# octree-nn/octfusion

Hardware: AMD Instinct MI355X
Metric: denoising-steps/sec (depth-8 octree, batch 8) (higher is better)
Workload: dtype f32 storage, fp16x3 products (fp16 hi + lo operand pairs = 22 significand bits, three fp16 MFMAs per product, fp32 accumulate)

## Files before the change

### include/ofx.h

```cpp
#ifndef OFX_H_
#define OFX_H_

#include <stddef.h>
#include <stdint.h>

#ifdef __cplusplus
extern "C" {
#endif

#define OFX_OK 0
#define OFX_EINVAL (-1)
#define OFX_ELAUNCH (-2)
#define OFX_ENODEV (-3)

#define OFX_ACT_NONE 0
#define OFX_ACT_SILU 1
#define OFX_ACT_GELU 2

#define OFX_MAX_DEPTH 16

int ofx_version(void);
const char* ofx_status_string(int status);
int ofx_device_check(void);
const char* ofx_build_hash(void);
// ... 189 lines not shown
                             const int32_t* col, const int32_t* nbr_ext, const int32_t* multi_seg, int64_t n_multi,
                             void* aux, size_t aux_bytes, const void* tfp, int64_t ldt_bytes, int nt, const void* W2,
                             int cout, const float* bias, const float* emb, int64_t lde, const int32_t* batch_id,
                             const float* res, int64_t ldr, float* out, int64_t ldc, double* stats ,
                             int64_t stats_ld, void* ws, size_t ws_bytes, void* sync , size_t sync_bytes,
                             int mode, int aux_ready, void* stream);
int ofx_set_gconv_persistent(int on);
int64_t ofx_gemm_planes_packed_bytes(int K, int N, int mode);
int ofx_pack_gemm_planes(const float* W, int64_t sk, int64_t sn, int K, int N, int mode, void* out, void* stream);
int ofx_gemm_planes(const void* ap, int64_t lda_bytes, int64_t n_a, int64_t M, int K, const int32_t* row_tab,
                    const void* W2, int N, const float* bias, float* out, int64_t ldc, int out_mode, void* ws,
                    size_t ws_bytes, void* sync, size_t sync_bytes, int mode, void* stream);
int ofx_set_gconv_cus(int cus);
int ofx_gconv3_plan(int64_t n_rows, int cout, int nkt, int wm, int ni, int cus, int32_t* out, int64_t out_len);
int ofx_set_gconv2_tile(int wm);

int ofx_grid_conv_table(int mode, int depth_out, int batch_size, int32_t pad, int32_t* nbr27,
                        void* stream);
int64_t ofx_conv3d_packed_k(int cin);
int ofx_pack_conv3d(const float* W, int cin, int cout, float* Wp, void* stream);
int ofx_gridconv_fwd(const float* x, int64_t ldx, int cin, int64_t n_in, int64_t n_out,
                     const int32_t* nbr27 ,
                     const int32_t* nbr27_ext ,
                     const float* zero_row ,
                     const float* Wp, int cout, const float* bias, const float* emb, int64_t lde,
                     const int32_t* batch_id, const float* res, int64_t ldr, float* out,
                     int64_t ldc, void* ws, size_t ws_bytes, void* stream);
int ofx_gather_gemm_f32(const float* x, int64_t ldx, int cin, int ntap, int64_t n_src, int64_t n_out, const int32_t* tab,
                        const float* zero_row, const float* Wp, int64_t Kp, int cout, const float* bias,
                        const float* res, int64_t ldr, float* out, int64_t ldc, const int32_t* out_rows, void* ws,
                        size_t ws_bytes, int out_mode, void* stream);
int ofx_set_attention_split(int on);
int ofx_attention(const float* qkv, int64_t ldq, int batch_size, int T, int heads, int ch,
                  float* out, int64_t ldo, void* stream);

int ofx_attention_bwd(const float* qkv, int64_t ldq, const float* dout, int64_t ldo, int batch_size, int T, int heads,
                      int ch, float* rowstat, float* dqkv, int64_t ldd, void* stream);

int ofx_gather_mean(const float* x, int64_t ldx, int cin, int64_t n_nodes,
                    const int32_t* seg_ptr, const int32_t* col, float* col_data,
                    void* stream);

int ofx_gn_stats(const float* x, int64_t ldx, int64_t n, int C, const int32_t* batch_id,
                 int batch_size, double* sums, void* stream);
int ofx_gn_stats_acc(const float* x, int64_t ldx, int64_t n, int C, const int32_t* batch_id, int batch_size,
                     double* sums, void* stream);
int ofx_gn_finalize(const double* sums, const float* count, int batch_size, int C, int groups,
                    float eps, float count_eps, float* mean, float* rstd, void* stream);
int ofx_gn_apply(const float* x, int64_t ldx, int64_t n, int C, const int32_t* batch_id,
                 const float* mean , const float* rstd , const double* sums ,
                 const float* count, int groups, float eps, float count_eps, const float* w, const float* bias,
                 int act, float* out, int64_t ldo, void* stream);

int ofx_gn_fused_rows(const float* x, int64_t ldx, int rows_per_batch, int batch_size, int C, int groups, float eps,
                      float count_eps, const float* w, const float* bias, int act, float* out, int64_t ldo,
                      void* stream);

int ofx_set_gn_rows16(int on);

int ofx_rows_copy(const float* src, int64_t lds, const int32_t* smap, float* dst, int64_t ldd,
                  const int32_t* dmap, int64_t n, int C, void* stream);
int ofx_rows_copy_planes(const float* src, int64_t lds, const int32_t* smap, float* dst, int64_t ldd,
                         const int32_t* dmap, int64_t n, int C, int mode, void* stream);
int ofx_act(const float* x, float* y, int64_t n, int act, void* stream);
int ofx_timestep_embedding(const float* t, int batch_size, int dim, float max_period,
                           float* out, void* stream);
int ofx_learned_sinusoid(const float* t, const float* w, int batch_size, int half, float* out, void* stream);
int ofx_linear_small(const float* a, int64_t lda, int M, int K, const float* W, int64_t ldw, int N, const float* bias,
                     const float* res, int64_t ldr, int act_in, int act_out, float* out, int64_t ldo, void* stream);
int ofx_ddim_eps_update(float* x, const float* eps, const float* coef, float* x0_out, int64_t n,
                        void* stream);
int ofx_ddim_x0_update(float* x, const float* x0, const float* noise, const float* coef,
                       int64_t n, void* stream);

size_t ofx_mc_ws_bytes(int batch, int size);
int ofx_mc_count(const float* sdf, int batch, int size, float level, void* ws, int64_t* counts, void* stream);
int ofx_mc_emit(const float* sdf, int batch, int size, float level, float step, float bbmin, float scale, void* ws,
                const int64_t* vert_off, const int64_t* tri_off, float* verts, int32_t* faces, void* stream);
int ofx_mc_table_host(int8_t* tri_table, uint8_t* ntri);

size_t ofx_mesh_cc_ws_bytes(int64_t total_verts, int64_t total_faces, int batch);
int ofx_mesh_cc_label(const int32_t* faces, const int64_t* vert_off, const int64_t* tri_off, int batch,
                      int64_t total_verts, int64_t total_faces, int32_t* label, void* ws, int32_t* status,
                      void* stream);
int ofx_mesh_cc_table(const int32_t* faces, const int32_t* label, const int64_t* vert_off, const int64_t* tri_off,
                      int batch, int64_t total_verts, int64_t total_faces, int32_t* comp_of_vert, int32_t* comp_off,
                      void* ws, const int32_t* status, void* stream);
int ofx_mesh_cc_stats(const float* verts, const int32_t* faces, const int32_t* label, const int64_t* vert_off,
                      const int64_t* tri_off, int batch, int64_t total_verts, int64_t total_faces, int64_t n_comp,
                      int32_t* table, void* ws, const int32_t* status, void* stream);
int ofx_mesh_cc_select(const float* verts, const int32_t* faces, const int32_t* label, const int64_t* vert_off,
                       const int64_t* tri_off, int batch, int64_t total_verts, int64_t total_faces,
                       int32_t* winner_label, int64_t* keep_counts, void* ws, const int32_t* status, void* stream);
int ofx_mesh_cc_extract(const float* verts, const int32_t* faces, const int64_t* vert_off, const int64_t* tri_off,
                        int batch, int64_t total_verts, int64_t total_faces, const int64_t* new_vert_off,
                        const int64_t* new_tri_off, float* out_verts, int32_t* out_faces, void* ws,
                        const int32_t* status, void* stream);

size_t ofx_voxmesh_ws_bytes(int batch, int depth, int weld);
int ofx_voxmesh_mask_keys(const int64_t* keys, int64_t n, int batch0, int batch, int depth, void* ws, void* stream);
int ofx_voxmesh_mask_dense(const float* occ, int batch, int depth, float threshold, void* ws, void* stream);
int ofx_voxmesh_count(int batch, int depth, int weld, void* ws, int64_t* counts, void* stream);
int ofx_voxmesh_emit(int batch, int depth, int weld, void* ws, const int64_t* vert_off, const int64_t* tri_off,
                     float* verts, int32_t* faces, void* stream);

#define OFX_EMD_MAX_POINTS 2048
// ... 28 lines not shown
```

### octfusion_amd/_lib.py

```python
import ctypes
import os

import torch

_HERE = os.path.dirname(os.path.abspath(__file__))
LIB_PATH = os.environ.get('OFX_LIB', os.path.join(_HERE, 'libofx.so'))

c_p = ctypes.c_void_p
c_i = ctypes.c_int
c_l = ctypes.c_int64
c_f = ctypes.c_float
c_sz = ctypes.c_size_t
c_u64 = ctypes.c_uint64


class OfxTree(ctypes.Structure):
    _fields_ = [('depth', c_i), ('full_depth', c_i), ('batch_size', c_i),
                ('child_all', c_p), ('key_all', c_p), ('leafrank_all', c_p),
                ('nnum_host', c_p), ('nnum_nempty_host', c_p)]


_SIGS = {
    'ofx_version': (c_i, [], False),
    'ofx_status_string': (ctypes.c_char_p, [c_i], False),
    'ofx_device_check': (c_i, [], False),
    'ofx_build_hash': (ctypes.c_char_p, [], False),
    'ofx_probe_mfma_sustained': (c_i, [c_i, c_i, c_p, c_p, c_p], True),
    'ofx_scan_ws_bytes': (c_sz, [c_l], False),
    'ofx_scan_i32': (c_i, [c_p, c_p, c_l, c_p, c_p], True),
    'ofx_octree_full_layer': (c_i, [c_i, c_i, c_p, c_p, c_p], True),
    'ofx_octree_split': (c_i, [c_p, c_l, c_p, c_p, c_p, c_p], True),
    'ofx_octree_grow': (c_i, [c_p, c_p, c_l, c_p, c_p, c_p], True),
    'ofx_split_small_label0': (c_i, [c_p, c_i, c_i, c_p, c_p], True),
    'ofx_split_small_label1': (c_i, [c_p, c_i, c_i, c_p, c_p, c_p], True),
    'ofx_split_large_label0': (c_i, [c_p, c_l, c_p, c_p], True),
    'ofx_split_large_label1': (c_i, [c_p, c_l, c_p, c_p, c_p], True),
    'ofx_octree2voxel_cf': (c_i, [c_p, c_l, c_i, c_i, c_i, c_p, c_p], True),
    'ofx_voxel2octree_cf': (c_i, [c_p, c_i, c_i, c_i, c_p, c_l, c_p], True),
    'ofx_points_sort_ws_bytes': (c_sz, [c_l], False),
    'ofx_points_keys': (c_i, [c_p, c_l, c_p, c_i, c_l, c_i, c_p, c_p, c_p], True),
    'ofx_points_sort': (c_i, [c_p, c_p, c_l, c_p, c_p, c_p, c_sz, c_p], True),
    'ofx_octree_label_from_points': (c_i, [c_p, c_l, c_p, c_l, c_i, c_i, c_p, c_p], True),
    'ofx_octree_point_features': (c_i, [c_p, c_p, c_l, c_p, c_l, c_p, c_l, c_p, c_l, c_i, c_p, c_p, c_p, c_p], True),
    'ofx_tree_leafrank_ws_bytes': (c_sz, [c_l], False),
    'ofx_tree_leafrank': (c_i, [c_p, c_p, c_i, c_p, c_p, c_p], True),
    'ofx_graph_nodes': (c_i, [ctypes.POINTER(OfxTree), c_i, c_p, c_p, c_p, c_p, c_p], True),
    'ofx_graph_count': (c_i, [ctypes.POINTER(OfxTree), c_i, c_p, c_p], True),
    'ofx_graph_reverse_count': (c_i, [c_p, c_p, c_l, c_p, c_p], True),
    'ofx_graph_reverse_fill': (c_i, [c_p, c_p, c_l, c_p, c_p, c_p, c_p, c_p], True),
    'ofx_graph_primary_w': (c_i, [c_p, c_p, c_p, c_l, c_p, c_p], True),
    'ofx_graph_multi_flag_w': (c_i, [c_p, c_p, c_l, c_p, c_p], True),
    'ofx_graph_primary_ext_w': (c_i, [c_p, c_p, c_p, c_l, c_p, c_p, c_p, c_p], True),
    'ofx_graphconv_bwd_data': (c_i, [c_p, c_l, c_i, c_l, c_p, c_p, c_p, c_p, c_p, c_p, c_l, c_p, c_p, c_l, c_i, c_p,
                                     c_l, c_p, c_sz, c_p], True),
    'ofx_graphconv_bwd_weight': (c_i, [c_p, c_l, c_i, c_l, c_p, c_p, c_p, c_p, c_p, c_l, c_p, c_p, c_l, c_i, c_p, c_l,
                                       c_i, c_p, c_l, c_p, c_sz, c_p], True),
    'ofx_gn_backward': (c_i, [c_p, c_l, c_p, c_l, c_l, c_i, c_p, c_i, c_p, c_i, c_f, c_p, c_p, c_p, c_p, c_i, c_p, c_p,
                              c_p, c_l, c_p, c_p, c_p], True),
    'ofx_gemm_tn_f32': (c_i, [c_p, c_l, c_p, c_l, c_l, c_l, c_l, c_p, c_p, c_sz, c_p], True),
    'ofx_table_reverse_count': (c_i, [c_p, c_l, c_i, c_l, c_p, c_p], True),
    'ofx_table_reverse_fill': (c_i, [c_p, c_l, c_i, c_l, c_p, c_p, c_p, c_p, c_p], True),
    'ofx_seg_primary_w': (c_i, [c_p, c_p, c_p, c_l, c_p, c_p], True),
    'ofx_seg_multi_flag_w': (c_i, [c_p, c_p, c_l, c_p, c_p], True),
    'ofx_seg_primary_ext_w': (c_i, [c_p, c_p, c_p, c_l, c_l, c_p, c_p, c_p, c_p], True),
    'ofx_gridconv_bwd_data': (c_i, [c_p, c_l, c_i, c_l, c_l, c_p, c_p, c_p, c_p, c_p, c_p, c_l, c_p, c_p, c_i, c_p, c_l,
                                    c_p, c_sz, c_p], True),
    'ofx_gridconv_bwd_weight': (c_i, [c_p, c_l, c_i, c_l, c_l, c_p, c_p, c_p, c_p, c_l, c_i, c_p, c_p, c_sz, c_p], True),
    'ofx_attention_bwd': (c_i, [c_p, c_l, c_p, c_l, c_i, c_i, c_i, c_i, c_p, c_p, c_l, c_p], True),
    'ofx_adamw_step': (c_i, [c_p, c_p, c_p, c_p, c_l, c_f, c_f, c_f, c_f, c_f, c_i, c_p], True),
    'ofx_ema_update': (c_i, [c_p, c_p, c_l, c_f, c_p], True),
    'ofx_gn_fused_rows': (c_i, [c_p, c_l, c_i, c_i, c_i, c_i, c_f, c_f, c_p, c_p, c_i, c_p, c_l, c_p], True),
    'ofx_set_gn_rows16': (c_i, [c_i], True),
    'ofx_mpu_eval': (c_i, [ctypes.POINTER(OfxTree), c_i, c_i, c_p, c_l, c_p, c_p, c_p, c_p], True),
    'ofx_mpu_eval_grid': (c_i, [ctypes.POINTER(OfxTree), c_i, c_i, c_p, c_i, c_f, c_f, c_i, c_l, c_l, c_p, c_p, c_p], True),
    'ofx_mpu_eval_grad': (c_i, [ctypes.POINTER(OfxTree), c_i, c_i, c_p, c_l, c_p, c_p, c_p, c_p, c_p], True),
    'ofx_mpu_backward': (c_i, [ctypes.POINTER(OfxTree), c_i, c_i, c_p, c_l, c_p, c_p, c_p, c_p, c_p], True),
    'ofx_octree_ce': (c_i, [c_p, c_l, c_p, c_l, c_f, c_p, c_p, c_l, c_p], True),
    'ofx_sdf_reg_loss': (c_i, [c_p, c_p, c_p, c_p, c_l, c_f, c_f, c_p, c_p, c_p, c_p], True),
    'ofx_kl_sample_fwd': (c_i, [c_p, c_l, c_p, c_l, c_i, c_p, c_p, c_p], True),
    'ofx_kl_sample_bwd': (c_i, [c_p, c_l, c_p, c_p, c_l, c_i, c_f, c_p, c_l, c_p], True),
    'ofx_graph_fill': (c_i, [ctypes.POINTER(OfxTree), c_i, c_p, c_p, c_p], True),
    'ofx_graph_expand': (c_i, [c_p, c_l, c_p, c_p, c_p, c_p, c_p], True),
    'ofx_graph_type_frac': (c_i, [c_p, c_p, c_p, c_l, c_i, c_p, c_l, c_p], True),
    'ofx_set_precision': (c_i, [c_i], True),
    'ofx_set_range_words': (c_i, [c_p], True),
    'ofx_get_precision': (c_i, [], False),
    'ofx_gn_apply_rows': (c_i, [], False),
    'ofx_set_attention_split': (c_i, [c_i], True),
    'ofx_gather_gemm_f32': (c_i, [c_p, c_l, c_i, c_i, c_l, c_l, c_p, c_p, c_p, c_l, c_i, c_p, c_p, c_l, c_p, c_l, c_p, c_p, c_sz, c_i, c_p], True),
    'ofx_graphconv_narrow_in_tab': (c_i, [c_p, c_l, c_i, c_l, c_p, c_p, c_p, c_p, c_l, c_p, c_p, c_i, c_p, c_i, c_p, c_p, c_p, c_l, c_p, c_l,
                                          c_p, c_sz, c_p], True),
    'ofx_graphconv_narrow_in': (c_i, [c_p, c_l, c_i, c_l, c_p, c_p, c_p, c_i, c_p, c_i, c_p, c_p, c_p, c_l, c_p, c_l, c_p, c_sz, c_p], True),
    'ofx_narrow_out_pack': (c_i, [c_p, c_i, c_i, c_i, c_i, c_p, c_p], True),
    'ofx_narrow_out_type_term': (c_i, [c_p, c_l, c_i, c_l, c_p, c_i, c_i, c_p, c_p, c_p], True),
    'ofx_graphconv_narrow_out': (c_i, [c_p, c_l, c_i, c_l, c_p, c_p, c_p, c_p, c_l, c_p], True),
    'ofx_packed_floats': (c_l, [c_l, c_l], False),
    'ofx_packed_k': (c_l, [c_l], False),
    'ofx_graphconv_packed_k': (c_l, [c_i, c_i], False),
    'ofx_pack_weights': (c_i, [c_p, c_l, c_l, c_l, c_l, c_i, c_i, c_p, c_l, c_p], True),
    'ofx_gemm_f32': (c_i, [c_p, c_l, c_p, c_l, c_l, c_p, c_l, c_l, c_p, c_p, c_l, c_p, c_l, c_p, c_p, c_sz, c_p], True),
    'ofx_gemm_f32_planes': (c_i, [c_p, c_l, c_p, c_l, c_l, c_p, c_l, c_l, c_p, c_p, c_l, c_p, c_l, c_p, c_p, c_sz, c_i, c_p], True),
    'ofx_graphconv_fwd': (c_i, [c_p, c_l, c_i, c_l, c_p, c_p, c_p, c_p, c_p, c_l, c_p, c_p, c_l, c_i, c_p, c_l,
                                c_i, c_p, c_p, c_l, c_p, c_p, c_l, c_p, c_l, c_p, c_l, c_p, c_sz, c_p], True),
    'ofx_planes_split': (c_i, [c_p, c_l, c_l, c_i, c_i, c_i, c_p, c_l, c_p], True),
    'ofx_planes_merge': (c_i, [c_p, c_l, c_l, c_i, c_i, c_p, c_l, c_p], True),
    'ofx_gn_apply_planes': (c_i, [c_p, c_l, c_l, c_i, c_p, c_p, c_p, c_p, c_p, c_i, c_f, c_f, c_p, c_p, c_i, c_i, c_p,
                                  c_l, c_p, c_p, c_p, c_l, c_p, c_p, c_l, c_p], True),
    'ofx_gn_apply_planes_oct': (c_i, [c_p, c_l, c_l, c_i, c_p, c_p, c_p, c_p, c_p, c_i, c_f, c_f, c_p, c_p, c_i, c_i, c_p,
                                      c_l, c_l, c_p, c_p, c_p, c_l, c_i, c_p, c_p, c_l, c_p], True),
    'ofx_planes_packed_ktiles': (c_l, [c_i, c_i, c_i], False),
    'ofx_planes_packed_bytes': (c_l, [c_i, c_i, c_i, c_i], False),
    'ofx_pack_weights_planes': (c_i, [c_p, c_l, c_l, c_i, c_i, c_i, c_i, c_p, c_p], True),
    'ofx_graphconv_fwd_planes': (c_i, [c_p, c_l, c_i, c_l, c_p, c_p, c_p, c_p, c_l, c_p, c_sz, c_p, c_l, c_i, c_p, c_i,
                                       c_p, c_p, c_l, c_p, c_p, c_l, c_p, c_l, c_p, c_l, c_p, c_sz, c_p, c_sz, c_i, c_i,
                                       c_p], True),
    'ofx_set_gconv_persistent': (c_i, [c_i], True),
    'ofx_set_gconv_cus': (c_i, [c_i], True),
    'ofx_gemm_planes_packed_bytes': (c_l, [c_i, c_i, c_i], False),
    'ofx_pack_gemm_planes': (c_i, [c_p, c_l, c_l, c_i, c_i, c_i, c_p, c_p], True),
    'ofx_gemm_planes': (c_i, [c_p, c_l, c_l, c_l, c_i, c_p, c_p, c_i, c_p, c_p, c_l, c_i, c_p, c_sz, c_p, c_sz, c_i, c_p], False),
    'ofx_gconv3_plan': (c_i, [c_l, c_i, c_i, c_i, c_i, c_i, c_p, c_l], False),
    'ofx_set_gconv2_tile': (c_i, [c_i], True),
    'ofx_graph_multi_flag': (c_i, [c_p, c_l, c_p, c_p], True),
    'ofx_graph_primary_ext': (c_i, [c_p, c_p, c_l, c_p, c_p, c_p, c_p], True),
    'ofx_graph_primary': (c_i, [c_p, c_p, c_l, c_p, c_p], True),
    'ofx_grid_conv_table': (c_i, [c_i, c_i, c_i, c_i, c_p, c_p], True),
    'ofx_conv3d_packed_k': (c_l, [c_i], False),
    'ofx_pack_conv3d': (c_i, [c_p, c_i, c_i, c_p, c_p], True),
    'ofx_gridconv_fwd': (c_i, [c_p, c_l, c_i, c_l, c_l, c_p, c_p, c_p, c_p, c_i, c_p, c_p, c_l, c_p, c_p, c_l, c_p,
                               c_l, c_p, c_sz, c_p], True),
    'ofx_attention': (c_i, [c_p, c_l, c_i, c_i, c_i, c_i, c_p, c_l, c_p], True),
    'ofx_gather_mean': (c_i, [c_p, c_l, c_i, c_l, c_p, c_p, c_p, c_p], True),
    'ofx_gn_stats': (c_i, [c_p, c_l, c_l, c_i, c_p, c_i, c_p, c_p], True),
    'ofx_gn_stats_acc': (c_i, [c_p, c_l, c_l, c_i, c_p, c_i, c_p, c_p], True),
    'ofx_gn_finalize': (c_i, [c_p, c_p, c_i, c_i, c_i, c_f, c_f, c_p, c_p, c_p], True),
    'ofx_gn_apply': (c_i, [c_p, c_l, c_l, c_i, c_p, c_p, c_p, c_p, c_p, c_i, c_f, c_f, c_p, c_p, c_i, c_p, c_l, c_p], True),
    'ofx_rows_copy': (c_i, [c_p, c_l, c_p, c_p, c_l, c_p, c_l, c_i, c_p], True),
    'ofx_rows_copy_planes': (c_i, [c_p, c_l, c_p, c_p, c_l, c_p, c_l, c_i, c_i, c_p], True),
    'ofx_act': (c_i, [c_p, c_p, c_l, c_i, c_p], True),
    'ofx_timestep_embedding': (c_i, [c_p, c_i, c_i, c_f, c_p, c_p], True),
    'ofx_learned_sinusoid': (c_i, [c_p, c_p, c_i, c_i, c_p, c_p], True),
    'ofx_linear_small': (c_i, [c_p, c_l, c_i, c_i, c_p, c_l, c_i, c_p, c_p, c_l, c_i, c_i, c_p, c_l, c_p], True),
    'ofx_ddim_eps_update': (c_i, [c_p, c_p, c_p, c_p, c_l, c_p], True),
    'ofx_ddim_x0_update': (c_i, [c_p, c_p, c_p, c_p, c_l, c_p], True),
    'ofx_mc_ws_bytes': (c_sz, [c_i, c_i], False),
    'ofx_mc_count': (c_i, [c_p, c_i, c_i, c_f, c_p, c_p, c_p], True),
    'ofx_mc_emit': (c_i, [c_p, c_i, c_i, c_f, c_f, c_f, c_f, c_p, c_p, c_p, c_p, c_p, c_p], True),
    'ofx_mc_table_host': (c_i, [c_p, c_p], True),
    'ofx_mesh_cc_ws_bytes': (c_sz, [c_l, c_l, c_i], False),
    'ofx_mesh_cc_label': (c_i, [c_p, c_p, c_p, c_i, c_l, c_l, c_p, c_p, c_p, c_p], True),
    'ofx_mesh_cc_table': (c_i, [c_p, c_p, c_p, c_p, c_i, c_l, c_l, c_p, c_p, c_p, c_p, c_p], True),
    'ofx_mesh_cc_stats': (c_i, [c_p, c_p, c_p, c_p, c_p, c_i, c_l, c_l, c_l, c_p, c_p, c_p, c_p], True),
    'ofx_mesh_cc_select': (c_i, [c_p, c_p, c_p, c_p, c_p, c_i, c_l, c_l, c_p, c_p, c_p, c_p, c_p], True),
    'ofx_mesh_cc_extract': (c_i, [c_p, c_p, c_p, c_p, c_i, c_l, c_l, c_p, c_p, c_p, c_p, c_p, c_p, c_p], True),
    'ofx_voxmesh_ws_bytes': (c_sz, [c_i, c_i, c_i], False),
    'ofx_voxmesh_mask_keys': (c_i, [c_p, c_l, c_i, c_i, c_i, c_p, c_p], True),
    'ofx_voxmesh_mask_dense': (c_i, [c_p, c_i, c_i, c_f, c_p, c_p], True),
    'ofx_voxmesh_count': (c_i, [c_i, c_i, c_i, c_p, c_p, c_p], True),
    'ofx_voxmesh_emit': (c_i, [c_i, c_i, c_i, c_p, c_p, c_p, c_p, c_p, c_p], True),
    'ofx_surface_sample_ws_bytes':(c_sz, [c_i, c_l], False),
    'ofx_surface_sample': (c_i, [c_p, c_p, c_p, c_p, c_i, c_l, c_i, c_u64, c_i, c_p, c_p, c_p], True),
    'ofx_surface_sample_oriented': (c_i, [c_p, c_p, c_p, c_p, c_i, c_l, c_i, c_u64, c_i, c_p, c_p, c_p, c_p], True),
    'ofx_nn_matrix': (c_i, [c_p, c_l, c_i, c_p, c_l, c_i, c_p, c_p], True),
    'ofx_emd_matrix': (c_i, [c_p, c_l, c_p, c_l, c_i, c_i, c_p, c_p], True),
    'ofx_metrics_hash': (c_u64, [c_u64, c_l, c_l, c_i], False),
    'ofx_sdf_sample_ws_bytes': (c_sz, [c_l, c_i], False),
    'ofx_sdf_sample_nodes': (c_i, [c_p, c_i, c_p, c_l, c_p, c_i, c_i, c_i, c_u64, c_l, c_p, c_f, c_p, c_p, c_p, c_p, c_p,
                                   c_p], True),
    'ofx_sdf_sample_occu': (c_i, [c_p, c_i, c_l, c_u64, c_l, c_p, c_f, c_p, c_p, c_p], True),
    'ofx_mesh_sdf_ws_bytes': (c_sz, [c_i, c_l, c_l, c_i], False),
    'ofx_mesh_sdf': (c_i, [c_p, c_p, c_p, c_p, c_i, c_i, c_i, c_p, c_p, c_p, c_p], True),
    'ofx_mesh_sdf_set_counters': (c_i, [c_p], True),
}

EXPORTS = sorted(_SIGS)


class OfxError(RuntimeError):
    pass


_lib = None


def lib():
    global _lib
    if _lib is None:
        if not os.path.exists(LIB_PATH):
            raise OfxError('libofx.so not built: run `python -m octfusion_amd.build` '
                           '(the product has no CPU / eager fallback)')
        L = ctypes.CDLL(LIB_PATH)
        for name, (res, args, _) in _SIGS.items():
            fn = getattr(L, name)
            fn.restype = res
            fn.argtypes = args
        _check_fresh(L)
        _lib = L
    return _lib


def _check_fresh(L):
    if 'OFX_LIB' in os.environ:
        return
    from . import build
    try:
        want = build.source_hash()
    except OSError:
        return
    have = L.ofx_build_hash().decode()
    if have != want:
        raise OfxError('libofx.so is stale: built from sources %s, the tree is %s -- run `python -m octfusion_amd.build`'
                       % (have, want))


PROFILE = None
META = None


def _timed(prof, name, args, always):
    global META
    meta, META = META, None
    e0 = torch.cuda.Event(enable_timing=True)
    e1 = torch.cuda.Event(enable_timing=True)
    e0.record()
    rc = getattr(lib(), name)(*args)
    e1.record()
    if always or rc == 0:
        prof.append((name, e0, e1, meta))
    return rc


def call(name, *args):
    prof = PROFILE
    if prof is not None and _SIGS[name][2]:
        rc = _timed(prof, name, args, True)
    else:
        rc = getattr(lib(), name)(*args)
    if _SIGS[name][2] and rc != 0:
        msg = lib().ofx_status_string(rc).decode()
        raise OfxError('%s failed: %s (%d)' % (name, msg, rc))
    return rc


def call_may_decline(name, *args):
    prof = PROFILE
    if prof is not None:
        rc = _timed(prof, name, args, False)
    else:
        rc = getattr(lib(), name)(*args)
    if rc < 0:
        raise OfxError('%s failed with status %d' % (name, rc))
    return rc == 0


def ptr(t):
    if t is None:
        return None
    return t.data_ptr()


def stream():
    return torch.cuda.current_stream().cuda_stream


def require_device():
    if not torch.cuda.is_available():
        raise OfxError('no HIP device: octfusion_amd has no CPU path')
    rc = lib().ofx_device_check()
    if rc != 0:
        raise OfxError('ofx_device_check: %s' % lib().ofx_status_string(rc).decode())
```

### octfusion_amd/csrc/ofx_common.h

```cpp
#pragma once
#include <hip/hip_runtime.h>
#include <stdint.h>

#include "../../include/ofx.h"

#define OFX_LAUNCH_CHECK()                         \
  do {                                             \
    if (hipGetLastError() != hipSuccess) return OFX_ELAUNCH; \
  } while (0)

static inline hipStream_t ofx_stream(void* s) { return reinterpret_cast<hipStream_t>(s); }

static inline int64_t ofx_cdiv(int64_t a, int64_t b) { return (a + b - 1) / b; }

constexpr int OFX_MAX_DEVICES = 64;
static inline bool ofx_raise_lds_limit(const void* kernel, int bytes, bool (&done)[OFX_MAX_DEVICES]) {
  int dev = 0;
  if (hipGetDevice(&dev) != hipSuccess || dev < 0 || dev >= OFX_MAX_DEVICES) return false;
  if (done[dev]) return true;
  if (hipFuncSetAttribute(kernel, hipFuncAttributeMaxDynamicSharedMemorySize, bytes) != hipSuccess) return false;
  done[dev] = true;
  return true;
}

uint32_t* ofx_range_words();

static inline int ofx_grid(int64_t work_items, int block) {
  int64_t g = ofx_cdiv(work_items, block);
  if (g < 1) g = 1;
  if (g > 2048 * 4) g = 2048 * 4;
  return (int)g;
}

constexpr uint64_t MT_GAMMA = 0x9E3779B97F4A7C15ull;
__host__ __device__ __forceinline__ uint64_t mt_mix(uint64_t z) {
  z = (z ^ (z >> 30)) * 0xBF58476D1CE4E5B9ull;
  z = (z ^ (z >> 27)) * 0x94D049BB133111EBull;
  return z ^ (z >> 31);
}
__host__ __device__ __forceinline__ uint64_t mt_step(uint64_t h, uint64_t x) { return mt_mix(h + MT_GAMMA * (x + 1)); }

__host__ __device__ static inline uint32_t ofx_compact3(uint64_t v) {
  v &= 0x1249249249249249ull;
  v = (v ^ (v >> 2)) & 0x10c30c30c30c30c3ull;
  v = (v ^ (v >> 4)) & 0x100f00f00f00f00full;
  v = (v ^ (v >> 8)) & 0x1f0000ff0000ffull;
  v = (v ^ (v >> 16)) & 0x1f00000000ffffull;
  v = (v ^ (v >> 32)) & 0x1fffffull;
  return (uint32_t)v;
}
__host__ __device__ static inline uint64_t ofx_spread3(uint64_t v) {
  v &= 0x1fffffull;
  v = (v | (v << 32)) & 0x1f00000000ffffull;
  v = (v | (v << 16)) & 0x1f0000ff0000ffull;
  v = (v | (v << 8)) & 0x100f00f00f00f00full;
  v = (v | (v << 4)) & 0x10c30c30c30c30c3ull;
  v = (v | (v << 2)) & 0x1249249249249249ull;
  return v;
}
__host__ __device__ static inline void ofx_key2xyz(int64_t key, int& x, int& y, int& z, int& b) {
  const uint64_t k = (uint64_t)key & ((1ull << 48) - 1);
  b = (int)((uint64_t)key >> 48);
  z = (int)ofx_compact3(k);
  y = (int)ofx_compact3(k >> 1);
  x = (int)ofx_compact3(k >> 2);
}
__host__ __device__ static inline uint64_t ofx_xyz2morton(int x, int y, int z) {
  return (ofx_spread3((uint64_t)x) << 2) | (ofx_spread3((uint64_t)y) << 1) | ofx_spread3((uint64_t)z);
}
```

### octfusion_amd/csrc/ofx_gemm.hip

```cpp
#include "ofx_gemm_common.h"

constexpr int BM = 128;
constexpr int BK = 32;
constexpr int A_LD = BK + 4;
constexpr int MODE_DENSE = 0;
constexpr int MODE_GATHER = 1;

struct TileCoords { int split, tm, tn; };
__device__ __forceinline__ TileCoords tile_coords(const GemmArgs& g) {
  const int ntile = g.ntm * g.ntn;
  int bid = ofx_xcd_swizzle(blockIdx.x, ntile * g.nsplit);
  const int split = bid / ntile;
  bid -= split * ntile;
  const int tm = bid / g.ntn;
  return {split, tm, bid - tm * g.ntn};
}

__device__ __forceinline__ void load_a_dense(const GemmArgs& g, int64_t m0, int64_t k0, float4 (&va)[4]) {
  const int c4 = threadIdx.x & 7, r0 = threadIdx.x >> 3;
  const int64_t k = k0 + c4 * 4;
  const bool vec = ((g.lda & 3) == 0) && (k + 3 < g.K) && ((((uintptr_t)g.A) & 15) == 0);
#pragma unroll
  for (int i = 0; i < 4; ++i) {
    const int64_t m = m0 + r0 + 32 * i;
// ... 748 lines not shown
                                                            int64_t N, const int32_t* __restrict__ bid,
                                                            double* __restrict__ stats, int64_t stats_ld) {
  __shared__ double red[3][64][2];
  const int c = threadIdx.x & 63, rg = threadIdx.x >> 6;
  const int64_t n = (int64_t)blockIdx.y * 64 + c;
  const int64_t w0 = (int64_t)blockIdx.x * 64;
  const int64_t nc = n < N ? n : N - 1;
  int b[16];
  float2 v[16];
#pragma unroll
  for (int i = 0; i < 16; ++i) {
    const int64_t w = w0 + rg * 16 + i;
    const int64_t wc = w < nwr ? w : nwr - 1;
    b[i] = bid[wc * wr_rows];
    v[i] = *reinterpret_cast<const float2*>(part + (wc * N + nc) * 2);
    if (w >= nwr) { b[i] = -1; v[i] = make_float2(0.f, 0.f); }
  }
  const int bfirst = bid[w0 * wr_rows];
  bool ok = true;
#pragma unroll
  for (int i = 0; i < 16; ++i) ok = ok && (b[i] == bfirst || b[i] < 0);
  const bool uni = __syncthreads_and(ok);
  auto flush = [&](int bb, double s, double q) {
    double* o = stats + ((int64_t)bb * stats_ld + n) * 2;
    unsafeAtomicAdd(o, s); unsafeAtomicAdd(o + 1, q);
  };
  if (uni) {
    double s = 0.0, q = 0.0;
#pragma unroll
    for (int i = 0; i < 16; ++i) { s += (double)v[i].x; q += (double)v[i].y; }
    if (rg > 0) { red[rg - 1][c][0] = s; red[rg - 1][c][1] = q; }
    __syncthreads();
    if (rg == 0 && n < N) {
#pragma unroll
      for (int r = 0; r < 3; ++r) { s += red[r][c][0]; q += red[r][c][1]; }
      flush(bfirst, s, q);
    }
  } else if (n < N) {
    double s = 0.0, q = 0.0;
    int sb = -1;
#pragma unroll
    for (int i = 0; i < 16; ++i) {
      if (b[i] < 0) continue;
      if (b[i] != sb) {
        if (sb >= 0) flush(sb, s, q);
        sb = b[i]; s = 0.0; q = 0.0;
      }
      s += (double)v[i].x; q += (double)v[i].y;
    }
    if (sb >= 0) flush(sb, s, q);
  }
}

int ofx_launch_stats_reduce(const GemmArgs& g, int wr_rows, hipStream_t st) {
  const int64_t nwr = ofx_cdiv(g.M, wr_rows);
  stats_reduce_kernel<<<dim3((unsigned)ofx_cdiv(nwr, 64), (unsigned)ofx_cdiv(g.N, 64)), 256, 0, st>>>(
      g.stats_part, nwr, wr_rows, g.N, g.bid, g.stats, g.stats_ld);
  OFX_LAUNCH_CHECK();
  return OFX_OK;
}

template <int MODE>
static int launch_gemm(GemmArgs& g, float* ws, size_t ws_bytes, hipStream_t st) {
  if (g.M <= 0 || g.N <= 0) return OFX_OK;
  if (MODE == MODE_GATHER && !(g.fast && g.nbr_ext && g.aux && (!g.out_rows || g.gather_out_rows))) return OFX_EINVAL;
  {
    auto al16 = [](const void* p) { return (reinterpret_cast<uintptr_t>(p) & 15) == 0; };
    g.vec4 = g.N % 4 == 0 && al16(g.out) && g.ldc % 4 == 0 && (!g.res || (al16(g.res) && g.ldr % 4 == 0)) &&
             (!g.emb || (al16(g.emb) && g.lde % 4 == 0)) && (!g.bias || al16(g.bias));
  }
  const int bn = g.N <= 32 ? 32 : (g.N <= 64 ? 64 : 128);
  g.ntm = (int)ofx_cdiv(g.M, BM);
  g.ntn = (int)ofx_cdiv(g.N, bn);
  const int nkt = (int)(g.Kp / BK);
  int nsplit = 1;
  const int tiles = g.ntm * g.ntn;
  if (ws && tiles < 256 && nkt >= 8) {
    nsplit = (int)ofx_cdiv(512, tiles);
    if (nsplit > nkt / 4) nsplit = nkt / 4;
    if (nsplit > 64) nsplit = 64;
    const size_t per = (size_t)g.M * g.N * sizeof(float);
    if ((size_t)nsplit * per > ws_bytes) nsplit = (int)(ws_bytes / per);
    if (nsplit < 2) nsplit = 1;
  }
  g.kt_per_split = (int)ofx_cdiv(nkt, nsplit);
  nsplit = (int)ofx_cdiv(nkt, g.kt_per_split);
  g.nsplit = nsplit;
  g.ws = ws;
  bool fast = true;
  if (MODE == MODE_DENSE) {
    fast = ((g.lda & 3) == 0) && ((g.K & 3) == 0) && g.K >= 4 && ((((uintptr_t)g.A) & 15) == 0);
    if (fast) { g.ndir = 1; g.n_src = 0; g.aux = g.A; g.tf = g.A; g.ldt = g.lda; g.nbr_ext = (const int32_t*)g.A; }
  }
  g.W16 = (g_precision != 1) ? reinterpret_cast<const uint16_t*>(g.Wp + g.Kp * g.N) : nullptr;
  const int wr_rows = bn == 32 ? 32 : 64;
  const int64_t nwr = ofx_cdiv(g.M, wr_rows);
  if (!(g.stats && g.vec4 && nsplit == 1 && g.stats_part &&
        (size_t)nwr * g.N * 2 * sizeof(float) <= g.stats_part_bytes && (((uintptr_t)g.stats_part) & 15) == 0))
    g.stats_part = nullptr;
  g.oscale_p = (fast && g.W16) ? g.Wp + 2 * g.Kp * g.N : nullptr;
  const int flavour = !fast ? 0 : (!g.W16 ? 1 : (g_precision == 3 ? 3 : 2));
  int rc;
  if (bn == 32) rc = launch_cfg<MODE, 4, 1, 1, 1>(g, flavour, st);
  else if (bn == 64) rc = launch_cfg<MODE, 2, 2, 2, 1>(g, flavour, st);
  else rc = launch_cfg<MODE, 2, 2, 2, 2>(g, flavour, st);
  if (rc) return rc;
  if (nsplit > 1) {
    const bool ws16 = (((uintptr_t)g.ws) & 15) == 0;
    if (g.vec4 && ws16) splitk_reduce_v4_kernel<<<ofx_grid(g.M * (g.N >> 2), 256), 256, 0, st>>>(g);
    else splitk_reduce_kernel<<<ofx_grid(g.M * g.N, 256), 256, 0, st>>>(g);
  }
  if (g.stats_part) {
    rc = ofx_launch_stats_reduce(g, wr_rows, st);
    if (rc) return rc;
  }
  OFX_LAUNCH_CHECK();
  return OFX_OK;
}

static inline int64_t pad32(int64_t v) { return (v + 31) / 32 * 32; }

extern "C" int64_t ofx_packed_k(int64_t K) { return pad32(K); }
extern "C" int64_t ofx_graphconv_packed_k(int cin, int nt) {
  return pad32(7 * (int64_t)cin) + (nt > 1 ? pad32(7 * (int64_t)nt) : 0);
}

__global__ void pack_weights_kernel(const float* __restrict__ W, int64_t sk, int64_t sn, int64_t K, int64_t N, int cin,
                                    int nt, float* __restrict__ Wp, int64_t Kp) {
  const int64_t total = (Kp / 4) * N;
  const int ntc = nt > 1 ? nt : 0;
  const int64_t Kf = (7 * (int64_t)cin + 31) / 32 * 32;
  for (int64_t t = (int64_t)blockIdx.x * blockDim.x + threadIdx.x; t < total; t += (int64_t)gridDim.x * blockDim.x) {
    const int64_t kq = t / N, n = t - kq * N;
    float v[4];
#pragma unroll
    for (int kk = 0; kk < 4; ++kk) {
      const int64_t k = kq * 4 + kk;
      int64_t src = -1;
      if (cin > 0) {
        if (k < 7 * (int64_t)cin) {
          const int64_t dir = k / cin, c = k - dir * cin;
          src = dir * (cin + ntc) + c;
        } else if (k >= Kf && ntc > 0 && k - Kf < 7 * (int64_t)ntc) {
          const int64_t kt = k - Kf, dir = kt / ntc, ty = kt - dir * ntc;
          src = dir * (cin + ntc) + cin + ty;
        }
      } else if (k < K) {
        src = k;
      }
      v[kk] = src >= 0 ? W[src * sk + n * sn] : 0.f;
    }
    *reinterpret_cast<float4*>(Wp + t * 4) = make_float4(v[0], v[1], v[2], v[3]);
  }
}

extern "C" int ofx_pack_weights(const float* W, int64_t sk, int64_t sn, int64_t K, int64_t N, int cin, int nt,
                                float* Wp, int64_t Kp, void* stream) {
  if (!W || !Wp || K < 1 || N < 1 || (Kp & 31) || cin < 0 || nt < 0) return OFX_EINVAL;
  if (cin > 0) {
    if (Kp != ofx_graphconv_packed_k(cin, nt) || K != 7 * (int64_t)(cin + (nt > 1 ? nt : 0))) return OFX_EINVAL;
  } else if (Kp != pad32(K)) {
    return OFX_EINVAL;
  }
  if (((uintptr_t)Wp & 15) != 0) return OFX_EINVAL;
  pack_weights_kernel<<<ofx_grid((Kp / 4) * N, 256), 256, 0, ofx_stream(stream)>>>(W, sk, sn, K, N, cin, nt, Wp, Kp);
  if (int rc = pack_bf16x3(Wp, Kp, N, ofx_stream(stream))) return rc;
// ... 52 lines not shown
extern "C" int ofx_gemm_f32(const float* A, int64_t lda, const int32_t* a_rows, int64_t M, int64_t K, const float* Wp,
                            int64_t Kp, int64_t N, const float* bias, const float* res, int64_t ldr, float* out,
                            int64_t ldc, const int32_t* out_rows, void* ws, size_t ws_bytes, void* stream) {
  return ofx_gemm_f32_planes(A, lda, a_rows, M, K, Wp, Kp, N, bias, res, ldr, out, ldc, out_rows, ws, ws_bytes, 0, stream);
}

static int gather_common(GemmArgs& g, const float* x, int64_t ldx, int cin, int ndir, int64_t n_rows,
                         const int32_t* nbr, const int32_t* seg_ptr, const int32_t* col, const float* Wp, int64_t Kp,
                         int cout, const float* bias, const float* emb, int64_t lde, const int32_t* batch_id,
                         const float* res, int64_t ldr, float* out, int64_t ldc) {
  if (n_rows < 0 || cin < 1 || cout < 1 || !x || !nbr || !Wp || !out || ldx < cin || ldc < cout ||
      (res && ldr < cout) || (emb && (!batch_id || lde < cout)) || ((uintptr_t)Wp & 15))
    return OFX_EINVAL;
  g.x = x; g.ldx = ldx; g.cin = cin; g.ndir = ndir;
  g.fast = (cin % 32 == 0) && ((ldx & 3) == 0) && (((uintptr_t)x & 15) == 0);
  g.nbr = nbr; g.seg_ptr = seg_ptr; g.col = col;
  g.Kf = pad32((int64_t)ndir * cin);
  g.M = n_rows; g.K = Kp; g.Wp = Wp; g.Kp = Kp; g.N = cout; g.bias = bias;
  g.emb = emb; g.lde = lde; g.bid = batch_id; g.res = res; g.ldr = ldr; g.out = out; g.ldc = ldc;
  return OFX_OK;
}

__device__ __forceinline__ float gather_elem(const GemmArgs& g, int64_t row, int64_t k) {
  if (k >= (int64_t)g.ndir * g.cin) return 0.f;
  const int dir = (int)(k / g.cin), c = (int)(k - (int64_t)dir * g.cin);
  const int32_t nb = g.nbr[row * g.ndir + dir];
  if (nb >= 0) return g.x[(int64_t)nb * g.ldx + c];
  if (nb == -1) return 0.f;
  const int64_t s = row * g.ndir + dir;
  const int32_t a = g.seg_ptr[s], e = g.seg_ptr[s + 1];
  float acc = 0.f;
  if (g.edge_w) {
    for (int32_t p = a; p < e; ++p) acc += g.edge_w[p] * g.x[(int64_t)g.col[p] * g.ldx + c];
    return acc;
  }
  for (int32_t p = a; p < e; ++p) acc += g.x[(int64_t)g.col[p] * g.ldx + c];
  if (e - a > 1) acc /= (float)(e - a);
  return acc;
}
__global__ void __launch_bounds__(256) col_rows_kernel(const GemmArgs g, int64_t row0, int64_t rows,
                                                       float* __restrict__ colbuf) {
  const int64_t k4n = g.Kp >> 2, total = rows * k4n;
  for (int64_t t = (int64_t)blockIdx.x * blockDim.x + threadIdx.x; t < total; t += (int64_t)gridDim.x * blockDim.x) {
    const int64_t r = t / k4n, k = (t - r * k4n) * 4;
    const int64_t row = row0 + r;
    float v[4];
#pragma unroll
    for (int kk = 0; kk < 4; ++kk)
      v[kk] = (k + kk < g.Kf) ? gather_elem(g, row, k + kk) : g.tf[row * g.ldt + (k + kk - g.Kf)];
    *reinterpret_cast<float4*>(colbuf + t * 4) = make_float4(v[0], v[1], v[2], v[3]);
  }
}

static int launch_gather_via_col(const GemmArgs& g, float* ws, size_t ws_bytes, hipStream_t st) {
  if (!ws || (((uintptr_t)ws) & 15)) return OFX_EINVAL;
  size_t tail = ws_bytes / 8;
  if (tail > (size_t(16) << 20)) tail = size_t(16) << 20;
  tail &= ~size_t(15);
  const size_t row_bytes = (size_t)g.Kp * sizeof(float);
  int64_t chunk = (int64_t)((ws_bytes - tail) / row_bytes) / 128 * 128;
  if (chunk < 128) return OFX_EINVAL;
  float* tail_ws = reinterpret_cast<float*>(reinterpret_cast<char*>(ws) + (ws_bytes - tail));
  for (int64_t r0 = 0; r0 < g.M; r0 += chunk) {
    const int64_t rows = g.M - r0 < chunk ? g.M - r0 : chunk;
    col_rows_kernel<<<ofx_grid(rows * (g.Kp >> 2), 256), 256, 0, st>>>(g, r0, rows, ws);
    GemmArgs d = {};
    d.A = ws; d.lda = g.Kp; d.M = rows; d.K = g.Kp; d.Wp = g.Wp; d.Kp = g.Kp; d.N = g.N; d.bias = g.bias;
    d.emb = g.emb; d.lde = g.lde; d.bid = g.bid ? g.bid + r0 : nullptr;
    d.res = g.res ? g.res + r0 * g.ldr : nullptr; d.ldr = g.ldr;
    d.out = g.out + r0 * g.ldc; d.ldc = g.ldc;
    d.stats = g.stats; d.stats_ld = g.stats_ld;
    if (g.stats) { d.stats_part = tail_ws; d.stats_part_bytes = tail; }
    const int rc = launch_gemm<MODE_DENSE>(d, g.stats ? nullptr : tail_ws, tail, st);
    if (rc) return rc;
  }
  return OFX_OK;
}

extern "C" int ofx_graphconv_fwd(const float* x, int64_t ldx, int cin, int64_t n_nodes, const int32_t* nbr,
                                 const int32_t* seg_ptr, const int32_t* col, const int32_t* nbr_ext,
                                 const int32_t* multi_seg, int64_t n_multi, float* aux, const float* type_frac,
                                 int64_t ldt, int nt_pad, const float* Wp, int64_t Kp, int cout, const float* bias,
                                 const float* emb, int64_t lde, const int32_t* batch_id, const float* res, int64_t ldr,
                                 float* out, int64_t ldc, double* stats, int64_t stats_ld, void* ws, size_t ws_bytes,
                                 void* stream) {
  if (n_nodes == 0 && cin >= 1 && cout >= 1) return OFX_OK;
  GemmArgs g = {};
  int rc = gather_common(g, x, ldx, cin, 7, n_nodes, nbr, seg_ptr, col, Wp, Kp, cout, bias, emb, lde, batch_id, res,
                         ldr, out, ldc);
  if (rc) return rc;
  if (!seg_ptr || !col) return OFX_EINVAL;
  if (nt_pad < 0 || (nt_pad & 31) || Kp != g.Kf + nt_pad) return OFX_EINVAL;
  if (nt_pad > 0 && (!type_frac || ldt < nt_pad || (ldt & 3) || ((uintptr_t)type_frac & 15))) return OFX_EINVAL;
  g.tf = type_frac; g.ldt = ldt;
  if (stats) {
    if (!batch_id || stats_ld < cout) return OFX_EINVAL;
    g.stats = stats; g.stats_ld = stats_ld; g.bid = batch_id;
    g.stats_part = (float*)ws; g.stats_part_bytes = ws_bytes;
    ws = nullptr;
  }
  hipStream_t st = ofx_stream(stream);
  if (g.fast && nbr_ext && aux && (((uintptr_t)aux & 15) == 0)) {
    if (n_multi < 0 || (n_multi > 0 && !multi_seg)) return OFX_EINVAL;
    multi_mean_kernel<<<ofx_grid((n_multi + 1) * (cin / 4), 256), 256, 0, st>>>(x, ldx, cin, seg_ptr, col, multi_seg,
                                                                               n_multi, aux, ldx, nullptr);
    g.nbr_ext = nbr_ext; g.aux = aux; g.ldaux = ldx; g.n_src = n_nodes;
    if (!g.tf) { g.tf = x; g.ldt = ldx; }
    return launch_gemm<MODE_GATHER>(g, (float*)ws, ws_bytes, st);
  }
  return launch_gather_via_col(g, stats ? g.stats_part : (float*)ws, stats ? g.stats_part_bytes : ws_bytes, st);
}

extern "C" int ofx_graphconv_bwd_data(const float* dy, int64_t ldy, int cout, int64_t n_nodes, const int32_t* nbr_rev,
                                      const int32_t* rev_ptr, const int32_t* rev_row, const float* rev_w,
                                      const int32_t* nbr_ext_rev, const int32_t* multi_seg, int64_t n_multi, float* aux,
                                      const float* WpT, int64_t KpT, int cin, float* dx, int64_t ldx, void* ws,
                                      size_t ws_bytes, void* stream) {
  if (n_nodes == 0 && cin >= 1 && cout >= 1) return OFX_OK;
  GemmArgs g = {};
  int rc = gather_common(g, dy, ldy, cout, 7, n_nodes, nbr_rev, rev_ptr, rev_row, WpT, KpT, cin, nullptr, nullptr, 0,
                         nullptr, nullptr, 0, dx, ldx);
  if (rc) return rc;
  if (!rev_ptr || !rev_row || !rev_w || KpT != g.Kf) return OFX_EINVAL;
  g.edge_w = rev_w;
  g.tf = dy; g.ldt = ldy;
  hipStream_t st = ofx_stream(stream);
  if (g.fast && nbr_ext_rev && aux && (((uintptr_t)aux & 15) == 0)) {
    if (n_multi < 0 || (n_multi > 0 && !multi_seg)) return OFX_EINVAL;
    multi_mean_kernel<<<ofx_grid((n_multi + 1) * (cout / 4), 256), 256, 0, st>>>(dy, ldy, cout, rev_ptr, rev_row,
                                                                                multi_seg, n_multi, aux, ldy, rev_w);
    g.nbr_ext = nbr_ext_rev; g.aux = aux; g.ldaux = ldy; g.n_src = n_nodes;
    return launch_gemm<MODE_GATHER>(g, (float*)ws, ws_bytes, st);
  }
  return launch_gather_via_col(g, (float*)ws, ws_bytes, st);
}

struct TnArgs {
  const float* P; int64_t ldp;
  const float* x; int64_t ldx; int cin; int ndir;
  const int32_t* nbr_ext; const float* aux; int64_t n_src;
  const float* tf; int64_t ldt; int64_t Kf;
  const float* Q; int64_t ldq;
  int64_t rows, row0, Kp, N;
  int64_t rows_per_slice;
  float* part;
};

template <bool DENSE_P, bool BF16X3>
__global__ void __launch_bounds__(256, 2) tn_gemm_kernel(const TnArgs a) {
  constexpr int LD = 132;
  constexpr int TP = 128 * 80;
  __shared__ __attribute__((aligned(16))) char tn_smem[BF16X3 ? 4 * TP : 2 * 32 * LD * 4];
  float* const Ps = reinterpret_cast<float*>(tn_smem);
  float* const Qs = Ps + 32 * LD;
  char* const Pt = tn_smem;
  char* const Qt = tn_smem + 2 * TP;
  const int lane = threadIdx.x & 63, wid = threadIdx.x >> 6;
  const int wm = wid >> 1, wn = wid & 1, l31 = lane & 31, h = lane >> 5;
  const int64_t m0 = (int64_t)blockIdx.x * 128, n0 = (int64_t)blockIdx.y * 128;
  const int64_t r_begin = (int64_t)blockIdx.z * a.rows_per_slice;
  const int64_t r_end = r_begin + a.rows_per_slice < a.rows ? r_begin + a.rows_per_slice : a.rows;
  f32x16 acc[2][2];
#pragma unroll
// ... 408 lines not shown
```

### octfusion_amd/csrc/ofx_gemm2.hip

```cpp
#include "ofx_planes.h"

template <int PREC, int WM, int NI>
__global__ void __launch_bounds__(512, 2) gconv2_kernel(const Gemm2Args a) {
  typedef G2Half<PREC, NI> Half;
  typedef G2Cfg<WM, NI> CF;
  constexpr int G2_NI = NI, G2_BN = CF::BN, G2_EPI_LOADS = CF::EPI_LOADS, RH = CF::READS;
  constexpr int G2_WM = WM, G2_BM = CF::BM, G2_A_BYTES = CF::A_BYTES, G2_BUF = CF::BUF, G2_TAB = CF::TAB;
  constexpr int G2_GLDS_PER_STEP = CF::GLDS;
  extern __shared__ __attribute__((aligned(128))) char smem2[];
  const GemmArgs& g = a.e;

  float osc = *g.oscale_p;
  asm volatile("" : "+s"(osc));
  const int ntile = g.ntm * g.ntn;
  const int bid = ofx_xcd_swizzle(blockIdx.x, ntile);
  const int tm = bid / g.ntn, tn = bid - tm * g.ntn;
  const int64_t m0 = a.row0 + (int64_t)tm * G2_BM, n0 = (int64_t)tn * G2_BN;

  const int lane = threadIdx.x & 63;
  const int wid = __builtin_amdgcn_readfirstlane(threadIdx.x >> 6);
  const int wm = wid >> 1, wn = wid & 1;
  const int l31 = lane & 31, h = lane >> 5;
  if (WM == 2 && a.stagger > 0 && blockIdx.x >= 256 && (int)blockIdx.x < a.prefetch) {
    const int grp = (int)blockIdx.x >> 8, ngrp = a.prefetch >> 8;
// ... 467 lines not shown
        const int64_t kk = k - Kf, dir = kk / ntc, ty = kk - dir * ntc;
        src = dir * (cin + ntc) + cin + ty;
      }
      w[e] = src >= 0 ? W[src * sk + n * sn] * wscale : 0.f;
    }
    u32x4 o;
    if (g2_pairs(mode)) {
#pragma unroll
      for (int e = 0; e < 4; ++e) {
        unsigned hi, lo;
        g2_split2(mode, w[2 * e], w[2 * e + 1], hi, lo);
        o[e] = p < 4 ? hi : lo;
      }
    } else {
#pragma unroll
      for (int e = 0; e < 4; ++e) o[e] = g2_pk_f16(w[2 * e], w[2 * e + 1]);
    }
    *reinterpret_cast<u32x4*>(out + t * 16) = o;
  }
}

extern "C" int ofx_pack_weights_planes(const float* W, int64_t sk, int64_t sn, int cin, int nt, int cout, int mode,
                                       void* out, void* stream) {
  if (!W || !out || mode < 1 || mode > 3 || cin < 1 || (cin % g2_chunk(mode)) || nt < 0 || cout < 1 ||
      ((uintptr_t)out & 15))
    return OFX_EINVAL;
  const int64_t nkt = ofx_planes_packed_ktiles(cin, nt, mode);
  const int ntc = nt > 1 ? nt : 0;
  if (ofx_launch_weight_scale(W, sk, sn, 7 * (int64_t)(cin + ntc), cout, mode != 2 ? 1 : 0,
                              reinterpret_cast<float*>((char*)out + nkt * cout * G2_LINE), ofx_stream(stream)))
    return OFX_ELAUNCH;
  planes_pack_kernel<<<ofx_grid(nkt * cout * 8, 256), 256, 0, ofx_stream(stream)>>>(W, sk, sn, cin, ntc,
                                                                                    cout, nkt, mode, (char*)out);
  OFX_LAUNCH_CHECK();
  return OFX_OK;
}

extern "C" int64_t ofx_gemm_planes_packed_bytes(int K, int N, int mode) {
  if (!g2_pairs(mode) || K < 32 || (K % 32) || N < 1) return 0;
  return (int64_t)(K / 32) * N * G2_LINE + G2_TRAILER;
}
extern "C" int ofx_pack_gemm_planes(const float* W, int64_t sk, int64_t sn, int K, int N, int mode, void* out,
                                    void* stream) {
  if (!W || !out || !g2_pairs(mode) || K < 32 || (K % 32) || N < 1 || ((uintptr_t)out & 15)) return OFX_EINVAL;
  const int64_t nkt = K / 32;
  if (ofx_launch_weight_scale(W, sk, sn, K, N, mode != 2 ? 1 : 0, reinterpret_cast<float*>((char*)out + nkt * N * G2_LINE),
                              ofx_stream(stream)))
    return OFX_ELAUNCH;
  planes_pack_kernel<<<ofx_grid(nkt * N * 8, 256), 256, 0, ofx_stream(stream)>>>(W, sk, sn, K, 0, N, nkt, mode, (char*)out, 1);
  OFX_LAUNCH_CHECK();
  return OFX_OK;
}

int ofx_launch_stats_reduce(const GemmArgs& g, int wr_rows, hipStream_t st);

template <int PREC, int WM, int NI>
static int g2_launch(const Gemm2Args& a, hipStream_t st) {
  static bool attr_set[OFX_MAX_DEVICES] = {};
  if (!ofx_raise_lds_limit(reinterpret_cast<const void*>(&gconv2_kernel<PREC, WM, NI>), G2Cfg<WM, NI>::LDS, attr_set))
    return OFX_ELAUNCH;
  gconv2_kernel<PREC, WM, NI><<<a.e.ntm * a.e.ntn, G2Cfg<WM, NI>::THREADS, G2Cfg<WM, NI>::LDS, st>>>(a);
  return OFX_OK;
}

static int g2_wm = 0;
constexpr int G2_STAGGER_PER_KTILE = 1100;
extern "C" int ofx_set_gconv2_tile(int wm) {
  if (wm != 0 && wm != 2 && wm != 4) return OFX_EINVAL;
  g2_wm = wm;
  return OFX_OK;
}

static int g3_wm_pref = 0;
static int g3_auto_wm(int64_t M, int cout, int nkt, int ni) {
  (void)cout; (void)ni;
  if (g3_wm_pref == 2 || g3_wm_pref == 4) return g3_wm_pref;
  const int64_t U4 = ofx_cdiv(M, 256) * ofx_cdiv(cout, 64 * ni) * nkt;
  return U4 >= 3500 ? 4 : 2;
}
int ofx_launch_gconv3(Gemm2Args& a, int mode, int wm, int ni, void* ws_tail, size_t ws_tail_bytes, void* sync,
                      size_t sync_bytes, hipStream_t st, int nd = 7);
static int g2_persistent = 1;
void ofx_gconv3_set_hybrid(int on);
extern "C" int ofx_set_gconv_persistent(int on) {
  if (on < 0 || on > 2) return OFX_EINVAL;
  g2_persistent = on ? 1 : 0;
  ofx_gconv3_set_hybrid(on == 2 ? 0 : 1);
  return OFX_OK;
}

extern "C" int ofx_graphconv_fwd_planes(const void* xp, int64_t ldx_bytes, int cin, int64_t n_nodes,
                                        const int32_t* seg_ptr, const int32_t* col, const int32_t* nbr_ext,
                                        const int32_t* multi_seg, int64_t n_multi, void* aux, size_t aux_bytes,
                                        const void* tfp, int64_t ldt_bytes, int nt, const void* W2, int cout,
                                        const float* bias, const float* emb, int64_t lde, const int32_t* batch_id,
                                        const float* res, int64_t ldr, float* out, int64_t ldc, double* stats,
                                        int64_t stats_ld, void* ws, size_t ws_bytes, void* sync, size_t sync_bytes,
                                        int mode, int aux_ready, void* stream) {
  if (mode < 1 || mode > 3) return OFX_EINVAL;
  const int64_t ch = g2_chunk(mode);
  if (n_nodes == 0 && cin >= 1 && cout >= 1) return OFX_OK;
  if (n_nodes < 0 || cin < 1 || (cin % ch) || cout < 1 || !xp || !seg_ptr || !col || !nbr_ext || !aux || !W2 || !out ||
      ldx_bytes < (int64_t)cin * (g2_pairs(mode) ? 4 : 2) || (ldx_bytes & 127) || ((uintptr_t)xp & 127) ||
      ((uintptr_t)aux & 127) || ((uintptr_t)W2 & 127) || ldc < cout || (res && ldr < cout) ||
      (emb && (!batch_id || lde < cout)) || n_multi < 0 || (n_multi > 0 && !multi_seg) || nt < 0)
    return OFX_EINVAL;
  if (aux_bytes < (size_t)(n_multi + 1) * (size_t)ldx_bytes) return OFX_EINVAL;
  const int ntc = nt > 1 ? nt : 0;
  if (ntc > 0 && (!tfp || (ldt_bytes & 127) || ((uintptr_t)tfp & 127))) return OFX_EINVAL;
  if (stats && (!batch_id || stats_ld < cout)) return OFX_EINVAL;
  hipStream_t st = ofx_stream(stream);
  if (!aux_ready)
    planes_multi_mean_kernel<<<ofx_grid((n_multi + 1) * (cin / 8), 256), 256, 0, st>>>(
        (const char*)xp, ldx_bytes, cin, seg_ptr, col, multi_seg, n_multi, mode, (char*)aux);
  Gemm2Args a = {};
  a.xp = (const char*)xp; a.ldx = ldx_bytes; a.aux = (const char*)aux; a.n_src = n_nodes; a.nbr_ext = nbr_ext;
  a.tfp = ntc ? (const char*)tfp : (const char*)xp; a.ldt = ntc ? ldt_bytes : ldx_bytes;
  a.W2 = (const char*)W2;
  a.tpd = (int)(cin / ch); a.nkt_g = 7 * a.tpd; a.nkt = (int)ofx_planes_packed_ktiles(cin, nt, mode);
  GemmArgs& g = a.e;
  g.M = n_nodes; g.N = cout; g.K = g.Kp = (int64_t)a.nkt * ch; g.bias = bias; g.emb = emb; g.lde = lde; g.bid = batch_id;
  g.res = res; g.ldr = ldr; g.out = out; g.ldc = ldc; g.nsplit = 1;
  g.oscale_p = reinterpret_cast<const float*>((const char*)W2 + (int64_t)a.nkt * cout * G2_LINE);
  {
    auto al16 = [](const void* p) { return (reinterpret_cast<uintptr_t>(p) & 15) == 0; };
    g.vec4 = g.N % 4 == 0 && al16(g.out) && g.ldc % 4 == 0 && (!g.res || (al16(g.res) && g.ldr % 4 == 0)) &&
             (!g.emb || (al16(g.emb) && g.lde % 4 == 0)) && (!g.bias || al16(g.bias));
  }
  const int ni = cout <= 64 ? 1 : 2;
  g.ntn = (int)ofx_cdiv(g.N, 64 * ni);
  if (stats) {
    g.stats = stats; g.stats_ld = stats_ld;
    const int64_t nwr = ofx_cdiv(g.M, 64);
    if (g.vec4 && ws && (size_t)nwr * g.N * 2 * sizeof(float) <= ws_bytes && (((uintptr_t)ws) & 15) == 0) {
      g.stats_part = (float*)ws; g.stats_part_bytes = ws_bytes;
    }
  }
  int rc = OFX_OK;
#define G2_GO(P_, WM_)                                                                        \
  (ni == 1 ? (WM_ == 4 ? g2_launch<P_, 4, 1>(a, st) : g2_launch<P_, 2, 1>(a, st))             \
           : (WM_ == 4 ? g2_launch<P_, 4, 2>(a, st) : g2_launch<P_, 2, 2>(a, st)))
  auto launch = [&](int wm, int64_t row0, int64_t rows) -> int {
    a.row0 = row0;
    g.ntm = (int)ofx_cdiv(rows, wm * 64);
    a.stagger = wm == 2 ? G2_STAGGER_PER_KTILE * a.nkt : 0;
    a.prefetch = wm == 4 ? 256 : (ni == 1 ? 768 : 512);
    return mode == 2 ? G2_GO(2, wm) : (mode == 3 ? G2_GO(3, wm) : G2_GO(1, wm));
  };
  const int64_t tiles4 = ofx_cdiv(g.M, 256) * g.ntn;
  const int64_t tail4 = tiles4 % 256;
  const bool small_tail = tail4 > 0 && tail4 <= 64 && tiles4 < 1536;
  int wm_auto = (cout <= 128 && tiles4 < 2048) ? 2 : 4;
  if (cout > 128 && small_tail) wm_auto = 2;
  rc = 1;
  if (g2_persistent && sync) {
    size_t used = 0;
    if (g.stats_part) used = ((size_t)ofx_cdiv(g.M, 64) * (size_t)g.N * 2 * sizeof(float) + 255) & ~(size_t)255;
    const int wm3 = (g2_wm == 2 || g2_wm == 4) ? g2_wm : g3_auto_wm(g.M, cout, a.nkt, ni);
    if (ws && used <= ws_bytes)
      rc = ofx_launch_gconv3(a, mode, wm3, ni, (char*)ws + used, ws_bytes - used, sync, sync_bytes, st);
    if (rc < 0) return rc;
  }
  if (rc == 1) rc = launch((g2_wm == 2 || g2_wm == 4) ? g2_wm : wm_auto, 0, g.M);
#undef G2_GO
  if (rc) return rc;
  if (g.stats_part) {
    rc = ofx_launch_stats_reduce(g, 64, st);
    if (rc) return rc;
  }
  OFX_LAUNCH_CHECK();
  return OFX_OK;
}

extern "C" int ofx_gemm_planes(const void* ap, int64_t lda_bytes, int64_t n_a, int64_t M, int K, const int32_t* row_tab,
                               const void* W2, int N, const float* bias, float* out, int64_t ldc, int out_mode, void* ws,
                               size_t ws_bytes, void* sync, size_t sync_bytes, int mode, void* stream) {
  if (!g2_pairs(mode) || !ap || !row_tab || !W2 || !out || M < 0 || n_a < 1 || K < 32 || (K % 32) || N < 4 || (N & 3) ||
      lda_bytes < (int64_t)K * 4 || (lda_bytes & 127) || ((uintptr_t)ap & 127) || ((uintptr_t)W2 & 127) || ldc < N ||
      (ldc & 3) || ((uintptr_t)out & 15) || (bias && ((uintptr_t)bias & 15)) ||
      (out_mode && (!g2_pairs(out_mode) || (ldc & 31) || (N & 31) || ((uintptr_t)out & 127))))
    return OFX_EINVAL;
  if (M == 0) return OFX_OK;
  if (!sync || !ws || N < 128) return 1;
  Gemm2Args a = {};
  a.xp = (const char*)ap; a.ldx = lda_bytes; a.aux = (const char*)ap; a.n_src = n_a; a.nbr_ext = row_tab;
  a.tfp = (const char*)ap; a.ldt = lda_bytes;
  a.W2 = (const char*)W2;
  a.tpd = K / 32; a.nkt_g = a.tpd; a.nkt = a.tpd;
  GemmArgs& g = a.e;
  g.M = M; g.N = N; g.K = g.Kp = K; g.bias = bias; g.out = out; g.ldc = ldc; g.nsplit = 1; g.out_planes = out_mode;
  g.oscale_p = reinterpret_cast<const float*>((const char*)W2 + (int64_t)a.nkt * N * G2_LINE);
  g.vec4 = 1;
  g.ntn = (int)ofx_cdiv(g.N, 128);
  const int wm = g3_auto_wm(M, N, a.nkt, 2);
  const int rc = ofx_launch_gconv3(a, mode, wm, 2, ws, ws_bytes, sync, sync_bytes, ofx_stream(stream), 1);
  if (rc) return rc;
  OFX_LAUNCH_CHECK();
  return OFX_OK;
}
```

### octfusion_amd/csrc/ofx_gemm_common.h

```cpp
#pragma once
#include "ofx_common.h"

typedef float f32x16 __attribute__((ext_vector_type(16)));

struct GemmArgs {
  const float* A; int64_t lda; const int32_t* a_rows;
  const float* x; int64_t ldx; int cin; int ndir; int fast;
  const int32_t* nbr;
  const int32_t* seg_ptr; const int32_t* col;
  const float* edge_w;
  const float* tf; int64_t ldt; int64_t Kf;
  const int32_t* nbr_ext;
  const float* aux; int64_t ldaux; int64_t n_src;
  int64_t M, K;
  const float* Wp; int64_t Kp, N;
  const uint16_t* W16;
  const float* oscale_p;
  const float* bias;
  const float* emb; int64_t lde; const int32_t* bid;
  const float* res; int64_t ldr;
  float* out; int64_t ldc; const int32_t* out_rows;
  int gather_out_rows;
  int out_planes;
  double* stats; int64_t stats_ld;
  int ntm, ntn, nsplit, kt_per_split;
  float* ws;
  int vec4;
  float* stats_part; size_t stats_part_bytes;
};

static __global__ void __launch_bounds__(256) weight_absmax_kernel(const float* __restrict__ W, int64_t sk, int64_t sn, int64_t K,
                                                            int64_t N, unsigned* __restrict__ acc) {
  __shared__ float red[256];
  float m = 0.f;
  for (int64_t t = (int64_t)blockIdx.x * 256 + threadIdx.x; t < K * N; t += (int64_t)gridDim.x * 256) {
    const float a = fabsf(W[(t / N) * sk + (t % N) * sn]);
    if (a <= 3.0e38f) m = fmaxf(m, a);
  }
  red[threadIdx.x] = m;
  __syncthreads();
  for (int o = 128; o > 0; o >>= 1) {
    if ((int)threadIdx.x < o) red[threadIdx.x] = fmaxf(red[threadIdx.x], red[threadIdx.x + o]);
    __syncthreads();
  }
  if (threadIdx.x == 0) atomicMax(acc, __float_as_uint(red[0]));
}
static __global__ void weight_scale_finish_kernel(int fp16_operands, float* __restrict__ scale) {
  const float mx = __uint_as_float(reinterpret_cast<const unsigned*>(scale)[0]);
  float s = 1.f;
  if (fp16_operands && mx > 0.f) {
    int e;
    frexpf(mx, &e);
    int sh = 15 - e;
    sh = sh < -60 ? -60 : (sh > 60 ? 60 : sh);
    s = ldexpf(1.f, sh);
  }
  scale[0] = 1.f / s;
  scale[1] = s;
}
static inline int ofx_launch_weight_scale(const float* W, int64_t sk, int64_t sn, int64_t K, int64_t N, int fp16_operands,
                                          float* scale, hipStream_t st) {
  if (hipMemsetAsync(scale, 0, sizeof(float), st) != hipSuccess) return OFX_ELAUNCH;
  int64_t nb = (K * N + 256 * 16 - 1) / (256 * 16);
  nb = nb < 1 ? 1 : (nb > 1024 ? 1024 : nb);
  weight_absmax_kernel<<<(unsigned)nb, 256, 0, st>>>(W, sk, sn, K, N, reinterpret_cast<unsigned*>(scale));
  if (hipGetLastError() != hipSuccess) return OFX_ELAUNCH;
  weight_scale_finish_kernel<<<1, 1, 0, st>>>(fp16_operands, scale);
  if (hipGetLastError() != hipSuccess) return OFX_ELAUNCH;
  return OFX_OK;
}


__device__ __forceinline__ unsigned g2_pk_bf16(float a, float b) {
  unsigned r;
  asm("v_cvt_pk_bf16_f32 %0, %1, %2" : "=v"(r) : "v"(a), "v"(b));
  return r;
}
__device__ __forceinline__ unsigned g2_pk_f16(float a, float b) {
  const _Float16 x = (_Float16)a, y = (_Float16)b;
  return (unsigned)__builtin_bit_cast(unsigned short, x) | ((unsigned)__builtin_bit_cast(unsigned short, y) << 16);
}
__device__ __forceinline__ float g2_bf16_lo(unsigned p) { return __uint_as_float(p << 16); }
__device__ __forceinline__ float g2_bf16_hi(unsigned p) { return __uint_as_float(p & 0xffff0000u); }
// ... 213 lines not shown
```

### octfusion_amd/csrc/ofx_narrow.hip

```cpp
#include "ofx_gemm_common.h"

int ofx_launch_stats_reduce(const GemmArgs& g, int wr_rows, hipStream_t st);

namespace {

struct NarrowInArgs {
  const float* x; int64_t ldx; int cin; int64_t N;
  const int32_t* seg_ptr; const int32_t* col;
  const uint8_t* ntype; int nt;
  const float* W; int cout; const float* bias;
  float* out; int64_t ldc;
  const int32_t* bid; float* stats_part; double* stats; int64_t stats_ld;
};

template <int KP, int CI>
__global__ void __launch_bounds__(512, KP == 64 ? 6 : 4) narrow_in_kernel(const NarrowInArgs a) {
  constexpr int LD = KP + 1;
  __shared__ float cd[64 * LD];
  __shared__ float red[8][32][2];
  const int tid = threadIdx.x, lane = tid & 63, wv = tid >> 6;
  const int64_t row0 = (int64_t)blockIdx.x * 64;
  const int cin = a.cin, nt = a.nt, cpd = cin + nt, K = 7 * cpd;
  const bool wide = a.cout == 128;
  const int slice = wide ? (wv & 3) : (wv & 1);
  const int mt0 = wide ? (wv >> 2) : ((wv >> 1) & 1), nmt = (wide || wv < 4) ? 1 : 0;
  const int ln = lane & 31, lk = lane >> 5;

  {
    const int r = tid >> 3;
    for (int k = K + (tid & 7); k < KP; k += 8) cd[r * LD + k] = 0.f;
  }
  for (int s = tid; s < 64 * 7; s += 512) {
    const int r = s / 7, dir = s - r * 7;
    const int64_t row = row0 + r;
    float acc[CI], tc[8];
#pragma unroll
    for (int c = 0; c < CI; ++c) acc[c] = 0.f;
#pragma unroll
    for (int t = 0; t < 8; ++t) tc[t] = 0.f;
    int32_t b = 0, e = 0;
    if (row < a.N) { b = a.seg_ptr[row * 7 + dir]; e = a.seg_ptr[row * 7 + dir + 1]; }
    for (int32_t p = b; p < e; ++p) {
      const int64_t j = a.col[p];
      const float* xr = a.x + j * a.ldx;
      float v[CI];
#pragma unroll
      for (int c = 0; c < CI; ++c) v[c] = xr[c < cin ? c : cin - 1];
      const int ty = nt ? (int)a.ntype[j] : 0;
#pragma unroll
      for (int c = 0; c < CI; ++c) acc[c] += v[c];
#pragma unroll
      for (int t = 0; t < 8; ++t) tc[t] += ty == t ? 1.f : 0.f;
    }
    const float inv = __frcp_rn((float)(e - b > 1 ? e - b : 1));
    float* o = &cd[r * LD + dir * cpd];
// ... 305 lines not shown
__global__ void __launch_bounds__(256) narrow_out_kernel(const NarrowOutArgs a) {
  const int tid = threadIdx.x;
  const int d = tid & 7;
  const int64_t row = (int64_t)blockIdx.x * 32 + (tid >> 3);
  float acc[CO];
#pragma unroll
  for (int o = 0; o < CO; ++o) acc[o] = 0.f;
  if (row < a.N) {
    if (d < 7) {
      const int32_t b = a.seg_ptr[row * 7 + d], e = a.seg_ptr[row * 7 + d + 1];
      for (int32_t p = b; p < e; ++p) {
        const float* pr = a.P + (int64_t)a.col[p] * a.ldp + d * a.cout;
        float v[CO];
#pragma unroll
        for (int o = 0; o < CO; ++o) v[o] = pr[o < a.cout ? o : 0];
#pragma unroll
        for (int o = 0; o < CO; ++o) acc[o] += v[o];
      }
      const float cnt = (float)(e - b > 1 ? e - b : 1);
#pragma unroll
      for (int o = 0; o < CO; ++o) acc[o] = o < a.cout ? acc[o] / cnt : 0.f;
    } else if (a.tt) {
#pragma unroll
      for (int o = 0; o < CO; ++o) {
        const float v = a.tt[row * a.cout + (o < a.cout ? o : 0)];
        acc[o] = o < a.cout ? v : 0.f;
      }
    }
  }
#pragma unroll
  for (int o = 0; o < CO; ++o) {
    acc[o] += __shfl_xor(acc[o], 1);
    acc[o] += __shfl_xor(acc[o], 2);
    acc[o] += __shfl_xor(acc[o], 4);
  }
  if (d == 0 && row < a.N) {
#pragma unroll
    for (int o = 0; o < CO; ++o)
      if (o < a.cout) a.out[row * a.ldc + o] = acc[o];
  }
}

__global__ void narrow_out_pack_kernel(const float* __restrict__ W, int C, int nt, int cout, int pw, float* __restrict__ Wd) {
  const int64_t total = (int64_t)C * pw;
  for (int64_t t = (int64_t)blockIdx.x * blockDim.x + threadIdx.x; t < total; t += (int64_t)gridDim.x * blockDim.x) {
    const int c = (int)(t / pw), q = (int)(t - (int64_t)c * pw);
    const int dir = q / cout, o = q - dir * cout;
    Wd[t] = q < 7 * cout ? W[((int64_t)dir * (C + nt) + c) * cout + o] : 0.f;
  }
}

}

extern "C" int ofx_graphconv_narrow_in(const float* x, int64_t ldx, int cin, int64_t n_nodes, const int32_t* seg_ptr,
                                       const int32_t* col, const uint8_t* node_type, int nt, const float* W, int cout,
                                       const float* bias, const int32_t* batch_id, float* out, int64_t ldc, double* stats,
                                       int64_t stats_ld, void* ws, size_t ws_bytes, void* stream) {
  if (!x || !seg_ptr || !col || !W || !out || cin < 1 || cin > 8 || ldx < cin || nt < 0 || nt > 8 || (nt > 0 && !node_type) ||
      (cout != 64 && cout != 128) || ldc < cout || n_nodes < 0 ||
      7 * (cin + nt) > 96)
    return OFX_EINVAL;
  if (n_nodes == 0) return OFX_OK;
  const int64_t nblk = ofx_cdiv(n_nodes, 64);
  if (stats && (!batch_id || stats_ld < cout || !ws || ws_bytes < (size_t)nblk * cout * 2 * sizeof(float))) return OFX_EINVAL;
  hipStream_t st = ofx_stream(stream);
  NarrowInArgs a = {x, ldx, cin, n_nodes, seg_ptr, col, node_type, nt, W, cout, bias, out, ldc,
                    batch_id, (float*)ws, stats, stats_ld};
  const int K = 7 * (cin + nt);
  const unsigned nb = (unsigned)nblk;
  if (K <= 64) { if (cin <= 4) narrow_in_kernel<64, 4><<<nb, 512, 0, st>>>(a); else narrow_in_kernel<64, 8><<<nb, 512, 0, st>>>(a); }
  else { if (cin <= 4) narrow_in_kernel<96, 4><<<nb, 512, 0, st>>>(a); else narrow_in_kernel<96, 8><<<nb, 512, 0, st>>>(a); }
  OFX_LAUNCH_CHECK();
  if (stats) {
    GemmArgs g = {};
    g.M = n_nodes; g.N = cout; g.bid = batch_id; g.stats = stats; g.stats_ld = stats_ld; g.stats_part = (float*)ws;
    return ofx_launch_stats_reduce(g, 64, st);
  }
  return OFX_OK;
}

extern "C" int ofx_graphconv_narrow_in_tab(const float* x, int64_t ldx, int cin, int64_t n_nodes, const int32_t* seg_ptr,
                                           const int32_t* col, const int32_t* nbr_ext, const int32_t* multi_seg,
                                           int64_t n_multi, void* aux, const uint8_t* node_type, int nt, const float* W,
                                           int cout, const float* bias, const int32_t* batch_id, float* out, int64_t ldc,
                                           double* stats, int64_t stats_ld, void* ws, size_t ws_bytes, void* stream) {
  if (!x || !seg_ptr || !col || !nbr_ext || !aux || ((uintptr_t)aux & 15) || n_multi < 0 || (n_multi > 0 && !multi_seg) || !W ||
      !out || cin < 1 || cin > 8 || ldx < cin || nt < 0 || nt > 8 || (nt > 0 && !node_type) || (cout != 64 && cout != 128) ||
      ldc < cout || n_nodes < 0 || 7 * (cin + nt) > 96 || n_nodes + 1 + n_multi >= (1ll << 31))
    return OFX_EINVAL;
  if (n_nodes == 0) return OFX_OK;
  const int64_t ngroups = ofx_cdiv(n_nodes, 64);
  if (stats && (!batch_id || stats_ld < cout || !ws || ws_bytes < (size_t)ngroups * cout * 2 * sizeof(float))) return OFX_EINVAL;
  hipStream_t st = ofx_stream(stream);
  {
    const int64_t nbn = ofx_cdiv(n_nodes + 1, 256);
    const unsigned gn_ = (unsigned)(nbn < 16384 ? nbn : 16384);
    if (cin <= 4) narrow_rec_nodes_kernel<4><<<gn_, 256, 0, st>>>(x, ldx, cin, n_nodes, node_type, nt, (float*)aux);
    else narrow_rec_nodes_kernel<8><<<gn_, 256, 0, st>>>(x, ldx, cin, n_nodes, node_type, nt, (float*)aux);
    if (n_multi > 0) {
      const unsigned ga_ = (unsigned)ofx_cdiv(n_multi, 256);
      if (cin <= 4) narrow_rec_aux_kernel<4><<<ga_, 256, 0, st>>>(x, ldx, cin, n_nodes, seg_ptr, col, multi_seg, n_multi, node_type, nt, (float*)aux);
      else narrow_rec_aux_kernel<8><<<ga_, 256, 0, st>>>(x, ldx, cin, n_nodes, seg_ptr, col, multi_seg, n_multi, node_type, nt, (float*)aux);
    }
  }
  OFX_LAUNCH_CHECK();
  NarrowIn2Args a = {x, ldx, cin, n_nodes, nbr_ext, (const float*)aux, nt, W, cout, bias, out, ldc,
                     batch_id, (float*)ws, stats, stats_ld, ngroups};
  int dev = 0, cus = 256;
  if (hipGetDevice(&dev) == hipSuccess) {
    int n = 0;
    if (hipDeviceGetAttribute(&n, hipDeviceAttributeMultiprocessorCount, dev) == hipSuccess && n > 0) cus = n;
  }
  const int64_t want = (int64_t)cus * 2;
  const unsigned nb = (unsigned)(ngroups < want ? ngroups : want);
  const int K = 7 * (cin + nt);
  if (K <= 64) { if (cin <= 4) narrow_in2_kernel<64, 4><<<nb, 512, 0, st>>>(a); else narrow_in2_kernel<64, 8><<<nb, 512, 0, st>>>(a); }
  else if (K <= 72) { if (cin <= 4) narrow_in2_kernel<72, 4><<<nb, 512, 0, st>>>(a); else narrow_in2_kernel<72, 8><<<nb, 512, 0, st>>>(a); }
  else { if (cin <= 4) narrow_in2_kernel<96, 4><<<nb, 512, 0, st>>>(a); else narrow_in2_kernel<96, 8><<<nb, 512, 0, st>>>(a); }
  OFX_LAUNCH_CHECK();
  if (stats) {
    GemmArgs g = {};
    g.M = n_nodes; g.N = cout; g.bid = batch_id; g.stats = stats; g.stats_ld = stats_ld; g.stats_part = (float*)ws;
    return ofx_launch_stats_reduce(g, 64, st);
  }
  return OFX_OK;
}

extern "C" int ofx_narrow_out_pack(const float* W, int C, int nt, int cout, int pw, float* Wd, void* stream) {
  if (!W || !Wd || C < 1 || nt < 0 || cout < 1 || cout > 8 || pw < 7 * cout) return OFX_EINVAL;
  narrow_out_pack_kernel<<<ofx_grid((int64_t)C * pw, 256), 256, 0, ofx_stream(stream)>>>(W, C, nt, cout, pw, Wd);
  OFX_LAUNCH_CHECK();
  return OFX_OK;
}

extern "C" int ofx_narrow_out_type_term(const float* type_frac, int64_t ldt, int nt, int64_t n_nodes, const float* W, int C,
                                        int cout, const float* bias, float* tt, void* stream) {
  if (!W || !tt || C < 1 || cout < 1 || cout > 8 || nt < 0 || (nt > 0 && (!type_frac || ldt < 7 * nt)) || n_nodes < 0)
    return OFX_EINVAL;
  if (n_nodes == 0) return OFX_OK;
  const unsigned nblk = (unsigned)ofx_cdiv(n_nodes, 32);
  hipStream_t st = ofx_stream(stream);
  if (cout <= 4) narrow_type_term_kernel<4><<<nblk, 256, 0, st>>>(type_frac, ldt, nt, n_nodes, W, C, cout, bias, tt);
  else narrow_type_term_kernel<8><<<nblk, 256, 0, st>>>(type_frac, ldt, nt, n_nodes, W, C, cout, bias, tt);
  OFX_LAUNCH_CHECK();
  return OFX_OK;
}

extern "C" int ofx_graphconv_narrow_out(const float* P, int64_t ldp, int cout, int64_t n_nodes, const int32_t* seg_ptr,
                                        const int32_t* col, const float* type_term, float* out, int64_t ldc, void* stream) {
  if (!P || !seg_ptr || !col || !out || cout < 1 || cout > 8 || ldp < 7 * cout || ldc < cout || n_nodes < 0) return OFX_EINVAL;
  if (n_nodes == 0) return OFX_OK;
  NarrowOutArgs a = {P, ldp, cout, n_nodes, seg_ptr, col, type_term, out, ldc};
  hipStream_t st = ofx_stream(stream);
  const unsigned nblk = (unsigned)ofx_cdiv(n_nodes, 32);
  if (cout <= 4) narrow_out_kernel<4><<<nblk, 256, 0, st>>>(a);
  else narrow_out_kernel<8><<<nblk, 256, 0, st>>>(a);
  OFX_LAUNCH_CHECK();
  return OFX_OK;
}
```

### octfusion_amd/csrc/ofx_norm.hip

```cpp
#include "ofx_planes.h"

constexpr int GN_ROWS_PER_BLOCK = 64;

static inline int64_t gn_stats_rows(int64_t n, int batch_size, int C = 128) {
  const int64_t chunks = (n + GN_ROWS_PER_BLOCK - 1) / GN_ROWS_PER_BLOCK;
  const int64_t bytes_per_batch = n * (int64_t)C * 4 / (batch_size > 0 ? batch_size : 1);
  int64_t per_batch = bytes_per_batch / (512 << 10);
  per_batch = per_batch < 8 ? 8 : (per_batch > 128 ? 128 : per_batch);
  int64_t cap = per_batch * (int64_t)batch_size;
  if (cap < 64) cap = 64;
  return chunks <= cap ? GN_ROWS_PER_BLOCK : GN_ROWS_PER_BLOCK * ((chunks + cap - 1) / cap);
}

__global__ void __launch_bounds__(256) gn_stats_kernel(const float* __restrict__ x, int64_t ldx, int64_t n, int C,
                                                       const int32_t* __restrict__ bid, double* __restrict__ sums,
                                                       int64_t rpb) {
  __shared__ int sb[256];
  __shared__ float sv[256][8];
  const int CT = C >> 2;
  const int RP = 256 / CT;
  const int cl = threadIdx.x % CT, rl = threadIdx.x / CT;
  int cb = -1;
  float s[4] = {0, 0, 0, 0}, q[4] = {0, 0, 0, 0};
  auto flush_direct = [&](int b, const float* ps, const float* pq) {
// ... 38 lines not shown
    for (int j = 0; j < RP; ++j) {
      const int t = j * CT + cl;
      const int b = sb[t];
      if (b < 0) continue;
      if (b == cb) {
#pragma unroll
        for (int k = 0; k < 4; ++k) { ds[k] += (double)sv[t][k]; dq[k] += (double)sv[t][4 + k]; }
      } else {
        flush_direct(b, &sv[t][0], &sv[t][4]);
      }
    }
    if (cb >= 0) {
      double* o = sums + ((int64_t)cb * C + cl * 4) * 2;
#pragma unroll
      for (int k = 0; k < 4; ++k) { unsafeAtomicAdd(o + 2 * k, ds[k]); unsafeAtomicAdd(o + 2 * k + 1, dq[k]); }
    }
  }
}

extern "C" int ofx_gn_stats(const float* x, int64_t ldx, int64_t n, int C, const int32_t* batch_id, int batch_size,
                            double* sums, void* stream) {
  if (!x || !batch_id || !sums || n < 0 || C < 4 || (C & 3) || C > 1024 || ldx < C || (ldx & 3) ||
      ((uintptr_t)x & 15) || batch_size < 1)
    return OFX_EINVAL;
  hipStream_t st = ofx_stream(stream);
  if (hipMemsetAsync(sums, 0, sizeof(double) * 2 * (size_t)batch_size * C, st) != hipSuccess) return OFX_ELAUNCH;
  if (n > 0) gn_stats_kernel<<<(int)ofx_cdiv(n, gn_stats_rows(n, batch_size, C)), 256, 0, st>>>(x, ldx, n, C, batch_id, sums,
                                                                                             gn_stats_rows(n, batch_size, C));
  OFX_LAUNCH_CHECK();
  return OFX_OK;
}

extern "C" int ofx_gn_stats_acc(const float* x, int64_t ldx, int64_t n, int C, const int32_t* batch_id, int batch_size,
                                double* sums, void* stream) {
  if (!x || !batch_id || !sums || n < 0 || C < 4 || (C & 3) || C > 1024 || ldx < C || (ldx & 3) ||
      ((uintptr_t)x & 15) || batch_size < 1)
    return OFX_EINVAL;
  if (n > 0) gn_stats_kernel<<<(int)ofx_cdiv(n, gn_stats_rows(n, batch_size, C)), 256, 0, ofx_stream(stream)>>>(
      x, ldx, n, C, batch_id, sums, gn_stats_rows(n, batch_size, C));
  OFX_LAUNCH_CHECK();
  return OFX_OK;
}

__global__ void gn_finalize_kernel(const double* __restrict__ sums, const float* __restrict__ count, int B, int C, int G,
                                   float eps, float count_eps, float* __restrict__ mean, float* __restrict__ rstd) {
  const int cpg = C / G;
  for (int t = blockIdx.x * blockDim.x + threadIdx.x; t < B * G; t += gridDim.x * blockDim.x) {
    const int b = t / G, g = t - b * G;
    double S = 0, SS = 0;
    for (int c = g * cpg; c < (g + 1) * cpg; ++c) {
      S += sums[((int64_t)b * C + c) * 2];
      SS += sums[((int64_t)b * C + c) * 2 + 1];
    }
    const float cnt = count[b] * (float)cpg;
    const float inv = 1.0f / (cnt + count_eps);
    const double m = S * (double)inv;
    const double ssd = SS - 2.0 * m * S + (double)cnt * m * m;
    const double var = (ssd > 0 ? ssd : 0) * (double)inv;
    const float rs = (float)(1.0 / sqrt(var + (double)eps));
    for (int c = g * cpg; c < (g + 1) * cpg; ++c) {
      mean[(int64_t)b * C + c] = (float)m;
      rstd[(int64_t)b * C + c] = rs;
    }
  }
}

extern "C" int ofx_gn_finalize(const double* sums, const float* count, int batch_size, int C, int groups, float eps,
                               float count_eps, float* mean, float* rstd, void* stream) {
  if (!sums || !count || !mean || !rstd || batch_size < 1 || C < 1 || groups < 1 || C % groups) return OFX_EINVAL;
  gn_finalize_kernel<<<ofx_grid((int64_t)batch_size * groups, 64), 64, 0, ofx_stream(stream)>>>(
      sums, count, batch_size, C, groups, eps, count_eps, mean, rstd);
  OFX_LAUNCH_CHECK();
  return OFX_OK;
}

__device__ __forceinline__ float ofx_apply_act(float v, int act) {
  if (act == OFX_ACT_SILU) return v / (1.f + __expf(-v));
  if (act == OFX_ACT_GELU) return 0.5f * v * (1.f + erff(v * 0.70710678118654752440f));
  return v;
}

constexpr int GN_APPLY_ROWS = 64;
struct GnFin { const double* sums; const float* count; int G; float eps, count_eps; };
__device__ __forceinline__ void gn_group_stats(const GnFin& f, int b, int g, int C, float& mean, float& rstd) {
  const int cpg = C / f.G;
  double S = 0, SS = 0;
  for (int c = g * cpg; c < (g + 1) * cpg; ++c) {
    S += f.sums[((int64_t)b * C + c) * 2];
    SS += f.sums[((int64_t)b * C + c) * 2 + 1];
  }
  const float cnt = f.count[b] * (float)cpg;
  const float inv = 1.0f / (cnt + f.count_eps);
  const double m = S * (double)inv;
  const double ssd = SS - 2.0 * m * S + (double)cnt * m * m;
  const double var = (ssd > 0 ? ssd : 0) * (double)inv;
  mean = (float)m;
  rstd = (float)(1.0 / sqrt(var + (double)f.eps));
}
template <int MODE, bool FIN>
__global__ void __launch_bounds__(256) gn_apply_kernel(const float* __restrict__ x, int64_t ldx, int64_t n, int C,
                                                       const int32_t* __restrict__ bid, const float* __restrict__ mean,
                                                       const float* __restrict__ rstd, const GnFin fin,
                                                       const float* __restrict__ w,
                                                       const float* __restrict__ bias, int act, char* __restrict__ out,
                                                       int64_t ldo, int64_t aux_blocks,
                                                       const int32_t* __restrict__ seg_ptr,
                                                       const int32_t* __restrict__ col,
                                                       const int32_t* __restrict__ multi_seg, int64_t n_multi,
                                                       char* __restrict__ aux, const int32_t* __restrict__ aux_plan) {
  const int CT = C >> 2, RP = 256 / CT;
  const int cl = threadIdx.x % CT, rl = threadIdx.x / CT;
  __shared__ float fin_ms[FIN ? 2 * 2 * 1024 : 1];
  constexpr int AUX_LDS = 64;
  __shared__ int aux_v[AUX_LDS], aux_n[AUX_LDS], aux_src[AUX_LDS][4];
  int fb0 = -1, fb1 = -1;
  const int64_t gT = gridDim.x;
  const int64_t a_before = aux_blocks > 0 ? ((int64_t)blockIdx.x * aux_blocks) / gT : 0;
  const bool is_aux = aux_blocks > 0 && (((int64_t)blockIdx.x + 1) * aux_blocks) / gT > a_before;
  const int64_t aux_id = a_before, main_id = (int64_t)blockIdx.x - a_before;
  const int64_t r_begin0 = main_id * GN_APPLY_ROWS;
  const int64_t r_end0 = r_begin0 + GN_APPLY_ROWS < n ? r_begin0 + GN_APPLY_ROWS : n;
  const bool pre = FIN && !is_aux && rl < RP && r_begin0 + rl + 3 * (int64_t)RP < r_end0;
  float4 pv0, pv1, pv2, pv3;
  int pb0 = 0, pb1 = 0, pb2 = 0, pb3 = 0;
  if (pre) {
    const int64_t r = r_begin0 + rl;
    const int c_ = cl * 4;
    pb0 = bid[r]; pb1 = bid[r + RP]; pb2 = bid[r + 2 * RP]; pb3 = bid[r + 3 * RP];
    pv0 = *reinterpret_cast<const float4*>(x + r * ldx + c_);
    pv1 = *reinterpret_cast<const float4*>(x + (r + RP) * ldx + c_);
    pv2 = *reinterpret_cast<const float4*>(x + (r + 2 * RP) * ldx + c_);
    pv3 = *reinterpret_cast<const float4*>(x + (r + 3 * RP) * ldx + c_);
  }
  if (FIN) {
    if (!is_aux) {
      fb0 = bid[r_begin0];
      fb1 = bid[r_end0 - 1];
    } else {
      const int64_t v0 = aux_id * RP, v1e = v0 + RP - 1 < n_multi ? v0 + RP - 1 : n_multi;
      if (n_multi > 0) {
        fb0 = bid[multi_seg[(v0 > 0 ? v0 : 1) - 1] / 7];
        fb1 = bid[multi_seg[(v1e > 0 ? v1e : 1) - 1] / 7];
      }
    }
    const int cpg = C / fin.G;
    for (int t = threadIdx.x; t < 2 * fin.G && fb0 >= 0; t += 256) {
      const int slot = t / fin.G, g = t - slot * fin.G;
      if (slot == 1 && fb1 == fb0) continue;
      float mm, rr;
      gn_group_stats(fin, slot ? fb1 : fb0, g, C, mm, rr);
// ... 826 lines not shown
```

### octfusion_amd/graph_unet_hr.py

```python
import inspect

import torch
import torch.nn as nn

from . import ops
from .modules import (GraphConv, GraphDownsample, GraphResBlockEmbed, GraphUpsample, _Linear,
                      graphnormalization)


def level_plan(input_depth, channel_mult, num_res_blocks):
    enc, dec = [], []
    d = input_depth
    last = len(channel_mult) - 1
    for level in range(len(channel_mult)):
        enc += [('res', d, level)] * num_res_blocks[level]
        if level != last:
            enc.append(('down', d, level))
            d -= 1
    for level in range(last, -1, -1):
        for i in range(num_res_blocks[level] + 1):
            dec.append(('res', d, level))
            if level and i == num_res_blocks[level]:
                dec.append(('up', d, level))
                d += 1
# ... 89 lines not shown
            self._emb_cat_w = torch.cat([l.weight.detach() for l in lins], dim=0).contiguous()
            self._emb_cat_b = torch.cat([l.bias.detach() for l in lins], dim=0).contiguous()
            self._emb_cat_pw = ops.PackedWeight()
            self._emb_cat_key = key
        if ops.LINEAR_SMALL and emb_act.shape[0] <= 16:
            allout = ops.linear_small(emb_act, self._emb_cat_w, self._emb_cat_b)
        else:
            allout = ops.gemm(emb_act, self._emb_cat_pw.get(self._emb_cat_w, 'nk'), self._emb_cat_b)
        outs, off = {}, 0
        for b, l in zip(blocks, lins):
            outs[id(b)] = allout[:, off:off + l.out_features]
            off += l.out_features
        return outs

    def forward_as_middle(self, h, doctree, timesteps, label, context, out=None):
        return self.forward(x=h, doctree=doctree, timesteps=timesteps, label=label, context=context,
                            as_middle=True, out=out)

    @torch.no_grad()
    def forward(self, x=None, doctree=None, unet_lr=None, timesteps=None, label=None, context=None,
                as_middle=False, out=None, **kwargs):
        with ops.stats_scope(x.device):
            return self._forward(x, doctree, unet_lr, timesteps, label, context, as_middle, out)

    def _forward(self, x, doctree, unet_lr, timesteps, label, context, as_middle, out_mid=None):
        assert (label is not None) == (self.num_classes is not None), \
            'must specify y if and only if the model is class-conditional'
        timesteps = timesteps.float()
        emb = None

        def embed():
            t_emb = ops.timestep_embedding(timesteps, self.model_channels)
            lab = None
            if self.num_classes is not None:
                assert label.shape == (doctree.batch_size,)
                lab = self.label_emb(label)
            e_act = self.time_embed[2](self.time_embed[0](t_emb, act_out='silu'), res=lab, act_out='silu')
            return e_act, self._all_emb_outs(e_act)
        emb_main, emb_fork = ops.fork_stream(x.device)
        if emb_fork is not None:
            with torch.cuda.stream(emb_fork):
                emb_act, emb_outs = embed()
            if unet_lr is not None and hasattr(unet_lr, 'precompute_embeddings'):
                unet_lr.precompute_embeddings(timesteps, label, doctree.batch_size)
        else:
            emb_act, emb_outs = embed()

        dev = x.device
        n_at = {dd: doctree.csr(dd)[2] for dd in range(self._d_mid, self.input_depth + 1)}
        cat_bufs = []
        for (c_h, c_skip, dd) in self._cat_plan:
            cat_bufs.append(torch.empty(n_at[dd], c_h + c_skip, dtype=torch.float32, device=dev))

        def skip_slot(i):
            c_h, c_skip, _ = self._cat_plan[i]
            return cat_bufs[i][:, c_h:]

        d = self.input_depth
        if as_middle:
            h = x
            ops.rows_copy(x, skip_slot(0), x.shape[0])
            hs = [skip_slot(0)]
        else:
            h = self.input_blocks[0](x, doctree, d, out=skip_slot(0))
            hs = [h]
        if emb_fork is not None:
            emb_main.wait_stream(emb_fork)
        for k, ((kind, dd, _), module) in enumerate(zip(self._enc, self.input_blocks[1:])):
            slot = skip_slot(k + 1)
            if kind == 'res':
                h = module(h, emb, doctree, dd, emb_act=emb_act, out=slot, emb_out=emb_outs[id(module)])
            else:
                h = module(h, doctree, dd, out=slot)
            hs.append(h)
        d = self._d_mid

        if unet_lr is not None:
            c_mid = self.middle_block1.out_channels
            mid = torch.empty(n_at[d], 2 * c_mid, dtype=torch.float32, device=dev)
            h = self.middle_block1(h, emb, doctree, d, emb_act=emb_act, out=mid[:, :c_mid], emb_out=emb_outs[id(self.middle_block1)])
            if 'out' in inspect.signature(unet_lr.forward_as_middle).parameters:
                h_lr = unet_lr.forward_as_middle(h, doctree, timesteps, label, context, out=mid[:, c_mid:])
            else:
                h_lr = unet_lr.forward_as_middle(h, doctree, timesteps, label, context)
            if h_lr.data_ptr() == mid[:, c_mid:].data_ptr() and h_lr.shape[1] == c_mid:
                h = ops.cat_channels(h, h_lr, buf=mid)
            else:
                h = ops.cat_channels(h, h_lr)
            h = self.middle_block2(h, emb, doctree, d, emb_act=emb_act, emb_out=emb_outs[id(self.middle_block2)])

        n_skip = len(hs)
        j = 0
        pending = h
        for idx, ((kind, dd, _), module) in enumerate(zip(self._dec, self.output_blocks)):
            nxt_is_res = idx + 1 < len(self._dec) and self._dec[idx + 1][0] == 'res'
            out_slot = None
            if nxt_is_res:
                c_h_n = self._cat_plan[n_skip - 1 - (j + (1 if kind == 'res' else 0))][0]
                out_slot = cat_bufs[n_skip - 1 - (j + (1 if kind == 'res' else 0))][:, :c_h_n]
            if kind == 'res':
                si = n_skip - 1 - j
                c_h = self._cat_plan[si][0]
                left = cat_bufs[si][:, :c_h]
                if pending.data_ptr() != left.data_ptr():
                    ops.rows_copy(pending, left, pending.shape[0])
                    st = ops.get_stats(pending)
                    if st is not None:
                        setattr(left, ops.STATS_ATTR, st)
                    pending = left
                hcat = ops.cat_channels(pending, hs[si], buf=cat_bufs[si])
                pending = module(hcat, emb, doctree, dd, emb_act=emb_act, out=out_slot, emb_out=emb_outs[id(module)])
                j += 1
            else:
                pending = module(pending, doctree, dd, out=out_slot)
        h = pending
        h = self.end_norm(h, doctree, self.input_depth, act='silu', out=out_mid if as_middle else None)
        if as_middle:
            return h
        out = self.out(h, doctree, self.input_depth)
        assert out.shape[0] == x.shape[0]
        return out
```

### octfusion_amd/modules.py

```python
import math

import torch
import torch.nn as nn

from . import ops


def _gn_groups(channels, group=32):
    if channels <= 32:
        group = channels // 4
    elif channels % group != 0:
        group = 30
    assert channels % group == 0
    return group


class GraphConv(nn.Module):

    def __init__(self, in_channels, out_channels, n_edge_type=7, avg_degree=7, n_node_type=0,
                 use_bias=False):
        super().__init__()
        assert n_edge_type == 7, 'the dual octree graph has 7 edge types'
        self.in_channels = in_channels
        self.out_channels = out_channels
        self.use_bias = use_bias
        self.n_edge_type = n_edge_type
        self.avg_degree = avg_degree
        self.n_node_type = n_node_type
        node_channel = n_node_type if n_node_type > 1 else 0
        self.weights = nn.Parameter(torch.empty(n_edge_type * (in_channels + node_channel), out_channels))
        if use_bias:
            self.bias = nn.Parameter(torch.empty(out_channels))
        self.reset_parameters()
        self._pw = ops.PackedWeight()
        self._pw2 = ops.PackedPlanes()
        self._pno = ops.PackedNarrowOut()
        self.emit_stats = True

    def planes_mode(self, doctree, d, cin=None):
        mode = ops.planes_mode()
        if not mode:
            return 0
        cin = self.in_channels if cin is None else (cin if ops.planes_pairs(mode) else 64)
        N = doctree.csr(d)[2]
        tiles = ((N + 255) // 256) * ((self.out_channels + 127) // 128)
        if (cin % (32 if ops.planes_pairs(mode) else 64) or self.out_channels % 4 or self.out_channels < 64 or
                tiles < ops.PLANES_MIN_TILES):
            return 0
        return mode

    def reset_parameters(self):
        fan_in = self.avg_degree * self.in_channels
        fan_out = self.avg_degree * self.out_channels
        a = math.sqrt(3.0) * math.sqrt(2.0 / float(fan_in + fan_out))
        nn.init.uniform_(self.weights, -a, a)
        if self.use_bias:
            nn.init.zeros_(self.bias)

    @torch.no_grad()
    def forward(self, x, doctree, d, emb=None, res=None, out=None, split_input=False):
        nt = self.n_node_type if self.n_node_type > 1 else 0
        seg_ptr, col, N, E = doctree.csr(d)
        assert x.shape[0] == N, 'x has %d rows, graph depth %d has %d nodes' % (x.shape[0], d, N)
        stats = None
        if self.emit_stats and N * self.out_channels >= (1 << 14) and self.out_channels % 4 == 0:
            stats = ops.stats_zeros(doctree.batch_size * self.out_channels * 2, x.device)
        mode = ops.planes_of(x)
        cin_k = self.in_channels
        if not mode and emb is None and res is None:
            if ops.narrow_in_ok(self.in_channels, self.out_channels, nt):
                y = ops.graphconv_narrow_in(x, seg_ptr, col, self.weights, self.in_channels, nt,
                                            doctree.node_type8(d) if nt else None, self.bias if self.use_bias else None,
                                            doctree.batch_id32(d) if stats is not None else None, out, stats,
                                            ext=doctree.ext(d))
                if stats is not None:
                    setattr(y, ops.STATS_ATTR, stats)
                return y
            if ops.NARROW_OUT and self.out_channels <= 8 and self.in_channels % 32 == 0 and N >= 4096:
                pno = self._pno.get(self.weights, self.in_channels, nt)
                bias = self.bias if self.use_bias else None
                tkey = ('narrow_tt', d, nt, self.weights.data_ptr(), self.weights._version,
                        None if bias is None else (bias.data_ptr(), bias._version))
                tt = doctree._tf.get(tkey)
                if tt is None and (nt or bias is not None):
                    tt = doctree._tf[tkey] = pno.type_term(doctree.type_frac(d, nt) if nt else None, nt, N, self.in_channels, bias)
                return ops.graphconv_narrow_out(x, seg_ptr, col, pno, self.in_channels, tt, out)
        if not mode and split_input:
            mode = self.planes_mode(doctree, d)
            if mode:
                x = ops.planes_split(x, mode)
        if not mode and self.in_channels < 32:
            mode = self.planes_mode(doctree, d, cin=32)
            if mode:
                cin_k = 32 if ops.planes_pairs(mode) else 64
                x = ops.planes_split(x, mode, Cpad=cin_k)
        if mode:
            pw2 = self._pw2.get(self.weights, self.in_channels, nt, mode, cin_pad=cin_k)
            y = ops.graphconv_planes(x, mode, seg_ptr, col, doctree.ext(d), pw2, cin_k, nt,
                                     doctree.type_frac_planes(d, nt, mode) if nt else None,
                                     self.bias if self.use_bias else None, emb,
                                     doctree.batch_id32(d) if (emb is not None or stats is not None) else None,
                                     res, out, stats=stats)
            if stats is not None:
                setattr(y, ops.STATS_ATTR, stats)
            return y
        pw = self._pw.get(self.weights, 'graphconv', self.in_channels, nt)
        tf = doctree.type_frac(d, nt) if nt else None
        y = ops.graphconv(x, doctree.nbr(d), seg_ptr, col, pw, self.in_channels, tf,
                          self.bias if self.use_bias else None, emb,
                          doctree.batch_id32(d) if (emb is not None or stats is not None) else None, res, out,
                          ext=doctree.ext(d), stats=stats)
        if stats is not None:
            setattr(y, ops.STATS_ATTR, stats)
        return y

    def extra_repr(self):
        return 'channel_in={}, channel_out={}, n_edge_type={}, avg_degree={}, n_node_type={}'.format(
            self.in_channels, self.out_channels, self.n_edge_type, self.avg_degree, self.n_node_type)


class DualOctreeGroupNorm(nn.Module):

    def __init__(self, in_channels, group=32, nempty=False):
        super().__init__()
        self.eps = 1e-5
        self.nempty = nempty
        self.in_channels = in_channels
        self.group = _gn_groups(in_channels, group)
        self.channels_per_group = in_channels // self.group
        self.weights = nn.Parameter(torch.ones(1, in_channels))
        self.bias = nn.Parameter(torch.zeros(1, in_channels))

    @torch.no_grad()
    def forward(self, data, doctree, depth, act=None, out=None, planes=0):
        assert doctree.batch_id32(depth).shape[0] == data.shape[0]
        stats = ops.get_stats(data)
        if ops.planes_pairs(planes) and out is not None and not ops.planes_ok(out, planes):
            out = None
        aux_graph = None
        if planes:
            seg_ptr, col, _, _ = doctree.csr(depth)
            _, multi_seg, n_multi = doctree.ext(depth)
            oct_plan = doctree.oct_plan(depth) if ops.AUX_PLAN == 'oct' else None
            block_plan = doctree.aux_plan(depth) if ops.AUX_PLAN and oct_plan is None else None
            aux_graph = ops.AuxGraph(seg_ptr, col, multi_seg, n_multi, oct_plan, block_plan)
        y = ops.group_norm(data, doctree.batch_id32(depth), doctree.count(depth), doctree.batch_size,
                           self.weights, self.bias, self.group, self.eps, act, out, stats=stats, planes=planes,
                           aux_graph=aux_graph)
        if out is data and stats is not None:
            delattr(data, ops.STATS_ATTR)
        return y

    def extra_repr(self):
        return 'in_channels={}, group={}, nempty={}'.format(self.in_channels, self.group, self.nempty)


class _Linear(nn.Module):

    def __init__(self, cin, cout, bias=True):
        super().__init__()
        self.in_features, self.out_features = cin, cout
        self.weight = nn.Parameter(torch.empty(cout, cin))
        self.bias = nn.Parameter(torch.empty(cout)) if bias else None
        nn.init.kaiming_uniform_(self.weight, a=math.sqrt(5))
        if bias:
            bound = 1 / math.sqrt(cin)
            nn.init.uniform_(self.bias, -bound, bound)
        self._pw = ops.PackedWeight()

    @torch.no_grad()
    def forward(self, x, res=None, out=None, act_in=None, act_out=None):
        if ops.LINEAR_SMALL and x.dim() == 2 and x.shape[0] <= 16:
            return ops.linear_small(x, self.weight, self.bias, res, act_in, act_out, out)
        if act_in is not None:
            x = ops.act(x, act_in)
        y = ops.gemm(x, self._pw.get(self.weight, 'nk'), self.bias, res, out)
        return ops.act(y, act_out, out=y) if act_out is not None else y


class Conv1x1(nn.Module):

    def __init__(self, channel_in, channel_out, use_bias=False):
        super().__init__()
        self.linear = _Linear(channel_in, channel_out, use_bias)

    def forward(self, x, res=None):
        return self.linear(x, res)


class Conv1x1Gn(nn.Module):

    def __init__(self, channel_in, channel_out):
        super().__init__()
        self.conv = Conv1x1(channel_in, channel_out, use_bias=False)
        self.gn = DualOctreeGroupNorm(channel_out)

    def forward(self, x, doctree, depth):
        return self.gn(self.conv(x), doctree, depth)


class Conv1x1GnGelu(nn.Module):

    def __init__(self, channel_in, channel_out):
# ... 76 lines not shown
            ops.rows_copy(x, xa, M, smap=a_rows, planes=mode)
            setattr(xa, ops.PLANES_ATTR, mode)
            if ops.gemm_planes(xa, self._pgp.get(self.weights.view(C, C * 8), mode), out, out_planes):
                return out
        y = ops.gemm(x, self.packed(), out=out, a_rows=a_rows, out_planes=out_planes)
        return y.view(-1, self.channels) if out is None else out

    def extra_repr(self):
        return 'channels={}'.format(self.channels)


def _planes_dst(n, C, planes, device):
    out = torch.empty(n, C, dtype=torch.float32, device=device)
    ok = ops.planes_pairs(planes) and C % 32 == 0 and out.data_ptr() % 128 == 0
    return out, (planes if ok else 0)


def pool_nodes(x, doctree, d, downsample, planes=0):
    copy_src, gemm_rows, n_out = doctree.pool_maps(d)
    C = x.shape[1]
    numd = int(doctree.nnum[d])
    out, planes = _planes_dst(n_out, C, planes, x.device)
    ops.rows_copy(x, out, n_out, smap=copy_src, planes=planes)
    downsample(x[x.shape[0] - numd:], out=out, out_rows=gemm_rows, out_planes=planes)
    if planes:
        setattr(out, ops.PLANES_ATTR, planes)
    return out


def unpool_nodes(x, doctree, d, upsample, planes=0):
    copy_src, a_rows, n_copy = doctree.unpool_maps(d)
    C = x.shape[1]
    n_ne = a_rows.numel()
    out, planes = _planes_dst(n_copy + 8 * n_ne, C, planes, x.device)
    if planes and n_ne and out[n_copy:].data_ptr() % 128:
        planes = 0
    ops.rows_copy(x, out, n_copy, smap=copy_src, planes=planes)
    if n_ne:
        upsample(x, a_rows=a_rows, out=out[n_copy:].view(n_ne, 8 * C), out_planes=planes)
    if planes:
        setattr(out, ops.PLANES_ATTR, planes)
    return out


class GraphDownsample(nn.Module):

    def __init__(self, channels_in, channels_out, n_edge_type, avg_degree, n_node_type):
        super().__init__()
        self.channels_in = channels_in
        self.channels_out = channels_out
        self.downsample = Downsample(channels_in)
        self.conv = GraphConv(channels_in, channels_out, n_edge_type, avg_degree, n_node_type)

    def forward(self, x, doctree, d, out=None):
        return self.conv(pool_nodes(x, doctree, d, self.downsample, planes=self.conv.planes_mode(doctree, d - 1)),
                         doctree, d - 1, out=out, split_input=True)


class GraphUpsample(nn.Module):

    def __init__(self, channels_in, channels_out, n_edge_type, avg_degree, n_node_type):
        super().__init__()
        self.channels_in = channels_in
        self.channels_out = channels_out
        self.upsample = Upsample(channels_in)
        self.conv = GraphConv(channels_in, channels_out, n_edge_type, avg_degree, n_node_type)

    def forward(self, x, doctree, d, out=None):
        return self.conv(unpool_nodes(x, doctree, d, self.upsample, planes=self.conv.planes_mode(doctree, d + 1)),
                         doctree, d + 1, out=out, split_input=True)


def graphnormalization(channels):
    return DualOctreeGroupNorm(channels, min(32, channels))


class TimestepBlock(nn.Module):
    pass


class GraphResBlockEmbed(TimestepBlock):

    def __init__(self, channels, emb_channels, dropout, out_channels, n_edge_type, avg_degree,
                 n_node_type, use_conv=False, use_scale_shift_norm=False, dims=2,
                 use_checkpoint=False, up=False, down=False):
        super().__init__()
        if use_scale_shift_norm or use_conv:
            raise NotImplementedError('use_scale_shift_norm / use_conv are dead in the reference')
        self.channels = channels
        self.emb_channels = emb_channels
        self.out_channels = channels if out_channels is None else out_channels
        self.use_checkpoint = use_checkpoint
        self.block1_norm = graphnormalization(self.channels)
        self.silu = nn.SiLU()
        self.conv1 = GraphConv(self.channels, self.out_channels, n_edge_type, avg_degree, n_node_type)
        self.emb_layers = nn.Sequential(nn.SiLU(), _Linear(emb_channels, self.out_channels))
        self.block2_norm = graphnormalization(self.out_channels)
        self.dropout = nn.Dropout(p=dropout)
        self.conv2 = GraphConv(self.out_channels, self.out_channels, n_edge_type, avg_degree, n_node_type)
        for p in self.conv2.parameters():
            p.detach().zero_()
        if self.out_channels == channels:
            self.skip_connection = nn.Identity()
        else:
            self.skip_connection = Conv1x1(self.channels, self.out_channels)

    @torch.no_grad()
    def forward(self, x, emb, doctree, depth, emb_act=None, out=None, emb_out=None):
        skip, side = x, None
        if not isinstance(self.skip_connection, nn.Identity):
            if ops.SIDE_STREAM:
                main, side = torch.cuda.current_stream(x.device), ops.side_stream(x.device)
                side.wait_stream(main)
                with torch.cuda.stream(side):
                    skip = self.skip_connection(x)
            else:
                skip = self.skip_connection(x)
        h = self.block1_norm(x, doctree, depth, act='silu', planes=self.conv1.planes_mode(doctree, depth))
        if emb_out is None:
            if emb_act is None:
                emb_act = ops.act(emb, 'silu')
            emb_out = self.emb_layers[1](emb_act)
        assert doctree.batch_size == emb_out.shape[0]
        h = self.conv1(h, doctree, depth, emb=emb_out)
        h = self.block2_norm(h, doctree, depth, act='silu', out=h, planes=self.conv2.planes_mode(doctree, depth))
        if side is not None:
            main.wait_stream(side)
        return self.conv2(h, doctree, depth, res=skip, out=out)


class GraphResBlock(nn.Module):

    def __init__(self, channel_in, channel_out, dropout, n_edge_type=7, avg_degree=7, n_node_type=0,
                 use_checkpoint=False):
        super().__init__()
        self.channel_in = channel_in
        self.channel_out = channel_out
        self.use_checkpoint = use_checkpoint
        self.norm1 = DualOctreeGroupNorm(channel_in)
        self.conv1 = GraphConv(channel_in, channel_out, n_edge_type, avg_degree, n_node_type)
        self.norm2 = DualOctreeGroupNorm(channel_out)
        self.dropout = nn.Dropout(dropout)
        self.conv2 = GraphConv(channel_out, channel_out, n_edge_type, avg_degree, n_node_type)
        if channel_in != channel_out:
            self.conv1x1c = Conv1x1Gn(channel_in, channel_out)

    @torch.no_grad()
    def forward(self, x, doctree, depth):
        h = self.norm1(x, doctree, depth, act='silu', planes=self.conv1.planes_mode(doctree, depth))
        h = self.conv1(h, doctree, depth)
        h = self.norm2(h, doctree, depth, act='silu', out=h, planes=self.conv2.planes_mode(doctree, depth))
        if self.channel_in != self.channel_out:
            x = self.conv1x1c(x, doctree, depth)
        return self.conv2(h, doctree, depth, res=x)


class GraphResBlocks(nn.Module):

    def __init__(self, channel_in, channel_out, dropout, resblk_num, n_edge_type=7, avg_degree=7,
                 n_node_type=0, use_checkpoint=False):
        super().__init__()
        self.resblk_num = resblk_num
        channels = [channel_in] + [channel_out] * resblk_num
        self.resblks = nn.ModuleList([
            GraphResBlock(channels[i], channels[i + 1], dropout, n_edge_type, avg_degree, n_node_type,
                          use_checkpoint) for i in range(resblk_num)])

    def forward(self, data, doctree, depth):
        for blk in self.resblks:
            data = blk(data, doctree, depth)
        return data
```

### octfusion_amd/ops.py

```python
import contextlib
import os
from typing import NamedTuple

import torch

from . import _lib
from ._lib import call, call_may_decline, ptr, stream

ACT = {None: 0, 'none': 0, 'silu': 1, 'gelu': 2}

GRAPHCONV_PROFILE = None
_NO_BRACKET = contextlib.nullcontext()


@contextlib.contextmanager
def _timed_layer(prof, *rec):
    e0 = torch.cuda.Event(enable_timing=True)
    e1 = torch.cuda.Event(enable_timing=True)
    e0.record()
    yield
    e1.record()
    prof.append((e0, e1) + rec)


def _layer_bracket(flops, nbytes, width, tag):
    prof = GRAPHCONV_PROFILE
    return _NO_BRACKET if prof is None else _timed_layer(prof, flops, nbytes, width, tag)


def _meta(kind, flops=0.0, nbytes=0.0, tag=None):
    if _lib.PROFILE is not None:
        _lib.META = (kind, float(flops), float(nbytes), tag)


def _chk(t, dtype=torch.float32):
    if t is None:
        return
    if not t.is_cuda:
        raise _lib.OfxError('octfusion_amd ops need HIP tensors (no CPU path)')
    if t.dtype != dtype:
        raise TypeError('expected %s, got %s' % (dtype, t.dtype))


def _row_major(t):
    if t is None:
        return None, 0
    _chk(t)
    if t.dim() != 2:
        raise ValueError('expected a 2-D tensor')
    if t.stride(1) != 1 and t.shape[1] != 1:
        t = t.contiguous()
    ld = t.stride(0) if t.shape[0] > 1 else max(t.shape[1], t.stride(0))
    if ld < t.shape[1]:
# ... 127 lines not shown
    Cpad = Cpad if Cpad is not None else (C + ch - 1) // ch * ch
    out, ldo = _planes_out(n, Cpad, mode, x.device, out)
    range_words(x.device)
    _meta('planes_split', 0, 4.0 * n * C + (4.0 if planes_pairs(mode) else 2.0) * n * Cpad, (n, C, Cpad))
    call('ofx_planes_split', ptr(x), ldx, n, C, Cpad, mode, ptr(out), ldo, stream())
    setattr(out, PLANES_ATTR, mode)
    return out


def planes_merge(p, mode=None):
    mode = mode or planes_of(p)
    n, C = p.shape
    ld = p.stride(0) * (4 if planes_pairs(mode) else 2)
    out = torch.empty(n, C, dtype=torch.float32, device=p.device)
    call('ofx_planes_merge', ptr(p), ld, n, C, mode, ptr(out), C, stream())
    return out


class PackedPlanes:

    def __init__(self):
        self.t = None
        self.key = None

    def get(self, w, cin, nt, mode, cin_pad=None):
        cin_pad = cin if cin_pad is None else cin_pad
        key = (w.data_ptr(), w._version, tuple(w.shape), cin, nt, mode, cin_pad)
        if key == self.key:
            return self
        _chk(w)
        w = w.detach()
        if not w.is_contiguous():
            w = w.contiguous()
        K, N = w.shape
        ntc = nt if nt > 1 else 0
        assert K == 7 * (cin + ntc)
        k_logical, cin_logical = K, cin
        if cin_pad != cin:
            wp = torch.zeros(7, cin_pad + ntc, N, dtype=torch.float32, device=w.device)
            w3 = w.view(7, cin + ntc, N)
            wp[:, :cin] = w3[:, :cin]
            wp[:, cin_pad:] = w3[:, cin:]
            w = wp.view(7 * (cin_pad + ntc), N)
            cin, K = cin_pad, 7 * (cin_pad + ntc)
        L = _lib.lib()
        out = torch.empty(L.ofx_planes_packed_bytes(cin, nt, N, mode), dtype=torch.uint8, device=w.device)
        call('ofx_pack_weights_planes', ptr(w), N, 1, cin, nt, N, mode, ptr(out), stream())
        self.t, self.key, self.N, self.K, self.cin, self.nt = out, key, N, k_logical, cin_logical, nt
        self.nkt = L.ofx_planes_packed_ktiles(cin, nt, mode)
        return self


def graphconv_planes(xp, mode, seg_ptr, col, ext, pw, cin, nt, tf_planes=None, bias=None, emb=None, batch_id=None,
                     res=None, out=None, stats=None):
    assert planes_of(xp) == mode and xp.shape[1] == cin
    N = xp.shape[0]
    bpc = 4 if planes_pairs(mode) else 2
    ldx = xp.stride(0) * bpc if N > 1 else cin * bpc
    out, ldc = _out2d(out, N, pw.N, xp.device)
    nbr_ext, multi_seg, n_multi = ext
    aux = getattr(xp, AUX_ATTR, None)
    aux_ready = 1 if aux is not None else 0
    if aux is None:
        aux = torch.empty((n_multi + 1) * ldx, dtype=torch.uint8, device=xp.device)
    assert aux.numel() >= (n_multi + 1) * ldx
    emb, lde = _row_major(emb)
    if emb is not None or stats is not None:
        _chk(batch_id, torch.int32)
    res, ldr = _row_major(res)
    ldt = tf_planes.stride(0) * bpc if tf_planes is not None else 0
    _chk(bias)
    _chk(stats, torch.float64)
    E = col.numel()
    flops = 2.0 * N * pw.K * pw.N
    nbytes = bpc * (E * pw.cin + pw.K * pw.N) + 4.0 * N * pw.N + 8.0 * E
    with _layer_bracket(flops, nbytes, pw.N, ('graph2' if planes_pairs(mode) else 'graph2h', N, pw.cin, pw.N)):
        ws = workspace(xp.device)
        sync = sync_words(xp.device)
        _meta('graphconv', flops, 0, (N, pw.cin, pw.N, 'planes', 'emb' if emb is not None else '',
                                      'res' if res is not None else '', 'stats' if stats is not None else ''))
        call('ofx_graphconv_fwd_planes', ptr(xp), ldx, cin, N, ptr(seg_ptr), ptr(col), ptr(nbr_ext), ptr(multi_seg),
             n_multi, ptr(aux), aux.numel() * aux.element_size(), ptr(tf_planes), ldt, nt, ptr(pw.t), pw.N, ptr(bias),
             ptr(emb), lde, ptr(batch_id) if (emb is not None or stats is not None) else None, ptr(res), ldr, ptr(out),
             ldc, ptr(stats), pw.N, ptr(ws), ws.numel(), ptr(sync), sync.numel() * 4, mode, aux_ready, stream())
    return out


SIDE_STREAM = os.environ.get('OFX_SIDE_STREAM', '0') == '1'


def set_lane_cus(cus):
    call('ofx_set_gconv_cus', int(cus))


def side_stream(device):
    return _scratch('side', device, False, lambda: torch.cuda.Stream(device))


FORK = int(os.environ.get('OFX_FORK', '0'))


def fork_stream(device, level=1):
    if FORK < level or device.type != 'cuda':
        return None, None
    s = _scratch('fork', device, False, lambda: torch.cuda.Stream(device))
    main = torch.cuda.current_stream(device)
    if main.cuda_stream == s.cuda_stream:
        return None, None
    s.wait_stream(main)
    return main, s


SYNC_WORDS = 4096


def sync_words(device):
    def make():
        _no_capture('the flag words')
        return torch.zeros(SYNC_WORDS, dtype=torch.int32, device=device)
    return _scratch('sync', device, True, make)


def sync_error(device):
    return any(int(t.abs().sum().item()) != 0 for t in _scratch_all('sync', device))


def raise_on_sync_error(device):
    if not sync_error(device):
        return
    for t in _scratch_all('sync', device):
        t.zero_()
    call('ofx_set_gconv_persistent', 0)
    raise _lib.OfxError('a flag wait of the persistent GraphConv launch gave up on %s: the results of this call are '
                        'invalid; the process now uses the one-tile-per-block launch (ofx_set_gconv_persistent(0))' % device)


AUTO_RANGE_FALLBACK = True
# ... 165 lines not shown
    M, K = a_planes.shape
    assert planes_pairs(mode) and K == pgp.K and a_planes.stride(1) == 1
    dev = a_planes.device
    out, ldc = _out2d(out, M, pgp.N, dev)
    tabs = _scratch('row_tab', dev, False, dict)
    tab = tabs.get(M)
    if tab is None:
        if len(tabs) > 64:
            tabs.clear()
        _no_capture('the row table of a dense planes GEMM')
        tab = torch.zeros(M * 7 + 4, dtype=torch.int32, device=dev)
        tab[:M * 7].view(M, 7)[:, 0] = torch.arange(M, dtype=torch.int32, device=dev)
        tabs[M] = tab
    ws = workspace(dev)
    sync = sync_words(dev)
    _meta('dense_gemm', 2.0 * M * K * pgp.N, 4.0 * (M * K + K * pgp.N + M * pgp.N), (M, K, pgp.N, 'planes'))
    return call_may_decline('ofx_gemm_planes', ptr(a_planes), a_planes.stride(0) * 4, M, M, K, ptr(tab), ptr(pgp.t), pgp.N,
                            ptr(bias), ptr(out), ldc, out_planes, ptr(ws), ws.numel(), ptr(sync), sync.numel() * 4, mode,
                            stream())


LINEAR_SMALL = True


def linear_small(a, weight, bias=None, res=None, act_in=None, act_out=None, out=None):
    a, lda = _row_major(a)
    w, ldw = _row_major(weight.detach())
    M, K = a.shape
    N = w.shape[0]
    assert w.shape[1] == K and M <= 16
    out, ldo = _out2d(out, M, N, a.device)
    res, ldr = _row_major(res)
    _chk(bias)
    _meta('small_linear', 2.0 * M * K * N, 4.0 * (N * K + M * K + M * N), (M, K, N))
    call('ofx_linear_small', ptr(a), lda, M, K, ptr(w), ldw, N, ptr(bias.detach() if bias is not None else None), ptr(res),
         ldr, ACT[act_in], ACT[act_out], ptr(out), ldo, stream())
    return out


def learned_sinusoid(t, w):
    _chk(t), _chk(w)
    t, w = t.contiguous(), w.detach().contiguous()
    out = torch.empty(t.shape[0], 2 * w.shape[0] + 1, dtype=torch.float32, device=t.device)
    _meta('elementwise', 0, 4.0 * out.numel(), (out.numel(),))
    call('ofx_learned_sinusoid', ptr(t), ptr(w), t.shape[0], w.shape[0], ptr(out), stream())
    return out


def zero_row(device, n=4096):
    return _scratch('zeros', device, False, lambda: torch.zeros(n, dtype=torch.float32, device=device))


def graphconv(x, nbr, seg_ptr, col, pw, cin, type_frac=None, bias=None, emb=None, batch_id=None,
              res=None, out=None, ext=None, stats=None):
    x, ldx = _row_major(x)
    N = x.shape[0]
    if x.shape[1] != cin:
        raise ValueError('cin mismatch')
    out, ldc = _out2d(out, N, pw.N, x.device)
    ldt = nt_pad = 0
    if type_frac is not None:
        _chk(type_frac)
        ldt = type_frac.stride(0)
        nt_pad = type_frac.shape[1]
    emb, lde = _row_major(emb)
    if emb is not None or stats is not None:
        _chk(batch_id, torch.int32)
    res, ldr = _row_major(res)
    _chk(bias)
    _chk(stats, torch.float64)
    E = col.numel()
    flops = 2.0 * N * pw.K * pw.N
    nbytes = 4.0 * (E * cin + N * pw.N + pw.K * pw.N) + 8.0 * E
    with _layer_bracket(flops, nbytes, pw.N, ('graph', N, cin, pw.N)):
        ws = workspace(x.device)
        nbr_ext = multi_seg = aux = None
        n_multi = 0
        if ext is not None and cin % 32 == 0:
            nbr_ext, multi_seg, n_multi = ext
            aux = torch.empty((n_multi + 1) * ldx, dtype=torch.float32, device=x.device)
        args = ('ofx_graphconv_fwd', ptr(x), ldx, cin, N, ptr(nbr), ptr(seg_ptr), ptr(col), ptr(nbr_ext), ptr(multi_seg),
                n_multi, ptr(aux), ptr(type_frac), ldt, nt_pad,
                ptr(pw.t), pw.Kp, pw.N, ptr(bias), ptr(emb), lde,
                ptr(batch_id) if (emb is not None or stats is not None) else None,
                ptr(res), ldr, ptr(out), ldc, ptr(stats), pw.N, ptr(ws), ws.numel(), stream())
        _meta('graphconv', flops, 0, (N, cin, pw.N, 'reg'))
        if pw.N <= 64 or cin <= 64:
            with policy_scope('small_gemm'):
                call(*args)
        else:
            call(*args)
    return out


NARROW_IN = os.environ.get('OFX_NARROW_IN', '1') == '1'
NARROW_OUT = os.environ.get('OFX_NARROW_OUT', '1') == '1'


def narrow_in_ok(cin, cout, nt):
    return NARROW_IN and cin <= 8 and cout in (64, 128) and 7 * (cin + nt) <= 96


NARROW_IN_TAB = os.environ.get('OFX_NARROW_IN_TAB', '1') == '1'
NARROW_IN_TAB_MIN_ROWS = int(os.environ.get('OFX_NARROW_IN_TAB_MIN_ROWS', str(1 << 19)))


def graphconv_narrow_in(x, seg_ptr, col, weights, cin, nt, node_type=None, bias=None, batch_id=None, out=None, stats=None,
                        ext=None):
    x, ldx = _row_major(x)
    w = weights.detach()
    if not w.is_contiguous():
        w = w.contiguous()
    _chk(w)
    N, cout = x.shape[0], w.shape[1]
    assert x.shape[1] == cin and w.shape[0] == 7 * (cin + nt)
    out, ldc = _out2d(out, N, cout, x.device)
    if nt:
        _chk(node_type, torch.uint8)
    _chk(bias)
    _chk(stats, torch.float64)
    if stats is not None:
        _chk(batch_id, torch.int32)
    E = col.numel()
    flops = 2.0 * N * w.shape[0] * cout
    nbytes = 4.0 * (E * cin + N * cout + w.numel()) + 8.0 * E
    with _layer_bracket(flops, nbytes, cout, ('graph', N, cin, cout)):
        ws = workspace(x.device)
        _meta('graphconv_narrow', flops, nbytes, (N, cin, cout, 'narrow_in'))
        if ext is not None and NARROW_IN_TAB and N >= NARROW_IN_TAB_MIN_ROWS:
            nbr_ext, multi_seg, n_multi = ext
            aux = torch.empty((N + n_multi + 1) * (8 if cin <= 4 else 16), dtype=torch.float32, device=x.device)
            call('ofx_graphconv_narrow_in_tab', ptr(x), ldx, cin, N, ptr(seg_ptr), ptr(col), ptr(nbr_ext), ptr(multi_seg),
                 n_multi, ptr(aux), ptr(node_type) if nt else None, nt, ptr(w), cout, ptr(bias),
                 ptr(batch_id) if stats is not None else None, ptr(out), ldc, ptr(stats), cout, ptr(ws), ws.numel(),
                 stream())
        else:
            call('ofx_graphconv_narrow_in', ptr(x), ldx, cin, N, ptr(seg_ptr), ptr(col), ptr(node_type) if nt else None, nt,
                 ptr(w), cout, ptr(bias), ptr(batch_id) if stats is not None else None, ptr(out), ldc, ptr(stats), cout,
                 ptr(ws), ws.numel(), stream())
    return out


class PackedNarrowOut:

    def __init__(self):
        self.key = None
        self.pw = PackedWeight()

    def get(self, w, C, nt):
        key = (w.data_ptr(), w._version, tuple(w.shape), C, nt)
        if key != self.key:
            wd = w.detach()
            if not wd.is_contiguous():
                wd = wd.contiguous()
            _chk(wd)
            cout = wd.shape[1]
            self.width = 32 if 7 * cout <= 32 else 64
            self.wd = torch.empty(C, self.width, dtype=torch.float32, device=w.device)
            call('ofx_narrow_out_pack', ptr(wd), C, nt, cout, self.width, ptr(self.wd), stream())
            self.w = wd
            self.key = key
        return self

    def type_term(self, type_frac, nt, N, C, bias):
        cout = self.w.shape[1]
        tt = torch.empty(N, cout, dtype=torch.float32, device=self.w.device)
        _chk(bias)
        call('ofx_narrow_out_type_term', ptr(type_frac) if nt else None, type_frac.stride(0) if nt else 0, nt, N, ptr(self.w),
             C, cout, ptr(bias), ptr(tt), stream())
        return tt


def graphconv_narrow_out(x, seg_ptr, col, pno, C, type_term=None, out=None):
    N = x.shape[0]
    cout = pno.w.shape[1]
    E = col.numel()
    flops = 2.0 * N * pno.w.shape[0] * cout
    pwid = pno.width
    agg_bytes = 4.0 * (N * pwid + E + 7 * N + 2 * N * cout)
    nbytes = agg_bytes + 4.0 * (N * C + N * pwid + pno.w.numel())
    with _layer_bracket(flops, nbytes, cout, ('graph', N, C, cout)):
        P = gemm(x, pno.pw.get(pno.wd, 'kn'))
        out, ldc = _out2d(out, N, cout, x.device)
        _chk(type_term)
        assert type_term is None or (type_term.is_contiguous() and tuple(type_term.shape) == (N, cout))
        _meta('graphconv_narrow', flops, agg_bytes, (N, C, cout, 'narrow_out'))
        call('ofx_graphconv_narrow_out', ptr(P), P.stride(0), cout, N, ptr(seg_ptr), ptr(col), ptr(type_term), ptr(out),
             ldc, stream())
    return out


def gemm_tn(p, q):
# ... 147 lines not shown
    call('ofx_grid_conv_table', mode, depth_out, batch_size, pad, ptr(t), stream())
    return t


def attention(qkv, batch_size, T, heads, out=None):
    qkv, ldq = _row_major(qkv)
    C = qkv.shape[1] // 3
    ch = C // heads
    out, ldo = _out2d(out, qkv.shape[0], C, qkv.device)
    _meta('attention', 4.0 * batch_size * heads * T * T * ch, 4.0 * qkv.shape[0] * 4 * C, (batch_size, T, heads, ch))
    call('ofx_attention', ptr(qkv), ldq, batch_size, T, heads, ch, ptr(out), ldo, stream())
    return out


def attention_backward(qkv, dout, batch_size, T, heads):
    qkv, ldq = _row_major(qkv)
    dout, ldo = _row_major(dout)
    _chk(qkv), _chk(dout)
    C = qkv.shape[1] // 3
    ch = C // heads
    dqkv = torch.empty(qkv.shape[0], 3 * C, dtype=torch.float32, device=qkv.device)
    rowstat = torch.empty(batch_size * heads * T * 3, dtype=torch.float32, device=qkv.device)
    call('ofx_attention_bwd', ptr(qkv), ldq, ptr(dout), ldo, batch_size, T, heads, ch, ptr(rowstat), ptr(dqkv), 3 * C,
         stream())
    return dqkv


def gather_mean(x, seg_ptr, col):
    x, ldx = _row_major(x)
    N, C = x.shape
    out = torch.empty(N, 7, C, dtype=torch.float32, device=x.device)
    call('ofx_gather_mean', ptr(x), ldx, C, N, ptr(seg_ptr), ptr(col), ptr(out), stream())
    return out


AUX_ATTR = '_ofx_aux'
GN_FINALIZE_LAUNCH = False
GN_ROWS_TWO_KERNELS = int(os.environ.get('OFX_GN_ROWS_TWO_KERNELS', '2048'))
GN_FUSE_AUX_FINALIZE = os.environ.get('OFX_GN_FUSE_AUX_FINALIZE', '0') == '1'
GN_OCT_FINALIZE = os.environ.get('OFX_GN_OCT_FINALIZE', '1') == '1'
GN_OCT_FINALIZE_MAX_ELEMS = int(os.environ.get('OFX_GN_OCT_FINALIZE_MAX_ELEMS', str(9 << 20)))
AUX_PLAN = {'1': 'oct', '0': ''}.get(os.environ.get('OFX_AUX_PLAN', 'oct'), os.environ.get('OFX_AUX_PLAN', 'oct'))


class AuxGraph(NamedTuple):
    seg_ptr: torch.Tensor
    col: torch.Tensor
    multi_seg: torch.Tensor
    n_multi: int
    oct_plan: tuple = None
    block_plan: tuple = None


def _gn_launch(planes, aux_graph, elems, cpg=2):
    g = aux_graph if planes else None
    oct_plan, block_plan = (g.oct_plan, g.block_plan) if g is not None and AUX_PLAN else (None, None)
    oct_fin = (GN_OCT_FINALIZE and AUX_PLAN == 'oct' and oct_plan is not None and elems <= GN_OCT_FINALIZE_MAX_ELEMS
               and cpg >= 2)
    finalize = GN_FINALIZE_LAUNCH or (g is not None and not GN_FUSE_AUX_FINALIZE and not oct_fin)
    if not planes:
        return 'fp32', finalize
    if oct_plan is not None:
        return ('oct' if finalize or oct_fin else 'plain'), finalize
    return ('block' if block_plan is not None else 'plain'), finalize


def group_norm(x, batch_id, count, batch_size, weight, bias, groups, eps=1e-5, act=None, out=None,
               count_eps=None, stats=None, rows_per_batch=None, planes=0, aux_graph=None):
    if count_eps is None:
        count_eps = eps
    x, ldx = _row_major(x)
    n, C = x.shape
    dev = x.device
    range_words(dev)
    if (rows_per_batch is not None and stats is None and not planes and rows_per_batch * (C // groups) <= (1 << 16)
            and rows_per_batch < GN_ROWS_TWO_KERNELS):
        assert n == rows_per_batch * batch_size
        out, ldo = _out2d(out, n, C, dev)
        _meta('gn_fused_rows', 0, 8.0 * n * C, (n, C))
        call('ofx_gn_fused_rows', ptr(x), ldx, rows_per_batch, batch_size, C, groups, eps, count_eps,
             ptr(weight.detach().reshape(-1)), ptr(bias.detach().reshape(-1)), ACT[act], ptr(out), ldo, stream())
        return out
    if stats is not None:
        _chk(stats, torch.float64)
        assert stats.numel() == batch_size * C * 2
        sums = stats
    else:
        _meta('gn_stats', 0, 4.0 * n * C, (n, C))
        if stats_pool_has_room(batch_size * C * 2, dev):
            sums = stats_zeros(batch_size * C * 2, dev)
            call('ofx_gn_stats_acc', ptr(x), ldx, n, C, ptr(batch_id), batch_size, ptr(sums), stream())
        else:
            sums = torch.empty(batch_size * C * 2, dtype=torch.float64, device=dev)
            call('ofx_gn_stats', ptr(x), ldx, n, C, ptr(batch_id), batch_size, ptr(sums), stream())
    w = weight.detach().reshape(-1)
    b = bias.detach().reshape(-1)
    mean = rstd = None
    launch, finalize = _gn_launch(planes, aux_graph, n * C, C // groups)
    if finalize:
        mean = torch.empty(batch_size * C, dtype=torch.float32, device=dev)
        rstd = torch.empty(batch_size * C, dtype=torch.float32, device=dev)
        _meta('gn_finalize', 0, 24.0 * batch_size * C, (batch_size, C))
        call('ofx_gn_finalize', ptr(sums), ptr(count), batch_size, C, groups, eps, count_eps, ptr(mean), ptr(rstd),
             stream())
    if planes:
        if aux_graph is not None and out is not None and out.data_ptr() == x.data_ptr():
            out = None
        out, ldo = _planes_out(n, C, planes, dev, out if planes_pairs(planes) else None)
        aux = seg_ptr = col = multi_seg = None
        n_multi = 0
        if aux_graph is not None:
            seg_ptr, col, multi_seg, n_multi = aux_graph[:4]
            aux = torch.empty((n_multi + 1) * ldo, dtype=torch.uint8, device=dev)
            setattr(out, AUX_ATTR, aux)
        setattr(out, PLANES_ATTR, planes)
        _meta('gn_apply', 0, 8.0 * n * C + (n_multi + 1) * float(ldo), (n, C, 'planes+aux' if aux is not None else 'planes'))
        if launch == 'oct':
            op, shift, n_own, n_left, (o_ptr, o_ent, o_head, o_src) = aux_graph.oct_plan
            base = op.data_ptr()
            call('ofx_gn_apply_planes_oct', ptr(x), ldx, n, C, ptr(batch_id), ptr(mean), ptr(rstd), ptr(sums), ptr(count),
                 groups, eps, count_eps, ptr(w), ptr(b), ACT[act], planes, ptr(out), ldo, n_multi, ptr(aux), base + 4 * o_ptr,
                 base + 4 * o_ent, n_own, shift, base + 4 * o_head, base + 4 * o_src, n_left, stream())
        else:
            plan, n_left = aux_graph.block_plan if launch == 'block' else (None, 0)
            call('ofx_gn_apply_planes', ptr(x), ldx, n, C, ptr(batch_id), ptr(mean), ptr(rstd), ptr(sums), ptr(count), groups,
                 eps, count_eps, ptr(w), ptr(b), ACT[act], planes, ptr(out), ldo, ptr(seg_ptr), ptr(col), ptr(multi_seg),
                 n_multi, ptr(aux), ptr(plan), n_left, stream())
        return out
    out, ldo = _out2d(out, n, C, dev)
    _meta('gn_apply', 0, 8.0 * n * C, (n, C, 'fp32'))
    call('ofx_gn_apply', ptr(x), ldx, n, C, ptr(batch_id), ptr(mean), ptr(rstd), ptr(sums), ptr(count), groups, eps, count_eps,
         ptr(w), ptr(b), ACT[act], ptr(out), ldo, stream())
    return out


def group_norm_backward(x, dy, batch_id, count, batch_size, weight, bias, groups, eps=1e-5, act=None, count_eps=None):
    if count_eps is None:
        count_eps = eps
    x, ldx = _row_major(x)
    dy, ldy = _row_major(dy)
    _chk(x), _chk(dy)
    n, C = x.shape
    dev = x.device
    mean = torch.empty(batch_size * C, dtype=torch.float32, device=dev)
    rstd = torch.empty(batch_size * C, dtype=torch.float32, device=dev)
    sums = torch.empty(batch_size * C * 2, dtype=torch.float64, device=dev)
    call('ofx_gn_stats', ptr(x), ldx, n, C, ptr(batch_id), batch_size, ptr(sums), stream())
    call('ofx_gn_finalize', ptr(sums), ptr(count), batch_size, C, groups, eps, count_eps, ptr(mean), ptr(rstd),
         stream())
    w = weight.detach().reshape(-1).contiguous()
    b = bias.detach().reshape(-1).contiguous()
    coef = torch.empty(batch_size * C * 3, dtype=torch.float32, device=dev)
    dx = torch.empty(n, C, dtype=torch.float32, device=dev)
    dgamma = torch.empty(C, dtype=torch.float32, device=dev)
    dbeta = torch.empty(C, dtype=torch.float32, device=dev)
    call('ofx_gn_backward', ptr(x), ldx, ptr(dy), ldy, n, C, ptr(batch_id), batch_size, ptr(count), groups, count_eps,
         ptr(mean), ptr(rstd), ptr(w), ptr(b), ACT[act], ptr(sums), ptr(coef), ptr(dx), C, ptr(dgamma), ptr(dbeta),
         stream())
    return dx, dgamma, dbeta


STATS_ATTR = '_ofx_gn_stats'


class _StatsPool:
    SIZE = 1 << 19

    def __init__(self):
        self.buf = None
        self.cur = 0
        self.depth = 0
        self.gen = 0


def _stats_pool_of(device):
    return _scratch('stats', device, True, _StatsPool)


@contextlib.contextmanager
def stats_scope(device):
    p = _stats_pool_of(device)
    if p.depth == 0:
        if p.buf is None:
            _no_capture('the GroupNorm statistics pool')
            p.buf = torch.empty(p.SIZE, dtype=torch.float64, device=device)
        p.buf.zero_()
        p.cur = 0
        p.gen += 1
    p.depth += 1
    try:
        yield
    finally:
        p.depth -= 1


def stats_pool_has_room(n, device):
    p = _stats_pool_of(device)
    return p.depth > 0 and p.cur + n <= p.SIZE


def stats_zeros(n, device):
    p = _stats_pool_of(device)
    if p.depth > 0 and p.cur + n <= p.SIZE:
        st = p.buf[p.cur:p.cur + n]
        p.cur += (n + 1) & ~1
        st._ofx_gen = p.gen
        st._ofx_pool = p
        return st
    return torch.zeros(n, dtype=torch.float64, device=device)


def get_stats(t):
    st = getattr(t, STATS_ATTR, None)
    pool = getattr(st, '_ofx_pool', None)
    if pool is not None and st._ofx_gen != pool.gen:
        return None
    return st


def cat_channels(a, b, buf=None):
    out = buf if buf is not None else torch.cat([a, b], dim=1)
    sa, sb = get_stats(a), get_stats(b)
    if sa is not None and sb is not None:
        B = sa.numel() // (a.shape[1] * 2)
        st = torch.cat([sa.view(B, a.shape[1], 2), sb.view(B, b.shape[1], 2)], dim=1).contiguous().view(-1)
        setattr(out, STATS_ATTR, st)
    return out


def rows_copy(src, dst, n, smap=None, dmap=None, C=None, planes=0):
    src, lds = _row_major(src)
    C = C if C is not None else src.shape[1]
    dst, ldd = _out2d(dst, n, C, src.device)
    _meta('rows_copy', 0, 8.0 * n * C, (n, C))
    if planes:
        call('ofx_rows_copy_planes', ptr(src), lds, ptr(smap), ptr(dst), ldd, ptr(dmap), n, C, planes, stream())
    else:
        call('ofx_rows_copy', ptr(src), lds, ptr(smap), ptr(dst), ldd, ptr(dmap), n, C, stream())
    return dst


def act(x, kind, out=None):
    _chk(x)
    x = x.contiguous()
    if out is None:
        out = torch.empty_like(x)
    _meta('elementwise', 0, 8.0 * x.numel(), (x.numel(),))
    call('ofx_act', ptr(x), ptr(out), x.numel(), ACT[kind], stream())
    return out


def timestep_embedding(t, dim, max_period=10000.0):
    _chk(t)
    t = t.contiguous()
    out = torch.empty(t.shape[0], dim, dtype=torch.float32, device=t.device)
    call('ofx_timestep_embedding', ptr(t), t.shape[0], dim, float(max_period), ptr(out), stream())
    return out


def octree2voxel_cf(data, batch_size, depth):
    data, ld = _row_major(data)
    C = data.shape[1]
    S = 1 << depth
    vox = torch.empty(batch_size, C, S, S, S, dtype=torch.float32, device=data.device)
    call('ofx_octree2voxel_cf', ptr(data), ld, C, batch_size, depth, ptr(vox), stream())
    return vox


def voxel2octree_cf(vox, depth, out=None):
    _chk(vox)
    vox = vox.contiguous()
    B, C = vox.shape[:2]
    out, ld = _out2d(out, B * (8 ** depth), C, vox.device)
    call('ofx_voxel2octree_cf', ptr(vox), C, B, depth, ptr(out), ld, stream())
    return out


def ddim_eps_update(x, eps, coef, x0_out=None):
# ... 14 lines not shown
```

Before: 120.9.

## Fuse GroupNorm mean/rstd finalize into graphconv stats-reduce epilogue

Result: no change. 120.7 (-0.1%).

```diff
diff --git a/include/ofx.h b/include/ofx.h
--- a/include/ofx.h
+++ b/include/ofx.h
@@ -265,6 +265,36 @@
                  const float* count, int groups, float eps, float count_eps, const float* w, const float* bias,
                  int act, float* out, int64_t ldo, void* stream);
 
+typedef struct OfxStatsFin {
+  const float* count;
+  float* mean;
+  float* rstd;
+  int batch_size, groups, col_off, c_total;
+  float eps, count_eps;
+} OfxStatsFin;
+int ofx_graphconv_fwd_fin(const float* x, int64_t ldx, int cin, int64_t n_nodes, const int32_t* nbr,
+                          const int32_t* seg_ptr, const int32_t* col, const int32_t* nbr_ext, const int32_t* multi_seg,
+                          int64_t n_multi, float* aux, const float* type_frac, int64_t ldt, int nt_pad, const float* Wp,
+                          int64_t Kp, int cout, const float* bias, const float* emb, int64_t lde, const int32_t* batch_id,
+                          const float* res, int64_t ldr, float* out, int64_t ldc, double* stats, int64_t stats_ld,
+                          void* ws, size_t ws_bytes, const OfxStatsFin* fin, void* stream);
+int ofx_graphconv_fwd_planes_fin(const void* xp, int64_t ldx_bytes, int cin, int64_t n_nodes, const int32_t* seg_ptr,
+                                 const int32_t* col, const int32_t* nbr_ext, const int32_t* multi_seg, int64_t n_multi,
+                                 void* aux, size_t aux_bytes, const void* tfp, int64_t ldt_bytes, int nt, const void* W2,
+                                 int cout, const float* bias, const float* emb, int64_t lde, const int32_t* batch_id,
+                                 const float* res, int64_t ldr, float* out, int64_t ldc, double* stats, int64_t stats_ld,
+                                 void* ws, size_t ws_bytes, void* sync , size_t sync_bytes, int mode,
+                                 int aux_ready, const OfxStatsFin* fin, void* stream);
+int ofx_graphconv_narrow_in_fin(const float* x, int64_t ldx, int cin, int64_t n_nodes, const int32_t* seg_ptr,
+                                const int32_t* col, const uint8_t* node_type, int nt, const float* W, int cout,
+                                const float* bias, const int32_t* batch_id, float* out, int64_t ldc, double* stats,
+                                int64_t stats_ld, void* ws, size_t ws_bytes, const OfxStatsFin* fin, void* stream);
+int ofx_graphconv_narrow_in_tab_fin(const float* x, int64_t ldx, int cin, int64_t n_nodes, const int32_t* seg_ptr,
+                                    const int32_t* col, const int32_t* nbr_ext, const int32_t* multi_seg, int64_t n_multi,
+                                    void* aux, const uint8_t* node_type, int nt, const float* W, int cout,
+                                    const float* bias, const int32_t* batch_id, float* out, int64_t ldc, double* stats,
+                                    int64_t stats_ld, void* ws, size_t ws_bytes, const OfxStatsFin* fin, void* stream);
+
 int ofx_gn_fused_rows(const float* x, int64_t ldx, int rows_per_batch, int batch_size, int C, int groups, float eps,
                       float count_eps, const float* w, const float* bias, int act, float* out, int64_t ldo,
                       void* stream);
diff --git a/octfusion_amd/_lib.py b/octfusion_amd/_lib.py
--- a/octfusion_amd/_lib.py
+++ b/octfusion_amd/_lib.py
@@ -19,6 +19,13 @@
                 ('child_all', c_p), ('key_all', c_p), ('leafrank_all', c_p),
                 ('nnum_host', c_p), ('nnum_nempty_host', c_p)]
 
+
+class OfxStatsFin(ctypes.Structure):
+    _fields_ = [('count', c_p), ('mean', c_p), ('rstd', c_p), ('batch_size', c_i), ('groups', c_i), ('col_off', c_i),
+                ('c_total', c_i), ('eps', c_f), ('count_eps', c_f)]
+
+
+c_fin = ctypes.POINTER(OfxStatsFin)
 
 _SIGS = {
     'ofx_version': (c_i, [], False),
@@ -91,6 +98,10 @@
     'ofx_graphconv_narrow_in_tab': (c_i, [c_p, c_l, c_i, c_l, c_p, c_p, c_p, c_p, c_l, c_p, c_p, c_i, c_p, c_i, c_p, c_p, c_p, c_l, c_p, c_l,
                                           c_p, c_sz, c_p], True),
     'ofx_graphconv_narrow_in': (c_i, [c_p, c_l, c_i, c_l, c_p, c_p, c_p, c_i, c_p, c_i, c_p, c_p, c_p, c_l, c_p, c_l, c_p, c_sz, c_p], True),
+    'ofx_graphconv_narrow_in_tab_fin': (c_i, [c_p, c_l, c_i, c_l, c_p, c_p, c_p, c_p, c_l, c_p, c_p, c_i, c_p, c_i, c_p, c_p, c_p,
+                                              c_l, c_p, c_l, c_p, c_sz, c_fin, c_p], True),
+    'ofx_graphconv_narrow_in_fin': (c_i, [c_p, c_l, c_i, c_l, c_p, c_p, c_p, c_i, c_p, c_i, c_p, c_p, c_p, c_l, c_p, c_l, c_p,
+                                          c_sz, c_fin, c_p], True),
     'ofx_narrow_out_pack': (c_i, [c_p, c_i, c_i, c_i, c_i, c_p, c_p], True),
     'ofx_narrow_out_type_term': (c_i, [c_p, c_l, c_i, c_l, c_p, c_i, c_i, c_p, c_p, c_p], True),
     'ofx_graphconv_narrow_out': (c_i, [c_p, c_l, c_i, c_l, c_p, c_p, c_p, c_p, c_l, c_p], True),
@@ -102,6 +113,8 @@
     'ofx_gemm_f32_planes': (c_i, [c_p, c_l, c_p, c_l, c_l, c_p, c_l, c_l, c_p, c_p, c_l, c_p, c_l, c_p, c_p, c_sz, c_i, c_p], True),
     'ofx_graphconv_fwd': (c_i, [c_p, c_l, c_i, c_l, c_p, c_p, c_p, c_p, c_p, c_l, c_p, c_p, c_l, c_i, c_p, c_l,
                                 c_i, c_p, c_p, c_l, c_p, c_p, c_l, c_p, c_l, c_p, c_l, c_p, c_sz, c_p], True),
+    'ofx_graphconv_fwd_fin': (c_i, [c_p, c_l, c_i, c_l, c_p, c_p, c_p, c_p, c_p, c_l, c_p, c_p, c_l, c_i, c_p, c_l,
+                                    c_i, c_p, c_p, c_l, c_p, c_p, c_l, c_p, c_l, c_p, c_l, c_p, c_sz, c_fin, c_p], True),
     'ofx_planes_split': (c_i, [c_p, c_l, c_l, c_i, c_i, c_i, c_p, c_l, c_p], True),
     'ofx_planes_merge': (c_i, [c_p, c_l, c_l, c_i, c_i, c_p, c_l, c_p], True),
     'ofx_gn_apply_planes': (c_i, [c_p, c_l, c_l, c_i, c_p, c_p, c_p, c_p, c_p, c_i, c_f, c_f, c_p, c_p, c_i, c_i, c_p,
@@ -114,6 +127,9 @@
     'ofx_graphconv_fwd_planes': (c_i, [c_p, c_l, c_i, c_l, c_p, c_p, c_p, c_p, c_l, c_p, c_sz, c_p, c_l, c_i, c_p, c_i,
                                        c_p, c_p, c_l, c_p, c_p, c_l, c_p, c_l, c_p, c_l, c_p, c_sz, c_p, c_sz, c_i, c_i,
                                        c_p], True),
+    'ofx_graphconv_fwd_planes_fin': (c_i, [c_p, c_l, c_i, c_l, c_p, c_p, c_p, c_p, c_l, c_p, c_sz, c_p, c_l, c_i, c_p, c_i,
+                                           c_p, c_p, c_l, c_p, c_p, c_l, c_p, c_l, c_p, c_l, c_p, c_sz, c_p, c_sz, c_i, c_i,
+                                           c_fin, c_p], True),
     'ofx_set_gconv_persistent': (c_i, [c_i], True),
     'ofx_set_gconv_cus': (c_i, [c_i], True),
     'ofx_gemm_planes_packed_bytes': (c_l, [c_i, c_i, c_i], False),
@@ -215,6 +231,9 @@
 
 PROFILE = None
 META = None
+_PROFILE_NAME = {'ofx_graphconv_fwd_fin': 'ofx_graphconv_fwd', 'ofx_graphconv_fwd_planes_fin': 'ofx_graphconv_fwd_planes',
+                 'ofx_graphconv_narrow_in_fin': 'ofx_graphconv_narrow_in',
+                 'ofx_graphconv_narrow_in_tab_fin': 'ofx_graphconv_narrow_in_tab'}
 
 
 def _timed(prof, name, args, always):
@@ -226,7 +245,7 @@
     rc = getattr(lib(), name)(*args)
     e1.record()
     if always or rc == 0:
-        prof.append((name, e0, e1, meta))
+        prof.append((_PROFILE_NAME.get(name, name), e0, e1, meta))
     return rc
 
 
diff --git a/octfusion_amd/csrc/ofx_common.h b/octfusion_amd/csrc/ofx_common.h
--- a/octfusion_amd/csrc/ofx_common.h
+++ b/octfusion_amd/csrc/ofx_common.h
@@ -30,6 +30,17 @@
   if (g < 1) g = 1;
   if (g > 2048 * 4) g = 2048 * 4;
   return (int)g;
+}
+
+__device__ __forceinline__ void ofx_gn_mean_rstd(double S, double SS, float count_b, int cpg, float eps, float count_eps,
+                                                 float& mean, float& rstd) {
+  const float cnt = count_b * (float)cpg;
+  const float inv = 1.0f / (cnt + count_eps);
+  const double m = S * (double)inv;
+  const double ssd = SS - 2.0 * m * S + (double)cnt * m * m;
+  const double var = (ssd > 0 ? ssd : 0) * (double)inv;
+  mean = (float)m;
+  rstd = (float)(1.0 / sqrt(var + (double)eps));
 }
 
 constexpr uint64_t MT_GAMMA = 0x9E3779B97F4A7C15ull;
diff --git a/octfusion_amd/csrc/ofx_gemm.hip b/octfusion_amd/csrc/ofx_gemm.hip
--- a/octfusion_amd/csrc/ofx_gemm.hip
+++ b/octfusion_amd/csrc/ofx_gemm.hip
@@ -824,16 +824,129 @@
   }
 }
 
-int ofx_launch_stats_reduce(const GemmArgs& g, int wr_rows, hipStream_t st) {
+constexpr int STATS_FIN_MAX_WR = 16384;
+__global__ void __launch_bounds__(256) stats_reduce_fin_kernel(const float* __restrict__ part, int nwr, int wr_rows,
+                                                                int N, const int32_t* __restrict__ bid,
+                                                                double* __restrict__ stats, int64_t stats_ld,
+                                                                const OfxStatsFin f) {
+  __shared__ unsigned short list[STATS_FIN_MAX_WR];
+  __shared__ double red[256][2];
+  __shared__ double tot[OFX_STATS_FIN_MAX_CPG][2];
+  __shared__ int wave_cnt[4];
+  __shared__ float ms[2];
+  const int tid = threadIdx.x;
+  const int b = blockIdx.x / f.groups, g = blockIdx.x - b * f.groups;
+  const int cpg = f.c_total / f.groups;
+  const int c0 = g * cpg;
+  const int lo = c0 > f.col_off ? c0 : f.col_off;
+  const int hi = c0 + cpg < f.col_off + N ? c0 + cpg : f.col_off + N;
+  const int ncols = hi > lo ? hi - lo : 0;
+  double* srow = stats + ((int64_t)b * stats_ld - f.col_off) * 2;
+  const bool reduce = part != nullptr && ncols > 0;
+  if (reduce) {
+    const int CH = (nwr + 255) >> 8;
+    const int w_begin = tid * CH;
+    unsigned long long mine = 0;
+    for (int i0 = 0; i0 < CH; i0 += 16) {
+      int bb[16];
+#pragma unroll
+      for (int i = 0; i < 16; ++i) {
+        const int w = w_begin + i0 + i;
+        bb[i] = (i0 + i < CH && w < nwr) ? bid[(int64_t)w * wr_rows] : -1;
+      }
+#pragma unroll
+      for (int i = 0; i < 16; ++i) mine |= (unsigned long long)(bb[i] == b) << (i0 + i);
+    }
+    const int cnt = __popcll(mine);
+    int incl = cnt;
+    const int lane = tid & 63;
+#pragma unroll
+    for (int d = 1; d < 64; d <<= 1) {
+      const int up = __shfl_up(incl, d, 64);
+      if (lane >= d) incl += up;
+    }
+    if (lane == 63) wave_cnt[tid >> 6] = incl;
+    __syncthreads();
+    int base = incl - cnt, n = 0;
+#pragma unroll
+    for (int k = 0; k < 4; ++k) {
+      if (k < (tid >> 6)) base += wave_cnt[k];
+      n += wave_cnt[k];
+    }
+    while (mine) {
+      const int i = __ffsll((long long)mine) - 1;
+      mine &= mine - 1;
+      list[base++] = (unsigned short)(w_begin + i);
+    }
+    __syncthreads();
+    const int RP = 256 / ncols;
+    const int cl = tid % ncols, rl = tid / ncols;
+    double s = 0.0, q = 0.0;
+    if (rl < RP) {
+      const float* pc = part + (int64_t)(lo - f.col_off + cl) * 2;
+      for (int jb = rl; jb < n; jb += 8 * RP) {
+        float2 v[8];
+#pragma unroll
+        for (int i = 0; i < 8; ++i) {
+          const int j = jb + i * RP;
+          v[i] = j < n ? *reinterpret_cast<const float2*>(pc + (int64_t)list[j] * N * 2) : make_float2(0.f, 0.f);
+        }
+#pragma unroll
+        for (int i = 0; i < 8; ++i) { s += (double)v[i].x; q += (double)v[i].y; }
+      }
+    }
+    red[tid][0] = s; red[tid][1] = q;
+    __syncthreads();
+    int P = 1;
+    while (P < RP) P <<= 1;
+    for (int h = P >> 1; h > 0; h >>= 1) {
+      if (rl < h && rl + h < RP) {
+        red[tid][0] += red[tid + h * ncols][0];
+        red[tid][1] += red[tid + h * ncols][1];
+      }
+      __syncthreads();
+    }
+  }
+  if (tid < cpg) {
+    const int c = c0 + tid;
+    const bool own = c >= lo && c < hi;
+    double S = srow[2 * (int64_t)c], Q = srow[2 * (int64_t)c + 1];
+    if (reduce && own) {
+      S += red[c - lo][0]; Q += red[c - lo][1];
+      srow[2 * (int64_t)c] = S; srow[2 * (int64_t)c + 1] = Q;
+    }
+    tot[tid][0] = S; tot[tid][1] = Q;
+  }
+  __syncthreads();
+  if (tid == 0) {
+    double S = 0, SS = 0;
+    for (int k = 0; k < cpg; ++k) { S += tot[k][0]; SS += tot[k][1]; }
+    ofx_gn_mean_rstd(S, SS, f.count[b], cpg, f.eps, f.count_eps, ms[0], ms[1]);
+  }
+  __syncthreads();
+  if (tid < cpg) {
+    f.mean[(int64_t)b * f.c_total + c0 + tid] = ms[0];
+    f.rstd[(int64_t)b * f.c_total + c0 + tid] = ms[1];
+  }
+}
+
+int ofx_launch_stats_reduce(const GemmArgs& g, int wr_rows, hipStream_t st, const OfxStatsFin* fin) {
   const int64_t nwr = ofx_cdiv(g.M, wr_rows);
-  stats_reduce_kernel<<<dim3((unsigned)ofx_cdiv(nwr, 64), (unsigned)ofx_cdiv(g.N, 64)), 256, 0, st>>>(
-      g.stats_part, nwr, wr_rows, g.N, g.bid, g.stats, g.stats_ld);
+  const bool fused = fin && g.stats_part && nwr <= STATS_FIN_MAX_WR;
+  if (g.stats_part && !fused) {
+    stats_reduce_kernel<<<dim3((unsigned)ofx_cdiv(nwr, 64), (unsigned)ofx_cdiv(g.N, 64)), 256, 0, st>>>(
+        g.stats_part, nwr, wr_rows, g.N, g.bid, g.stats, g.stats_ld);
+  }
+  if (fin) {
+    stats_reduce_fin_kernel<<<(unsigned)(fin->batch_size * fin->groups), 256, 0, st>>>(
+        fused ? g.stats_part : nullptr, (int)(fused ? nwr : 0), wr_rows, (int)g.N, g.bid, g.stats, g.stats_ld, *fin);
+  }
   OFX_LAUNCH_CHECK();
   return OFX_OK;
 }
 
 template <int MODE>
-static int launch_gemm(GemmArgs& g, float* ws, size_t ws_bytes, hipStream_t st) {
+static int launch_gemm(GemmArgs& g, float* ws, size_t ws_bytes, hipStream_t st, const OfxStatsFin* fin = nullptr) {
   if (g.M <= 0 || g.N <= 0) return OFX_OK;
   if (MODE == MODE_GATHER && !(g.fast && g.nbr_ext && g.aux && (!g.out_rows || g.gather_out_rows))) return OFX_EINVAL;
   {
@@ -882,8 +995,8 @@
     if (g.vec4 && ws16) splitk_reduce_v4_kernel<<<ofx_grid(g.M * (g.N >> 2), 256), 256, 0, st>>>(g);
     else splitk_reduce_kernel<<<ofx_grid(g.M * g.N, 256), 256, 0, st>>>(g);
   }
-  if (g.stats_part) {
-    rc = ofx_launch_stats_reduce(g, wr_rows, st);
+  if (g.stats_part || fin) {
+    rc = ofx_launch_stats_reduce(g, wr_rows, st, fin);
     if (rc) return rc;
   }
   OFX_LAUNCH_CHECK();
@@ -1042,7 +1155,8 @@
   }
 }
 
-static int launch_gather_via_col(const GemmArgs& g, float* ws, size_t ws_bytes, hipStream_t st) {
+static int launch_gather_via_col(const GemmArgs& g, float* ws, size_t ws_bytes, hipStream_t st,
+                                 const OfxStatsFin* fin = nullptr) {
   if (!ws || (((uintptr_t)ws) & 15)) return OFX_EINVAL;
   size_t tail = ws_bytes / 8;
   if (tail > (size_t(16) << 20)) tail = size_t(16) << 20;
@@ -1064,16 +1178,22 @@
     const int rc = launch_gemm<MODE_DENSE>(d, g.stats ? nullptr : tail_ws, tail, st);
     if (rc) return rc;
   }
+  if (fin) {
+    GemmArgs d = g;
+    d.stats_part = nullptr;
+    return ofx_launch_stats_reduce(d, 64, st, fin);
+  }
   return OFX_OK;
 }
 
-extern "C" int ofx_graphconv_fwd(const float* x, int64_t ldx, int cin, int64_t n_nodes, const int32_t* nbr,
-                                 const int32_t* seg_ptr, const int32_t* col, const int32_t* nbr_ext,
-                                 const int32_t* multi_seg, int64_t n_multi, float* aux, const float* type_frac,
-                                 int64_t ldt, int nt_pad, const float* Wp, int64_t Kp, int cout, const float* bias,
-                                 const float* emb, int64_t lde, const int32_t* batch_id, const float* res, int64_t ldr,
-                                 float* out, int64_t ldc, double* stats, int64_t stats_ld, void* ws, size_t ws_bytes,
-                                 void* stream) {
+extern "C" int ofx_graphconv_fwd_fin(const float* x, int64_t ldx, int cin, int64_t n_nodes, const int32_t* nbr,
+                                     const int32_t* seg_ptr, const int32_t* col, const int32_t* nbr_ext,
+                                     const int32_t* multi_seg, int64_t n_multi, float* aux, const float* type_frac,
+                                     int64_t ldt, int nt_pad, const float* Wp, int64_t Kp, int cout, const float* bias,
+                                     const float* emb, int64_t lde, const int32_t* batch_id, const float* res,
+                                     int64_t ldr, float* out, int64_t ldc, double* stats, int64_t stats_ld, void* ws,
+                                     size_t ws_bytes, const OfxStatsFin* fin, void* stream) {
+  if (fin && !ofx_stats_fin_ok(fin, stats, stats_ld, cout)) return OFX_EINVAL;
   if (n_nodes == 0 && cin >= 1 && cout >= 1) return OFX_OK;
   GemmArgs g = {};
   int rc = gather_common(g, x, ldx, cin, 7, n_nodes, nbr, seg_ptr, col, Wp, Kp, cout, bias, emb, lde, batch_id, res,
@@ -1096,9 +1216,20 @@
                                                                                n_multi, aux, ldx, nullptr);
     g.nbr_ext = nbr_ext; g.aux = aux; g.ldaux = ldx; g.n_src = n_nodes;
     if (!g.tf) { g.tf = x; g.ldt = ldx; }
-    return launch_gemm<MODE_GATHER>(g, (float*)ws, ws_bytes, st);
-  }
-  return launch_gather_via_col(g, stats ? g.stats_part : (float*)ws, stats ? g.stats_part_bytes : ws_bytes, st);
+    return launch_gemm<MODE_GATHER>(g, (float*)ws, ws_bytes, st, fin);
+  }
+  return launch_gather_via_col(g, stats ? g.stats_part : (float*)ws, stats ? g.stats_part_bytes : ws_bytes, st, fin);
+}
+extern "C" int ofx_graphconv_fwd(const float* x, int64_t ldx, int cin, int64_t n_nodes, const int32_t* nbr,
+                                 const int32_t* seg_ptr, const int32_t* col, const int32_t* nbr_ext,
+                                 const int32_t* multi_seg, int64_t n_multi, float* aux, const float* type_frac,
+                                 int64_t ldt, int nt_pad, const float* Wp, int64_t Kp, int cout, const float* bias,
+                                 const float* emb, int64_t lde, const int32_t* batch_id, const float* res, int64_t ldr,
+                                 float* out, int64_t ldc, double* stats, int64_t stats_ld, void* ws, size_t ws_bytes,
+                                 void* stream) {
+  return ofx_graphconv_fwd_fin(x, ldx, cin, n_nodes, nbr, seg_ptr, col, nbr_ext, multi_seg, n_multi, aux, type_frac, ldt,
+                               nt_pad, Wp, Kp, cout, bias, emb, lde, batch_id, res, ldr, out, ldc, stats, stats_ld, ws,
+                               ws_bytes, nullptr, stream);
 }
 
 extern "C" int ofx_graphconv_bwd_data(const float* dy, int64_t ldy, int cout, int64_t n_nodes, const int32_t* nbr_rev,
diff --git a/octfusion_amd/csrc/ofx_gemm2.hip b/octfusion_amd/csrc/ofx_gemm2.hip
--- a/octfusion_amd/csrc/ofx_gemm2.hip
+++ b/octfusion_amd/csrc/ofx_gemm2.hip
@@ -543,7 +543,6 @@
   return OFX_OK;
 }
 
-int ofx_launch_stats_reduce(const GemmArgs& g, int wr_rows, hipStream_t st);
 
 template <int PREC, int WM, int NI>
 static int g2_launch(const Gemm2Args& a, hipStream_t st) {
@@ -580,15 +579,16 @@
   return OFX_OK;
 }
 
-extern "C" int ofx_graphconv_fwd_planes(const void* xp, int64_t ldx_bytes, int cin, int64_t n_nodes,
-                                        const int32_t* seg_ptr, const int32_t* col, const int32_t* nbr_ext,
-                                        const int32_t* multi_seg, int64_t n_multi, void* aux, size_t aux_bytes,
-                                        const void* tfp, int64_t ldt_bytes, int nt, const void* W2, int cout,
-                                        const float* bias, const float* emb, int64_t lde, const int32_t* batch_id,
-                                        const float* res, int64_t ldr, float* out, int64_t ldc, double* stats,
-                                        int64_t stats_ld, void* ws, size_t ws_bytes, void* sync, size_t sync_bytes,
-                                        int mode, int aux_ready, void* stream) {
+extern "C" int ofx_graphconv_fwd_planes_fin(const void* xp, int64_t ldx_bytes, int cin, int64_t n_nodes,
+                                            const int32_t* seg_ptr, const int32_t* col, const int32_t* nbr_ext,
+                                            const int32_t* multi_seg, int64_t n_multi, void* aux, size_t aux_bytes,
+                                            const void* tfp, int64_t ldt_bytes, int nt, const void* W2, int cout,
+                                            const float* bias, const float* emb, int64_t lde, const int32_t* batch_id,
+                                            const float* res, int64_t ldr, float* out, int64_t ldc, double* stats,
+                                            int64_t stats_ld, void* ws, size_t ws_bytes, void* sync, size_t sync_bytes,
+                                            int mode, int aux_ready, const OfxStatsFin* fin, void* stream) {
   if (mode < 1 || mode > 3) return OFX_EINVAL;
+  if (fin && !ofx_stats_fin_ok(fin, stats, stats_ld, cout)) return OFX_EINVAL;
   const int64_t ch = g2_chunk(mode);
   if (n_nodes == 0 && cin >= 1 && cout >= 1) return OFX_OK;
   if (n_nodes < 0 || cin < 1 || (cin % ch) || cout < 1 || !xp || !seg_ptr || !col || !nbr_ext || !aux || !W2 || !out ||
@@ -655,12 +655,25 @@
   if (rc == 1) rc = launch((g2_wm == 2 || g2_wm == 4) ? g2_wm : wm_auto, 0, g.M);
 #undef G2_GO
   if (rc) return rc;
-  if (g.stats_part) {
-    rc = ofx_launch_stats_reduce(g, 64, st);
+  if (g.stats_part || fin) {
+    rc = ofx_launch_stats_reduce(g, 64, st, fin);
     if (rc) return rc;
   }
   OFX_LAUNCH_CHECK();
   return OFX_OK;
+}
+extern "C" int ofx_graphconv_fwd_planes(const void* xp, int64_t ldx_bytes, int cin, int64_t n_nodes,
+                                        const int32_t* seg_ptr, const int32_t* col, const int32_t* nbr_ext,
+                                        const int32_t* multi_seg, int64_t n_multi, void* aux, size_t aux_bytes,
+                                        const void* tfp, int64_t ldt_bytes, int nt, const void* W2, int cout,
+                                        const float* bias, const float* emb, int64_t lde, const int32_t* batch_id,
+                                        const float* res, int64_t ldr, float* out, int64_t ldc, double* stats,
+                                        int64_t stats_ld, void* ws, size_t ws_bytes, void* sync, size_t sync_bytes,
+                                        int mode, int aux_ready, void* stream) {
+  return ofx_graphconv_fwd_planes_fin(xp, ldx_bytes, cin, n_nodes, seg_ptr, col, nbr_ext, multi_seg, n_multi, aux,
+                                      aux_bytes, tfp, ldt_bytes, nt, W2, cout, bias, emb, lde, batch_id, res, ldr, out,
+                                      ldc, stats, stats_ld, ws, ws_bytes, sync, sync_bytes, mode, aux_ready, nullptr,
+                                      stream);
 }
 
 extern "C" int ofx_gemm_planes(const void* ap, int64_t lda_bytes, int64_t n_a, int64_t M, int K, const int32_t* row_tab,
diff --git a/octfusion_amd/csrc/ofx_gemm_common.h b/octfusion_amd/csrc/ofx_gemm_common.h
--- a/octfusion_amd/csrc/ofx_gemm_common.h
+++ b/octfusion_amd/csrc/ofx_gemm_common.h
@@ -29,6 +29,14 @@
   float* stats_part; size_t stats_part_bytes;
 };
 
+int ofx_launch_stats_reduce(const GemmArgs& g, int wr_rows, hipStream_t st, const OfxStatsFin* fin = nullptr);
+constexpr int OFX_STATS_FIN_MAX_CPG = 256;
+static inline bool ofx_stats_fin_ok(const OfxStatsFin* f, const double* stats, int64_t stats_ld, int64_t cout) {
+  return stats && f->count && f->mean && f->rstd && f->batch_size >= 1 && f->groups >= 1 && f->c_total >= 1 &&
+         f->c_total % f->groups == 0 && f->c_total / f->groups <= OFX_STATS_FIN_MAX_CPG && f->col_off >= 0 &&
+         f->col_off + cout <= f->c_total && stats_ld >= cout && (f->c_total == cout || stats_ld >= f->c_total);
+}
+
 static __global__ void __launch_bounds__(256) weight_absmax_kernel(const float* __restrict__ W, int64_t sk, int64_t sn, int64_t K,
                                                             int64_t N, unsigned* __restrict__ acc) {
   __shared__ float red[256];
diff --git a/octfusion_amd/csrc/ofx_narrow.hip b/octfusion_amd/csrc/ofx_narrow.hip
--- a/octfusion_amd/csrc/ofx_narrow.hip
+++ b/octfusion_amd/csrc/ofx_narrow.hip
@@ -1,6 +1,5 @@
 #include "ofx_gemm_common.h"
 
-int ofx_launch_stats_reduce(const GemmArgs& g, int wr_rows, hipStream_t st);
 
 namespace {
 
@@ -412,10 +411,12 @@
 
 }
 
-extern "C" int ofx_graphconv_narrow_in(const float* x, int64_t ldx, int cin, int64_t n_nodes, const int32_t* seg_ptr,
-                                       const int32_t* col, const uint8_t* node_type, int nt, const float* W, int cout,
-                                       const float* bias, const int32_t* batch_id, float* out, int64_t ldc, double* stats,
-                                       int64_t stats_ld, void* ws, size_t ws_bytes, void* stream) {
+extern "C" int ofx_graphconv_narrow_in_fin(const float* x, int64_t ldx, int cin, int64_t n_nodes, const int32_t* seg_ptr,
+                                           const int32_t* col, const uint8_t* node_type, int nt, const float* W, int cout,
+                                           const float* bias, const int32_t* batch_id, float* out, int64_t ldc,
+                                           double* stats, int64_t stats_ld, void* ws, size_t ws_bytes,
+                                           const OfxStatsFin* fin, void* stream) {
+  if (fin && !ofx_stats_fin_ok(fin, stats, stats_ld, cout)) return OFX_EINVAL;
   if (!x || !seg_ptr || !col || !W || !out || cin < 1 || cin > 8 || ldx < cin || nt < 0 || nt > 8 || (nt > 0 && !node_type) ||
       (cout != 64 && cout != 128) || ldc < cout || n_nodes < 0 ||
       7 * (cin + nt) > 96)
@@ -434,16 +435,27 @@
   if (stats) {
     GemmArgs g = {};
     g.M = n_nodes; g.N = cout; g.bid = batch_id; g.stats = stats; g.stats_ld = stats_ld; g.stats_part = (float*)ws;
-    return ofx_launch_stats_reduce(g, 64, st);
+    return ofx_launch_stats_reduce(g, 64, st, fin);
   }
   return OFX_OK;
 }
 
-extern "C" int ofx_graphconv_narrow_in_tab(const float* x, int64_t ldx, int cin, int64_t n_nodes, const int32_t* seg_ptr,
-                                           const int32_t* col, const int32_t* nbr_ext, const int32_t* multi_seg,
-                                           int64_t n_multi, void* aux, const uint8_t* node_type, int nt, const float* W,
-                                           int cout, const float* bias, const int32_t* batch_id, float* out, int64_t ldc,
-                                           double* stats, int64_t stats_ld, void* ws, size_t ws_bytes, void* stream) {
+extern "C" int ofx_graphconv_narrow_in(const float* x, int64_t ldx, int cin, int64_t n_nodes, const int32_t* seg_ptr,
+                                       const int32_t* col, const uint8_t* node_type, int nt, const float* W, int cout,
+                                       const float* bias, const int32_t* batch_id, float* out, int64_t ldc, double* stats,
+                                       int64_t stats_ld, void* ws, size_t ws_bytes, void* stream) {
+  return ofx_graphconv_narrow_in_fin(x, ldx, cin, n_nodes, seg_ptr, col, node_type, nt, W, cout, bias, batch_id, out, ldc,
+                                     stats, stats_ld, ws, ws_bytes, nullptr, stream);
+}
+
+extern "C" int ofx_graphconv_narrow_in_tab_fin(const float* x, int64_t ldx, int cin, int64_t n_nodes,
+                                               const int32_t* seg_ptr, const int32_t* col, const int32_t* nbr_ext,
+                                               const int32_t* multi_seg, int64_t n_multi, void* aux,
+                                               const uint8_t* node_type, int nt, const float* W, int cout,
+                                               const float* bias, const int32_t* batch_id, float* out, int64_t ldc,
+                                               double* stats, int64_t stats_ld, void* ws, size_t ws_bytes,
+                                               const OfxStatsFin* fin, void* stream) {
+  if (fin && !ofx_stats_fin_ok(fin, stats, stats_ld, cout)) return OFX_EINVAL;
   if (!x || !seg_ptr || !col || !nbr_ext || !aux || ((uintptr_t)aux & 15) || n_multi < 0 || (n_multi > 0 && !multi_seg) || !W ||
       !out || cin < 1 || cin > 8 || ldx < cin || nt < 0 || nt > 8 || (nt > 0 && !node_type) || (cout != 64 && cout != 128) ||
       ldc < cout || n_nodes < 0 || 7 * (cin + nt) > 96 || n_nodes + 1 + n_multi >= (1ll << 31))
@@ -481,9 +493,19 @@
   if (stats) {
     GemmArgs g = {};
     g.M = n_nodes; g.N = cout; g.bid = batch_id; g.stats = stats; g.stats_ld = stats_ld; g.stats_part = (float*)ws;
-    return ofx_launch_stats_reduce(g, 64, st);
+    return ofx_launch_stats_reduce(g, 64, st, fin);
   }
   return OFX_OK;
+}
+
+extern "C" int ofx_graphconv_narrow_in_tab(const float* x, int64_t ldx, int cin, int64_t n_nodes, const int32_t* seg_ptr,
+                                           const int32_t* col, const int32_t* nbr_ext, const int32_t* multi_seg,
+                                           int64_t n_multi, void* aux, const uint8_t* node_type, int nt, const float* W,
+                                           int cout, const float* bias, const int32_t* batch_id, float* out, int64_t ldc,
+                                           double* stats, int64_t stats_ld, void* ws, size_t ws_bytes, void* stream) {
+  return ofx_graphconv_narrow_in_tab_fin(x, ldx, cin, n_nodes, seg_ptr, col, nbr_ext, multi_seg, n_multi, aux, node_type,
+                                         nt, W, cout, bias, batch_id, out, ldc, stats, stats_ld, ws, ws_bytes, nullptr,
+                                         stream);
 }
 
 extern "C" int ofx_narrow_out_pack(const float* W, int C, int nt, int cout, int pw, float* Wd, void* stream) {
diff --git a/octfusion_amd/csrc/ofx_norm.hip b/octfusion_amd/csrc/ofx_norm.hip
--- a/octfusion_amd/csrc/ofx_norm.hip
+++ b/octfusion_amd/csrc/ofx_norm.hip
@@ -114,14 +114,10 @@
       S += sums[((int64_t)b * C + c) * 2];
       SS += sums[((int64_t)b * C + c) * 2 + 1];
     }
-    const float cnt = count[b] * (float)cpg;
-    const float inv = 1.0f / (cnt + count_eps);
-    const double m = S * (double)inv;
-    const double ssd = SS - 2.0 * m * S + (double)cnt * m * m;
-    const double var = (ssd > 0 ? ssd : 0) * (double)inv;
-    const float rs = (float)(1.0 / sqrt(var + (double)eps));
+    float m, rs;
+    ofx_gn_mean_rstd(S, SS, count[b], cpg, eps, count_eps, m, rs);
     for (int c = g * cpg; c < (g + 1) * cpg; ++c) {
-      mean[(int64_t)b * C + c] = (float)m;
+      mean[(int64_t)b * C + c] = m;
       rstd[(int64_t)b * C + c] = rs;
     }
   }
@@ -151,13 +147,7 @@
     S += f.sums[((int64_t)b * C + c) * 2];
     SS += f.sums[((int64_t)b * C + c) * 2 + 1];
   }
-  const float cnt = f.count[b] * (float)cpg;
-  const float inv = 1.0f / (cnt + f.count_eps);
-  const double m = S * (double)inv;
-  const double ssd = SS - 2.0 * m * S + (double)cnt * m * m;
-  const double var = (ssd > 0 ? ssd : 0) * (double)inv;
-  mean = (float)m;
-  rstd = (float)(1.0 / sqrt(var + (double)f.eps));
+  ofx_gn_mean_rstd(S, SS, f.count[b], cpg, f.eps, f.count_eps, mean, rstd);
 }
 template <int MODE, bool FIN>
 __global__ void __launch_bounds__(256) gn_apply_kernel(const float* __restrict__ x, int64_t ldx, int64_t n, int C,
diff --git a/octfusion_amd/graph_unet_hr.py b/octfusion_amd/graph_unet_hr.py
--- a/octfusion_amd/graph_unet_hr.py
+++ b/octfusion_amd/graph_unet_hr.py
@@ -165,9 +165,19 @@
         for (c_h, c_skip, dd) in self._cat_plan:
             cat_bufs.append(torch.empty(n_at[dd], c_h + c_skip, dtype=torch.float32, device=dev))
 
+        cat_stats = [ops.stats_buffer(doctree.batch_size, c_h + c_skip, dev) if ops.STATS_FIN else None
+                     for (c_h, c_skip, _) in self._cat_plan]
+
         def skip_slot(i):
             c_h, c_skip, _ = self._cat_plan[i]
             return cat_bufs[i][:, c_h:]
+
+        def skip_stats(i):
+            return (cat_stats[i], self._cat_plan[i][0]) if cat_stats[i] is not None else None
+
+        def block1_norm_of(module):
+            return module.block1_norm if isinstance(module, GraphResBlockEmbed) else None
+        enc_next = list(self.input_blocks[1:]) + [self.middle_block1 if unet_lr is not None else None]
 
         d = self.input_depth
         if as_middle:
@@ -175,16 +185,18 @@
             ops.rows_copy(x, skip_slot(0), x.shape[0])
             hs = [skip_slot(0)]
         else:
-            h = self.input_blocks[0](x, doctree, d, out=skip_slot(0))
+            h = self.input_blocks[0](x, doctree, d, out=skip_slot(0), norm=block1_norm_of(enc_next[0]),
+                                     stats_slot=skip_stats(0))
             hs = [h]
         if emb_fork is not None:
             emb_main.wait_stream(emb_fork)
         for k, ((kind, dd, _), module) in enumerate(zip(self._enc, self.input_blocks[1:])):
             slot = skip_slot(k + 1)
-            if kind == 'res':
-                h = module(h, emb, doctree, dd, emb_act=emb_act, out=slot, emb_out=emb_outs[id(module)])
-            else:
-                h = module(h, doctree, dd, out=slot)
+            nxt = dict(out_norm=block1_norm_of(enc_next[k + 1]), out_stats=skip_stats(k + 1))
+            if kind == 'res':
+                h = module(h, emb, doctree, dd, emb_act=emb_act, out=slot, emb_out=emb_outs[id(module)], **nxt)
+            else:
+                h = module(h, doctree, dd, out=slot, **nxt)
             hs.append(h)
         d = self._d_mid
 
@@ -208,9 +220,17 @@
         for idx, ((kind, dd, _), module) in enumerate(zip(self._dec, self.output_blocks)):
             nxt_is_res = idx + 1 < len(self._dec) and self._dec[idx + 1][0] == 'res'
             out_slot = None
+            nxt = {}
             if nxt_is_res:
-                c_h_n = self._cat_plan[n_skip - 1 - (j + (1 if kind == 'res' else 0))][0]
-                out_slot = cat_bufs[n_skip - 1 - (j + (1 if kind == 'res' else 0))][:, :c_h_n]
+                sn = n_skip - 1 - (j + (1 if kind == 'res' else 0))
+                c_h_n = self._cat_plan[sn][0]
+                out_slot = cat_bufs[sn][:, :c_h_n]
+                if cat_stats[sn] is not None:
+                    seam = ops.get_stats(hs[sn]) is not None and ops.get_stats(hs[sn]).dim() == 3
+                    nxt = dict(out_stats=(cat_stats[sn], 0),
+                               out_norm=self.output_blocks[idx + 1].block1_norm if seam else None)
+            elif idx + 1 == len(self._dec):
+                nxt = dict(out_norm=self.end_norm)
             if kind == 'res':
                 si = n_skip - 1 - j
                 c_h = self._cat_plan[si][0]
@@ -221,11 +241,12 @@
                     if st is not None:
                         setattr(left, ops.STATS_ATTR, st)
                     pending = left
-                hcat = ops.cat_channels(pending, hs[si], buf=cat_bufs[si])
-                pending = module(hcat, emb, doctree, dd, emb_act=emb_act, out=out_slot, emb_out=emb_outs[id(module)])
+                hcat = ops.cat_channels(pending, hs[si], buf=cat_bufs[si], stats_buf=cat_stats[si])
+                pending = module(hcat, emb, doctree, dd, emb_act=emb_act, out=out_slot, emb_out=emb_outs[id(module)],
+                                 **nxt)
                 j += 1
             else:
-                pending = module(pending, doctree, dd, out=out_slot)
+                pending = module(pending, doctree, dd, out=out_slot, **nxt)
         h = pending
         h = self.end_norm(h, doctree, self.input_depth, act='silu', out=out_mid if as_middle else None)
         if as_middle:
diff --git a/octfusion_amd/modules.py b/octfusion_amd/modules.py
--- a/octfusion_amd/modules.py
+++ b/octfusion_amd/modules.py
@@ -58,13 +58,22 @@
             nn.init.zeros_(self.bias)
 
     @torch.no_grad()
-    def forward(self, x, doctree, d, emb=None, res=None, out=None, split_input=False):
+    def forward(self, x, doctree, d, emb=None, res=None, out=None, split_input=False, norm=None, stats_slot=None):
         nt = self.n_node_type if self.n_node_type > 1 else 0
         seg_ptr, col, N, E = doctree.csr(d)
         assert x.shape[0] == N, 'x has %d rows, graph depth %d has %d nodes' % (x.shape[0], d, N)
-        stats = None
+        stats = fin = None
         if self.emit_stats and N * self.out_channels >= (1 << 14) and self.out_channels % 4 == 0:
-            stats = ops.stats_zeros(doctree.batch_size * self.out_channels * 2, x.device)
+            off, c_total = 0, self.out_channels
+            if stats_slot is not None:
+                off, c_total = stats_slot[1], stats_slot[0].shape[1]
+                stats = ops.stats_view(stats_slot[0], off, self.out_channels)
+            else:
+                stats = ops.stats_zeros(doctree.batch_size * self.out_channels * 2, x.device)
+            if norm is not None and ops.STATS_FIN and norm.in_channels in (self.out_channels, c_total):
+                own = norm.in_channels == self.out_channels
+                fin = ops.StatsFin(doctree.count(d), doctree.batch_size, norm.group, norm.eps, norm.eps,
+                                   self.out_channels if own else c_total, 0 if own else off, x.device)
         mode = ops.planes_of(x)
         cin_k = self.in_channels
         if not mode and emb is None and res is None:
@@ -72,10 +81,8 @@
                 y = ops.graphconv_narrow_in(x, seg_ptr, col, self.weights, self.in_channels, nt,
                                             doctree.node_type8(d) if nt else None, self.bias if self.use_bias else None,
                                             doctree.batch_id32(d) if stats is not None else None, out, stats,
-                                            ext=doctree.ext(d))
-                if stats is not None:
-                    setattr(y, ops.STATS_ATTR, stats)
-                return y
+                                            ext=doctree.ext(d), fin=fin)
+                return self._with_stats(y, stats, fin)
             if ops.NARROW_OUT and self.out_channels <= 8 and self.in_channels % 32 == 0 and N >= 4096:
                 pno = self._pno.get(self.weights, self.in_channels, nt)
                 bias = self.bias if self.use_bias else None
@@ -100,18 +107,24 @@
                                      doctree.type_frac_planes(d, nt, mode) if nt else None,
                                      self.bias if self.use_bias else None, emb,
                                      doctree.batch_id32(d) if (emb is not None or stats is not None) else None,
-                                     res, out, stats=stats)
-            if stats is not None:
-                setattr(y, ops.STATS_ATTR, stats)
-            return y
+                                     res, out, stats=stats, fin=fin)
+            return self._with_stats(y, stats, fin)
         pw = self._pw.get(self.weights, 'graphconv', self.in_channels, nt)
         tf = doctree.type_frac(d, nt) if nt else None
         y = ops.graphconv(x, doctree.nbr(d), seg_ptr, col, pw, self.in_channels, tf,
                           self.bias if self.use_bias else None, emb,
                           doctree.batch_id32(d) if (emb is not None or stats is not None) else None, res, out,
-                          ext=doctree.ext(d), stats=stats)
+                          ext=doctree.ext(d), stats=stats, fin=fin)
+        return self._with_stats(y, stats, fin)
+
+    @staticmethod
+    def _with_stats(y, stats, fin):
         if stats is not None:
             setattr(y, ops.STATS_ATTR, stats)
+        if fin is not None:
+            setattr(y, ops.FIN_ATTR, fin.result)
+        elif hasattr(y, ops.FIN_ATTR):
+            delattr(y, ops.FIN_ATTR)
         return y
 
     def extra_repr(self):
@@ -146,9 +159,11 @@
             aux_graph = ops.AuxGraph(seg_ptr, col, multi_seg, n_multi, oct_plan, block_plan)
         y = ops.group_norm(data, doctree.batch_id32(depth), doctree.count(depth), doctree.batch_size,
                            self.weights, self.bias, self.group, self.eps, act, out, stats=stats, planes=planes,
-                           aux_graph=aux_graph)
+                           aux_graph=aux_graph, fin=ops.get_fin(data))
         if out is data and stats is not None:
             delattr(data, ops.STATS_ATTR)
+            if hasattr(data, ops.FIN_ATTR):
+                delattr(data, ops.FIN_ATTR)
         return y
 
     def extra_repr(self):
@@ -331,9 +346,9 @@
         self.downsample = Downsample(channels_in)
         self.conv = GraphConv(channels_in, channels_out, n_edge_type, avg_degree, n_node_type)
 
-    def forward(self, x, doctree, d, out=None):
+    def forward(self, x, doctree, d, out=None, out_norm=None, out_stats=None):
         return self.conv(pool_nodes(x, doctree, d, self.downsample, planes=self.conv.planes_mode(doctree, d - 1)),
-                         doctree, d - 1, out=out, split_input=True)
+                         doctree, d - 1, out=out, split_input=True, norm=out_norm, stats_slot=out_stats)
 
 
 class GraphUpsample(nn.Module):
@@ -345,9 +360,9 @@
         self.upsample = Upsample(channels_in)
         self.conv = GraphConv(channels_in, channels_out, n_edge_type, avg_degree, n_node_type)
 
-    def forward(self, x, doctree, d, out=None):
+    def forward(self, x, doctree, d, out=None, out_norm=None, out_stats=None):
         return self.conv(unpool_nodes(x, doctree, d, self.upsample, planes=self.conv.planes_mode(doctree, d + 1)),
-                         doctree, d + 1, out=out, split_input=True)
+                         doctree, d + 1, out=out, split_input=True, norm=out_norm, stats_slot=out_stats)
 
 
 def graphnormalization(channels):
@@ -385,7 +400,7 @@
             self.skip_connection = Conv1x1(self.channels, self.out_channels)
 
     @torch.no_grad()
-    def forward(self, x, emb, doctree, depth, emb_act=None, out=None, emb_out=None):
+    def forward(self, x, emb, doctree, depth, emb_act=None, out=None, emb_out=None, out_norm=None, out_stats=None):
         skip, side = x, None
         if not isinstance(self.skip_connection, nn.Identity):
             if ops.SIDE_STREAM:
@@ -401,11 +416,11 @@
                 emb_act = ops.act(emb, 'silu')
             emb_out = self.emb_layers[1](emb_act)
         assert doctree.batch_size == emb_out.shape[0]
-        h = self.conv1(h, doctree, depth, emb=emb_out)
+        h = self.conv1(h, doctree, depth, emb=emb_out, norm=self.block2_norm)
         h = self.block2_norm(h, doctree, depth, act='silu', out=h, planes=self.conv2.planes_mode(doctree, depth))
         if side is not None:
             main.wait_stream(side)
-        return self.conv2(h, doctree, depth, res=skip, out=out)
+        return self.conv2(h, doctree, depth, res=skip, out=out, norm=out_norm, stats_slot=out_stats)
 
 
 class GraphResBlock(nn.Module):
@@ -427,7 +442,7 @@
     @torch.no_grad()
     def forward(self, x, doctree, depth):
         h = self.norm1(x, doctree, depth, act='silu', planes=self.conv1.planes_mode(doctree, depth))
-        h = self.conv1(h, doctree, depth)
+        h = self.conv1(h, doctree, depth, norm=self.norm2)
         h = self.norm2(h, doctree, depth, act='silu', out=h, planes=self.conv2.planes_mode(doctree, depth))
         if self.channel_in != self.channel_out:
             x = self.conv1x1c(x, doctree, depth)
diff --git a/octfusion_amd/ops.py b/octfusion_amd/ops.py
--- a/octfusion_amd/ops.py
+++ b/octfusion_amd/ops.py
@@ -1,4 +1,5 @@
 import contextlib
+import ctypes
 import os
 from typing import NamedTuple
 
@@ -232,7 +233,7 @@
 
 
 def graphconv_planes(xp, mode, seg_ptr, col, ext, pw, cin, nt, tf_planes=None, bias=None, emb=None, batch_id=None,
-                     res=None, out=None, stats=None):
+                     res=None, out=None, stats=None, fin=None):
     assert planes_of(xp) == mode and xp.shape[1] == cin
     N = xp.shape[0]
     bpc = 4 if planes_pairs(mode) else 2
@@ -259,10 +260,14 @@
         sync = sync_words(xp.device)
         _meta('graphconv', flops, 0, (N, pw.cin, pw.N, 'planes', 'emb' if emb is not None else '',
                                       'res' if res is not None else '', 'stats' if stats is not None else ''))
-        call('ofx_graphconv_fwd_planes', ptr(xp), ldx, cin, N, ptr(seg_ptr), ptr(col), ptr(nbr_ext), ptr(multi_seg),
-             n_multi, ptr(aux), aux.numel() * aux.element_size(), ptr(tf_planes), ldt, nt, ptr(pw.t), pw.N, ptr(bias),
-             ptr(emb), lde, ptr(batch_id) if (emb is not None or stats is not None) else None, ptr(res), ldr, ptr(out),
-             ldc, ptr(stats), pw.N, ptr(ws), ws.numel(), ptr(sync), sync.numel() * 4, mode, aux_ready, stream())
+        args = (ptr(xp), ldx, cin, N, ptr(seg_ptr), ptr(col), ptr(nbr_ext), ptr(multi_seg),
+                n_multi, ptr(aux), aux.numel() * aux.element_size(), ptr(tf_planes), ldt, nt, ptr(pw.t), pw.N, ptr(bias),
+                ptr(emb), lde, ptr(batch_id) if (emb is not None or stats is not None) else None, ptr(res), ldr, ptr(out),
+                ldc, ptr(stats), _stats_ld(stats, pw.N), ptr(ws), ws.numel(), ptr(sync), sync.numel() * 4, mode, aux_ready)
+        if fin is not None:
+            call('ofx_graphconv_fwd_planes_fin', *args, fin.ref(), stream())
+        else:
+            call('ofx_graphconv_fwd_planes', *args, stream())
     return out
 
 
@@ -534,7 +539,7 @@
 
 
 def graphconv(x, nbr, seg_ptr, col, pw, cin, type_frac=None, bias=None, emb=None, batch_id=None,
-              res=None, out=None, ext=None, stats=None):
+              res=None, out=None, ext=None, stats=None, fin=None):
     x, ldx = _row_major(x)
     N = x.shape[0]
     if x.shape[1] != cin:
@@ -561,11 +566,12 @@
         if ext is not None and cin % 32 == 0:
             nbr_ext, multi_seg, n_multi = ext
             aux = torch.empty((n_multi + 1) * ldx, dtype=torch.float32, device=x.device)
-        args = ('ofx_graphconv_fwd', ptr(x), ldx, cin, N, ptr(nbr), ptr(seg_ptr), ptr(col), ptr(nbr_ext), ptr(multi_seg),
-                n_multi, ptr(aux), ptr(type_frac), ldt, nt_pad,
+        args = ('ofx_graphconv_fwd_fin' if fin is not None else 'ofx_graphconv_fwd', ptr(x), ldx, cin, N, ptr(nbr),
+                ptr(seg_ptr), ptr(col), ptr(nbr_ext), ptr(multi_seg), n_multi, ptr(aux), ptr(type_frac), ldt, nt_pad,
                 ptr(pw.t), pw.Kp, pw.N, ptr(bias), ptr(emb), lde,
                 ptr(batch_id) if (emb is not None or stats is not None) else None,
-                ptr(res), ldr, ptr(out), ldc, ptr(stats), pw.N, ptr(ws), ws.numel(), stream())
+                ptr(res), ldr, ptr(out), ldc, ptr(stats), _stats_ld(stats, pw.N), ptr(ws), ws.numel()) + (
+                    (fin.ref(),) if fin is not None else ()) + (stream(),)
         _meta('graphconv', flops, 0, (N, cin, pw.N, 'reg'))
         if pw.N <= 64 or cin <= 64:
             with policy_scope('small_gemm'):
@@ -588,7 +594,7 @@
 
 
 def graphconv_narrow_in(x, seg_ptr, col, weights, cin, nt, node_type=None, bias=None, batch_id=None, out=None, stats=None,
-                        ext=None):
+                        ext=None, fin=None):
     x, ldx = _row_major(x)
     w = weights.detach()
     if not w.is_contiguous():
@@ -612,14 +618,19 @@
         if ext is not None and NARROW_IN_TAB and N >= NARROW_IN_TAB_MIN_ROWS:
             nbr_ext, multi_seg, n_multi = ext
             aux = torch.empty((N + n_multi + 1) * (8 if cin <= 4 else 16), dtype=torch.float32, device=x.device)
-            call('ofx_graphconv_narrow_in_tab', ptr(x), ldx, cin, N, ptr(seg_ptr), ptr(col), ptr(nbr_ext), ptr(multi_seg),
-                 n_multi, ptr(aux), ptr(node_type) if nt else None, nt, ptr(w), cout, ptr(bias),
-                 ptr(batch_id) if stats is not None else None, ptr(out), ldc, ptr(stats), cout, ptr(ws), ws.numel(),
-                 stream())
+            name, args = 'ofx_graphconv_narrow_in_tab', (
+                ptr(x), ldx, cin, N, ptr(seg_ptr), ptr(col), ptr(nbr_ext), ptr(multi_seg), n_multi, ptr(aux),
+                ptr(node_type) if nt else None, nt, ptr(w), cout, ptr(bias), ptr(batch_id) if stats is not None else None,
+                ptr(out), ldc, ptr(stats), _stats_ld(stats, cout), ptr(ws), ws.numel())
         else:
-            call('ofx_graphconv_narrow_in', ptr(x), ldx, cin, N, ptr(seg_ptr), ptr(col), ptr(node_type) if nt else None, nt,
-                 ptr(w), cout, ptr(bias), ptr(batch_id) if stats is not None else None, ptr(out), ldc, ptr(stats), cout,
-                 ptr(ws), ws.numel(), stream())
+            name, args = 'ofx_graphconv_narrow_in', (
+                ptr(x), ldx, cin, N, ptr(seg_ptr), ptr(col), ptr(node_type) if nt else None, nt, ptr(w), cout, ptr(bias),
+                ptr(batch_id) if stats is not None else None, ptr(out), ldc, ptr(stats), _stats_ld(stats, cout), ptr(ws),
+                ws.numel())
+        if fin is not None:
+            call(name + '_fin', *args, fin.ref(), stream())
+        else:
+            call(name, *args, stream())
     return out
 
 
@@ -873,12 +884,12 @@
     block_plan: tuple = None
 
 
-def _gn_launch(planes, aux_graph, elems, cpg=2):
+def _gn_launch(planes, aux_graph, elems, cpg=2, have_fin=False):
     g = aux_graph if planes else None
     oct_plan, block_plan = (g.oct_plan, g.block_plan) if g is not None and AUX_PLAN else (None, None)
     oct_fin = (GN_OCT_FINALIZE and AUX_PLAN == 'oct' and oct_plan is not None and elems <= GN_OCT_FINALIZE_MAX_ELEMS
                and cpg >= 2)
-    finalize = GN_FINALIZE_LAUNCH or (g is not None and not GN_FUSE_AUX_FINALIZE and not oct_fin)
+    finalize = have_fin or GN_FINALIZE_LAUNCH or (g is not None and not GN_FUSE_AUX_FINALIZE and not oct_fin)
     if not planes:
         return 'fp32', finalize
     if oct_plan is not None:
@@ -887,7 +898,7 @@
 
 
 def group_norm(x, batch_id, count, batch_size, weight, bias, groups, eps=1e-5, act=None, out=None,
-               count_eps=None, stats=None, rows_per_batch=None, planes=0, aux_graph=None):
+               count_eps=None, stats=None, rows_per_batch=None, planes=0, aux_graph=None, fin=None):
     if count_eps is None:
         count_eps = eps
     x, ldx = _row_major(x)
@@ -902,10 +913,17 @@
         call('ofx_gn_fused_rows', ptr(x), ldx, rows_per_batch, batch_size, C, groups, eps, count_eps,
              ptr(weight.detach().reshape(-1)), ptr(bias.detach().reshape(-1)), ACT[act], ptr(out), ldo, stream())
         return out
+    use_fin = (fin is not None and stats is not None and fin.C == C and fin.groups == groups and fin.eps == eps and
+               fin.count_eps == count_eps and fin.mean.numel() == batch_size * C)
+    launch, finalize = _gn_launch(planes, aux_graph, n * C, C // groups)
+    if use_fin and (finalize or GN_PRODUCER_FIN_SMALL):
+        launch, finalize = _gn_launch(planes, aux_graph, n * C, C // groups, have_fin=True)
+    else:
+        use_fin = False
     if stats is not None:
         _chk(stats, torch.float64)
         assert stats.numel() == batch_size * C * 2
-        sums = stats
+        sums = stats if use_fin or stats.is_contiguous() else stats.contiguous()
     else:
         _meta('gn_stats', 0, 4.0 * n * C, (n, C))
         if stats_pool_has_room(batch_size * C * 2, dev):
@@ -917,8 +935,9 @@
     w = weight.detach().reshape(-1)
     b = bias.detach().reshape(-1)
     mean = rstd = None
-    launch, finalize = _gn_launch(planes, aux_graph, n * C, C // groups)
-    if finalize:
+    if use_fin:
+        mean, rstd = fin.mean, fin.rstd
+    elif finalize:
         mean = torch.empty(batch_size * C, dtype=torch.float32, device=dev)
         rstd = torch.empty(batch_size * C, dtype=torch.float32, device=dev)
         _meta('gn_finalize', 0, 24.0 * batch_size * C, (batch_size, C))
@@ -982,6 +1001,56 @@
 
 
 STATS_ATTR = '_ofx_gn_stats'
+FIN_ATTR = '_ofx_gn_fin'
+STATS_FIN = os.environ.get('OFX_STATS_FIN', '1') == '1'
+GN_PRODUCER_FIN_SMALL = os.environ.get('OFX_GN_PRODUCER_FIN_SMALL', '1') == '1'
+
+
+class NormFin(NamedTuple):
+    mean: torch.Tensor
+    rstd: torch.Tensor
+    C: int
+    groups: int
+    eps: float
+    count_eps: float
+
+
+class StatsFin:
+
+    def __init__(self, count, batch_size, groups, eps, count_eps, c_total, col_off, device):
+        _chk(count)
+        mean = torch.empty(batch_size * c_total, dtype=torch.float32, device=device)
+        rstd = torch.empty(batch_size * c_total, dtype=torch.float32, device=device)
+        self.result = NormFin(mean, rstd, c_total, groups, eps, count_eps)
+        self._count = count
+        self._desc = _lib.OfxStatsFin(ptr(count), ptr(mean), ptr(rstd), batch_size, groups, col_off, c_total, eps, count_eps)
+
+    def ref(self):
+        return ctypes.byref(self._desc)
+
+
+def _carry_pool(src, dst):
+    for a in ('_ofx_gen', '_ofx_pool'):
+        if hasattr(src, a):
+            setattr(dst, a, getattr(src, a))
+    return dst
+
+
+def _stats_ld(stats, cout):
+    return stats.stride(0) // 2 if stats is not None and stats.dim() == 3 else cout
+
+
+def stats_view(buf, off, C):
+    return _carry_pool(buf, buf[:, off:off + C])
+
+
+def stats_buffer(batch_size, C, device):
+    flat = stats_zeros(batch_size * C * 2, device)
+    return _carry_pool(flat, flat.view(batch_size, C, 2))
+
+
+def get_fin(t):
+    return getattr(t, FIN_ATTR, None) if get_stats(t) is not None else None
 
 
 class _StatsPool:
@@ -1039,12 +1108,22 @@
     return st
 
 
-def cat_channels(a, b, buf=None):
+def cat_channels(a, b, buf=None, stats_buf=None):
     out = buf if buf is not None else torch.cat([a, b], dim=1)
     sa, sb = get_stats(a), get_stats(b)
     if sa is not None and sb is not None:
-        B = sa.numel() // (a.shape[1] * 2)
-        st = torch.cat([sa.view(B, a.shape[1], 2), sb.view(B, b.shape[1], 2)], dim=1).contiguous().view(-1)
+        Ca, Cb = a.shape[1], b.shape[1]
+        if (stats_buf is not None and sa.dim() == 3 and sb.dim() == 3 and stats_buf.shape[1] == Ca + Cb and
+                sa.data_ptr() == stats_buf.data_ptr() and sb.data_ptr() == stats_buf[:, Ca:].data_ptr() and
+                sa.stride(0) == sb.stride(0) == stats_buf.stride(0)):
+            st = _carry_pool(stats_buf, stats_buf.view(-1))
+            for t in (a, b):
+                f = getattr(t, FIN_ATTR, None)
+                if f is not None and f.C == Ca + Cb:
+                    setattr(out, FIN_ATTR, f)
+        else:
+            B = sa.numel() // (Ca * 2)
+            st = torch.cat([sa.reshape(B, Ca, 2), sb.reshape(B, Cb, 2)], dim=1).contiguous().view(-1)
         setattr(out, STATS_ATTR, st)
     return out
 
```
